# scale-lab/MTLoRA

Hardware: AMD Instinct MI355X
Metric: images/sec (train step) Swin-T/448 r=64 4-task (higher is better)
Workload: dtype bf16; 1 GPU; BASELINE configs[1]: Swin-T 448, 4 tasks (semseg,normals,sal,human_parts), r_shared=64 r_task=4 scale4; train step (fwd+loss+bwd+clip+AdamW), dropout .05, drop_path .2; per_gpu_batch=32, global_batch=32, img_size=448, parallelism=dp1, trainable_params=8344634, allreduce_bytes=0

## Files before the change

include/mtlora_hip.h:

```cpp
#ifndef MTLORA_HIP_H
#define MTLORA_HIP_H

#include <stdint.h>

#ifdef __cplusplus
extern "C" {
#endif

#define MTLORA_ABI_VERSION 12
#define MTLORA_MAX_TASKS 8

typedef enum mtlora_dtype {
    MTLORA_F32 = 0,
    MTLORA_BF16 = 1,
    MTLORA_F16 = 2,
    MTLORA_U8 = 3
} mtlora_dtype;

typedef enum mtlora_status {
    MTLORA_OK = 0,
    MTLORA_ERR_DTYPE = -1,
    MTLORA_ERR_SHAPE = -2,
    MTLORA_ERR_ALIGN = -3,
    MTLORA_ERR_NULL = -4,
// ... 4 lines not shown

int mtlora_version(void);
const char* mtlora_error_string(int status);

int mtlora_roll_and_window_partition_forward(const void* image, void* windows, int64_t B, int64_t H, int64_t W,
                                             int64_t C, int shift_size, int window_size, int dtype, void* stream);
int mtlora_roll_and_window_partition_backward(const void* grad_windows, void* grad_image, int64_t B, int64_t H,
                                              int64_t W, int64_t C, int shift_size, int window_size, int dtype,
                                              void* stream);
int mtlora_window_merge_and_roll_forward(const void* windows, void* image, int64_t B, int64_t H, int64_t W,
                                         int64_t C, int shift_size, int window_size, int dtype, void* stream);
int mtlora_window_merge_and_roll_backward(const void* grad_image, void* grad_windows, int64_t B, int64_t H,
                                          int64_t W, int64_t C, int shift_size, int window_size, int dtype,
                                          void* stream);

typedef struct mtlora_linear_desc {
    int64_t M, K, N;
    int32_t dtype;
    int32_t mode;
    int32_t T;
    int32_t r_s;
    int32_t r_t[MTLORA_MAX_TASKS];
    float scale_s;
    float scale_t[MTLORA_MAX_TASKS];
    int32_t has_x_tasks;
    float dropout_p;
    uint64_t seed;
    const uint64_t* seed_offset;
    int32_t bwd_phase;
    int32_t sel_stream;
    int32_t sel_dense;
    int32_t sel_tn;
    int32_t sel_projk;
    int32_t max_cu;
    const void* packed;
    int32_t hid;
    int32_t hid_pad_;
    const void* hid_ptr;
} mtlora_linear_desc;

#define MTLORA_HID_FWD_BASE 1
#define MTLORA_HID_P_GIVEN 2
#define MTLORA_HID_Q_GIVEN 4

int64_t mtlora_linear_ctx_bytes(const mtlora_linear_desc* d);

int64_t mtlora_linear_packed_bytes(const mtlora_linear_desc* d);
int mtlora_linear_pack(const mtlora_linear_desc* d, const float* A_s, const float* B_s, const float* const* A_t,
                       const float* const* B_t, void* packed, int64_t packed_bytes, void* stream);
int64_t mtlora_linear_pack_entry_bytes(void);
int mtlora_linear_pack_entry(const mtlora_linear_desc* d, const float* A_s, const float* B_s, const float* const* A_t,
                             const float* const* B_t, void* packed, int64_t packed_bytes, void* entry_host);
int mtlora_linear_pack_table(const void* table_dev, int n_entries, int dtype, void* stream);
int64_t mtlora_linear_bwd_scratch_bytes(const mtlora_linear_desc* d);

int mtlora_linear_fwd(const mtlora_linear_desc* d, const void* x, const void* const* x_t, const void* W,
                      const float* bias, const float* A_s, const float* B_s, const float* const* A_t,
                      const float* const* B_t, void* y_s, void* const* y_t, void* ctx, int64_t ctx_bytes,
                      void* stream);

int mtlora_linear_bwd(const mtlora_linear_desc* d, const void* x, const void* const* x_t, const void* Wt,
                      const void* dy_s, const void* const* dy_t, const void* ctx, int64_t ctx_bytes, void* dx,
                      void* const* dx_t, float* dA_s, float* dB_s, float* const* dA_t, float* const* dB_t,
                      void* scratch, int64_t scratch_bytes, void* stream);

int mtlora_linear_fwd_gelu(const mtlora_linear_desc* d, const void* x, const void* const* x_t, const void* W,
                           const float* bias, const float* A_s, const float* B_s, const float* const* A_t,
                           const float* const* B_t, void* y_s, void* const* y_t, void* a_s, void* const* a_t, void* ctx,
                           int64_t ctx_bytes, void* stream);

int mtlora_linear_bwd_gelu(const mtlora_linear_desc* d, const void* x, const void* const* x_t, const void* Wt,
                           const void* dy_s, const void* const* dy_t, const void* ctx, int64_t ctx_bytes, void* dx,
                           void* const* dx_t, float* dA_s, float* dB_s, float* const* dA_t, float* const* dB_t,
                           void* scratch, int64_t scratch_bytes, const void* h_s, const void* const* h_t, void* stream);

int mtlora_mlp_hid_supported(const mtlora_linear_desc* d1, const mtlora_linear_desc* d2);
int64_t mtlora_mlp_hid_fwd_scratch_bytes(const mtlora_linear_desc* d1, const mtlora_linear_desc* d2);
int64_t mtlora_mlp_hid_bwd_scratch_bytes(const mtlora_linear_desc* d1, const mtlora_linear_desc* d2);
int mtlora_mlp_hid_proj(const mtlora_linear_desc* d1, const mtlora_linear_desc* d2, const void* h_base, const void* ctx1,
                        void* ctx2, void* scratch, int64_t scratch_bytes, void* stream);
int mtlora_mlp_hid_bwd(const mtlora_linear_desc* d1, const mtlora_linear_desc* d2, const void* h_base, const void* dh_s,
                       const void* ctx1, const void* ctx2, const void* scratch2, void* scratch1, void* g, float* const* dB1_t,
                       float* const* dA2_t, void* part, int64_t part_bytes, void* stream);

int64_t mtlora_gemm_tn_scratch_bytes(int64_t M, int Na, int Nb);
int mtlora_gemm_tn(const void* a, const void* b, float* out, int64_t M, int Na, int Nb, int64_t lda, int64_t ldb,
                   int dtype, void* scratch, int64_t scratch_bytes, void* stream);

typedef struct mtlora_attn_desc {
    int64_t B;
    int32_t H, W;
    int32_t window_size;
    int32_t shift;
    int32_t num_heads;
    int32_t head_dim;
    int32_t image_layout;
    int32_t dtype;
    float scale;
    float mask_value;
} mtlora_attn_desc;

int64_t mtlora_window_attn_bwd_scratch_bytes(const mtlora_attn_desc* d);

int mtlora_window_attn_fwd(const mtlora_attn_desc* d, const void* qkv, const float* bias, const float* mask,
                           const int32_t* mask_ids, void* out, void* stream);
int mtlora_window_attn_bwd(const mtlora_attn_desc* d, const void* qkv, const float* bias, const float* mask,
                           const int32_t* mask_ids, const void* dout, void* dqkv, float* dbias, void* scratch,
                           int64_t scratch_bytes, void* stream);

int mtlora_layernorm_fwd(const void* x, const float* gamma, const float* beta, void* y, float* mean, float* rstd,
                         int64_t M, int64_t C, float eps, int x_dtype, int y_dtype, int merge_h, int merge_w, void* stream);
int64_t mtlora_layernorm_bwd_scratch_bytes(int64_t M, int64_t C, int x_dtype);
int mtlora_layernorm_bwd(const void* dy, const void* x, const float* gamma, const float* mean, const float* rstd,
                         void* dx, float* dgamma, float* dbeta, int64_t M, int64_t C, int x_dtype, int dy_dtype,
                         void* scratch, int64_t scratch_bytes, const void* dx_addend, int merge_h, int merge_w, void* stream);

int mtlora_residual_layernorm_fwd(const void* shortcut, const void* branch, const float* scale, int64_t B, const float* gamma,
                                  const float* beta, void* x_new, void* y, float* mean, float* rstd, int64_t M, int64_t C,
                                  float eps, int x_dtype, int y_dtype, void* stream);
int mtlora_residual_layernorm_bwd(const void* dy, const void* x_new, const float* gamma, const float* mean, const float* rstd,
                                  void* d_shortcut, void* d_branch, float* dgamma, float* dbeta, const float* scale,
                                  int64_t B, int64_t M, int64_t C, int x_dtype, int dy_dtype, void* scratch,
                                  int64_t scratch_bytes, const void* dx_addend, void* stream);

int64_t mtlora_layernorm_multi_bwd_scratch_bytes(int n, int64_t M, int64_t C, int x_dtype);
int mtlora_layernorm_multi_fwd(int n, const void* const* x, const float* gamma, const float* beta, void* const* y,
                               float* const* mean, float* const* rstd, int64_t M, int64_t C, float eps, int x_dtype, int y_dtype,
                               int merge_h, int merge_w, void* stream);
int mtlora_layernorm_multi_bwd(int n, const void* const* dy, const void* const* x, const float* gamma, const float* const* mean,
                               const float* const* rstd, void* const* dx, float* dgamma, float* dbeta, int64_t M, int64_t C,
                               int x_dtype, int dy_dtype, void* scratch, int64_t scratch_bytes, const void* const* dx_addend,
                               int merge_h, int merge_w, void* stream);

int mtlora_residual_layernorm_streams_fwd(int n, const void* const* res, const void* const* branch, const float* scale,
                                          int64_t B, const float* gamma, const float* beta, void* const* x_new, void* const* y,
                                          float* const* mean, float* const* rstd, int64_t M, int64_t C, float eps, int x_dtype,
                                          int y_dtype, int merge_h, int merge_w, void* stream);
int mtlora_residual_layernorm_streams_bwd(int n, const void* const* dy, const void* const* x_new, const float* gamma,
                                          const float* const* mean, const float* const* rstd, void* const* d_res,
                                          void* const* d_branch, float* dgamma, float* dbeta, const float* scale, int64_t B,
                                          int64_t M, int64_t C, int x_dtype, int dy_dtype, void* scratch, int64_t scratch_bytes,
                                          const void* const* dx_addend, int merge_h, int merge_w, void* stream);

int mtlora_residual_layernorm_multi_fwd(int n, const void* shortcut, const void* const* branch, const float* scale, int64_t B,
                                        const float* gamma, const float* beta, void* const* x_new, void* const* y,
                                        float* const* mean, float* const* rstd, int64_t M, int64_t C, float eps, int x_dtype,
                                        int y_dtype, void* stream);
int mtlora_residual_layernorm_multi_bwd(int n, const void* const* dy, const void* const* x_new, const float* gamma,
                                        const float* const* mean, const float* const* rstd, const void* const* dx_addend,
                                        void* d_shortcut, void* const* d_branch, float* dgamma, float* dbeta, const float* scale,
                                        int64_t B, int64_t M, int64_t C, int x_dtype, int dy_dtype, void* scratch,
                                        int64_t scratch_bytes, void* stream);

int64_t mtlora_bn_scratch_bytes(int64_t R, int64_t C, int dtype);
int mtlora_bn_relu_fwd(const void* x, const float* gamma, const float* beta, float* running_mean, float* running_var,
                       float momentum, float eps, int relu, void* y, float* save_mean, float* save_rstd,
                       float* save_scale, float* save_shift, int64_t R, int64_t C, int dtype, void* scratch,
                       int64_t scratch_bytes, void* stream);
int mtlora_bn_relu_bwd(const void* dy, const void* x, const float* save_mean, const float* save_rstd,
                       const float* save_scale, const float* save_shift, int relu, void* dx, float* dgamma, float* dbeta,
                       int64_t R, int64_t C, int dtype, void* scratch, int64_t scratch_bytes, void* stream);

int mtlora_residual_droppath_fwd(int n, const void* const* res, const void* const* y, void* const* out,
                                 const float* scale, int64_t M, int64_t C, int64_t B, int res_dtype, int y_dtype,
                                 void* stream);
int mtlora_residual_droppath_bwd(int n, const void* const* g, void* const* dy, void* dres, const float* scale,
                                 int64_t M, int64_t C, int64_t B, int res_dtype, int y_dtype, void* stream);

int64_t mtlora_upsample_loss_partials(int64_t B, int h, int w, int scale);
int mtlora_upsample_loss(int kind, const void* low, const float* label, const float* stat, void* dlow, float* partials,
                         int64_t B, int h, int w, int C, int scale, int dtype, float ignore_index, void* stream);

int mtlora_upsample_metrics_sizes(int kind, int64_t B, int h, int w, int C, int scale, int64_t* n_int64,
                                  int64_t* n_float_partials);
int mtlora_upsample_metrics(int kind, const void* low, const float* label, const float* stat, int64_t* counts,
                            float* fpartials, int64_t B, int h, int w, int C, int scale, int dtype, float ignore_index,
                            void* stream);

int mtlora_upsample_predict(int kind, const void* low, void* out, int64_t B, int h, int w, int C, int scale, int dtype,
                            int out_dtype, void* stream);

int64_t mtlora_colsum_scratch_bytes(int64_t M, int64_t N);
int mtlora_colsum(const void* x, int64_t M, int64_t N, int dtype, float* out, void* scratch, int64_t scratch_bytes, void* stream);
int64_t mtlora_label_stat_scratch_bytes(int64_t n);
int mtlora_label_stat(const float* label, int64_t n, int kind, float ignore_index, float* out, void* scratch,
                      int64_t scratch_bytes, void* stream);

int mtlora_upsample_cl_fwd(const void* coarse, void* fine, int64_t B, int h, int w, int C, int scale, int64_t ld_fine,
                           int dtype, void* stream);
int mtlora_upsample_cl_bwd(const void* grad_fine, void* grad_coarse, int64_t B, int h, int w, int C, int scale,
                           int64_t ld_fine, int dtype, void* stream);

typedef struct mtlora_block_desc {
    int64_t B;
    int32_t H, W, C, hidden;
    int32_t num_heads, window_size, shift;
    int32_t dtype;
    int32_t x_dtype;
    int32_t has_norm1;
    float eps1, eps2, eps_next;
    float attn_scale, mask_value;
    mtlora_linear_desc lin[4];
} mtlora_block_desc;

typedef struct mtlora_block_params {
    const float *norm1_g, *norm1_b;
    const float *norm2_g, *norm2_b, *next_g, *next_b;
    const void* W[4];
    const void* Wt[4];
    const float* bias[4];
    const float* A[4];
    const float* Bf[4];
    const float* attn_bias;
    const int32_t* mask_ids;
    const float* mask;
    const float *scale1, *scale2;
} mtlora_block_params;

typedef struct mtlora_block_grads {
    void* g_x;
    void* g_normed;
    float *d_norm1_g, *d_norm1_b;
    float *d_norm2_g, *d_norm2_b, *d_next_g, *d_next_b;
    float* dA[4];
    float* dB[4];
    float* dbias;
} mtlora_block_grads;

int64_t mtlora_block_save_bytes(const mtlora_block_desc* d);
int64_t mtlora_block_fwd_tmp_bytes(const mtlora_block_desc* d);
int64_t mtlora_block_bwd_scratch_bytes(const mtlora_block_desc* d);
int mtlora_block_fwd(const mtlora_block_desc* d, const mtlora_block_params* p, const void* x, const void* normed, void* x_out,
                     void* normed_out, void* save, int64_t save_bytes, void* tmp, int64_t tmp_bytes, void* stream);
int mtlora_block_bwd(const mtlora_block_desc* d, const mtlora_block_params* p, const void* x, const void* normed,
                     const void* x_out, const void* g_x_out, const void* g_normed_out, const void* save, int64_t save_bytes,
                     const mtlora_block_grads* g, void* scratch, int64_t scratch_bytes, int phase, void* stream);

#define MTLORA_ADAMW_CHUNK 4096
#define MTLORA_ADAMW_MAX_GROUPS 16
#define MTLORA_ADAMW_CTRL_WORDS 64
typedef struct mtlora_adamw_group {
    double lr, beta1, beta2, eps, weight_decay;
} mtlora_adamw_group;
int mtlora_adamw_sizes(int64_t n_tensors, const int64_t* numel, int64_t* n_chunks, int64_t* table_bytes,
                       int64_t* scratch_bytes);
int mtlora_adamw_table(int64_t n_tensors, const int64_t* numel, const int32_t* group, void* const* p, void* const* m,
                       void* const* v, void* host_table, int64_t table_bytes);
int mtlora_adamw_update(const void* table, const void* grads, int64_t n_tensors, int64_t n_chunks,
                        const mtlora_adamw_group* groups, int n_groups, float max_norm, float* ctrl, float* norm_out,
                        float* scale, int32_t* growth_tracker, float growth_factor, float backoff_factor,
                        int growth_interval, void* scratch, int64_t scratch_bytes, void* stream);

#define MTLORA_INGEST_MAX_JOBS 8
typedef enum mtlora_ingest_kind {
    MTLORA_INGEST_IMAGE = 0,
    MTLORA_INGEST_CLASS = 1,
    MTLORA_INGEST_CLASS_ALLZERO_IGNORE = 2,
    MTLORA_INGEST_NORMALS = 3,
    MTLORA_INGEST_DEPTH = 4
} mtlora_ingest_kind;
typedef struct mtlora_ingest_job {
    const void* src;
    void* dst;
    int32_t kind, src_dtype, C, reserved;
} mtlora_ingest_job;
int64_t mtlora_ingest_scratch_bytes(int n_jobs, int64_t B);
int mtlora_ingest_batch(const mtlora_ingest_job* jobs, int n_jobs, int64_t B, int32_t H, int32_t W, const uint8_t* flip,
                        const float* lut, void* scratch, int64_t scratch_bytes, void* stream);

#define MTLORA_AUGMENT_GEOM_BITS 24
#define MTLORA_AUGMENT_FLAG_NO_RENORM 1
typedef enum mtlora_augment_kind {
    MTLORA_AUGMENT_IMAGE_CUBIC_U8 = 0,
    MTLORA_AUGMENT_CLASS_NEAREST_U8 = 1,
    MTLORA_AUGMENT_NORMALS_CUBIC_F32 = 2,
    MTLORA_AUGMENT_DEPTH_NEAREST_F32 = 3
} mtlora_augment_kind;
typedef struct mtlora_augment_job {
    const void* src;
    void* dst;
    int32_t kind, flags;
} mtlora_augment_job;
int mtlora_augment_batch(const mtlora_augment_job* jobs, int n_jobs, int64_t B, int32_t Hc, int32_t Wc, int32_t Ho, int32_t Wo,
                         const int32_t* size, const int64_t* geom, const float* side, const int32_t* cubic_q15,
                         const float* cubic_f32, void* stream);

int mtlora_selftest_layouts(int32_t* out, void* stream);

#define MTLORA_PROF_KINDS 24
typedef struct mtlora_prof_summary {
    int64_t count[MTLORA_PROF_KINDS];
    double ms[MTLORA_PROF_KINDS];
    double alg_bytes[MTLORA_PROF_KINDS];
    double s8d_bytes[MTLORA_PROF_KINDS];
    double flops[MTLORA_PROF_KINDS];
} mtlora_prof_summary;
int mtlora_prof_begin(int max_records);
int mtlora_prof_end(mtlora_prof_summary* out);
const char* mtlora_prof_kind_name(int kind);

#ifdef __cplusplus
}
#endif
#endif
```

mtlora_amd/_lib.py:

```python
from __future__ import annotations

import ctypes
import os
from ctypes import POINTER, Structure, c_char_p, c_double, c_float, c_int, c_int32, c_int64, c_uint64, c_void_p

import torch

MAX_TASKS = 8
ABI_VERSION = 12
F32, BF16, F16, U8 = 0, 1, 2, 3
_DT = {torch.float32: F32, torch.bfloat16: BF16, torch.float16: F16}

_HERE = os.path.dirname(os.path.abspath(__file__))
LIB_PATH = os.path.join(_HERE, "csrc", "libmtlora_hip.so")


class LinearDesc(Structure):
    _fields_ = [("M", c_int64), ("K", c_int64), ("N", c_int64), ("dtype", c_int32), ("mode", c_int32),
                ("T", c_int32), ("r_s", c_int32), ("r_t", c_int32 * MAX_TASKS), ("scale_s", c_float),
                ("scale_t", c_float * MAX_TASKS), ("has_x_tasks", c_int32), ("dropout_p", c_float),
                ("seed", c_uint64), ("seed_offset", c_void_p), ("bwd_phase", c_int32),
                ("sel_stream", c_int32), ("sel_dense", c_int32), ("sel_tn", c_int32), ("sel_projk", c_int32),
                ("max_cu", c_int32), ("packed", c_void_p),
                ("hid", c_int32), ("hid_pad_", c_int32), ("hid_ptr", c_void_p)]


HID_FWD_BASE, HID_P_GIVEN, HID_Q_GIVEN = 1, 2, 4


class AttnDesc(Structure):
    _fields_ = [("B", c_int64), ("H", c_int32), ("W", c_int32), ("window_size", c_int32), ("shift", c_int32),
                ("num_heads", c_int32), ("head_dim", c_int32), ("image_layout", c_int32), ("dtype", c_int32),
                ("scale", c_float), ("mask_value", c_float)]


class BlockDesc(Structure):
    _fields_ = [("B", c_int64), ("H", c_int32), ("W", c_int32), ("C", c_int32), ("hidden", c_int32), ("num_heads", c_int32),
                ("window_size", c_int32), ("shift", c_int32), ("dtype", c_int32), ("x_dtype", c_int32), ("has_norm1", c_int32),
                ("eps1", c_float), ("eps2", c_float), ("eps_next", c_float), ("attn_scale", c_float), ("mask_value", c_float),
                ("lin", LinearDesc * 4)]


class BlockParams(Structure):
    _fields_ = [("norm1_g", c_void_p), ("norm1_b", c_void_p), ("norm2_g", c_void_p), ("norm2_b", c_void_p), ("next_g", c_void_p),
                ("next_b", c_void_p), ("W", c_void_p * 4), ("Wt", c_void_p * 4), ("bias", c_void_p * 4), ("A", c_void_p * 4),
                ("Bf", c_void_p * 4), ("attn_bias", c_void_p), ("mask_ids", c_void_p), ("mask", c_void_p), ("scale1", c_void_p),
                ("scale2", c_void_p)]


class BlockGrads(Structure):
    _fields_ = [("g_x", c_void_p), ("g_normed", c_void_p), ("d_norm1_g", c_void_p), ("d_norm1_b", c_void_p), ("d_norm2_g", c_void_p),
                ("d_norm2_b", c_void_p), ("d_next_g", c_void_p), ("d_next_b", c_void_p), ("dA", c_void_p * 4), ("dB", c_void_p * 4),
                ("dbias", c_void_p)]


class AdamwGroup(Structure):
    _fields_ = [("lr", c_double), ("beta1", c_double), ("beta2", c_double), ("eps", c_double), ("weight_decay", c_double)]


class IngestJob(Structure):
    _fields_ = [("src", c_void_p), ("dst", c_void_p), ("kind", c_int32), ("src_dtype", c_int32), ("C", c_int32),
                ("reserved", c_int32)]


class AugmentJob(Structure):
    _fields_ = [("src", c_void_p), ("dst", c_void_p), ("kind", c_int32), ("flags", c_int32)]


INGEST_MAX_JOBS = 8
AUGMENT_IMAGE_CUBIC_U8, AUGMENT_CLASS_NEAREST_U8, AUGMENT_NORMALS_CUBIC_F32, AUGMENT_DEPTH_NEAREST_F32 = 0, 1, 2, 3
AUGMENT_GEOM_BITS, AUGMENT_FLAG_NO_RENORM = 24, 1
INGEST_IMAGE, INGEST_CLASS, INGEST_CLASS_ALLZERO_IGNORE, INGEST_NORMALS, INGEST_DEPTH = 0, 1, 2, 3, 4

ADAMW_CHUNK, ADAMW_MAX_GROUPS, ADAMW_CTRL_WORDS = 4096, 16, 64

PROF_KINDS = 24


class ProfSummary(Structure):
    _fields_ = [("count", c_int64 * PROF_KINDS), ("ms", ctypes.c_double * PROF_KINDS),
                ("alg_bytes", ctypes.c_double * PROF_KINDS), ("s8d_bytes", ctypes.c_double * PROF_KINDS),
                ("flops", ctypes.c_double * PROF_KINDS)]


PtrArr = c_void_p * MAX_TASKS
PtrArr9 = c_void_p * (MAX_TASKS + 1)

_SIGS = {
    "mtlora_version": (c_int, []),
    "mtlora_error_string": (c_char_p, [c_int]),
    "mtlora_roll_and_window_partition_forward": (c_int, [c_void_p, c_void_p, c_int64, c_int64, c_int64, c_int64, c_int, c_int, c_int, c_void_p]),
    "mtlora_roll_and_window_partition_backward": (c_int, [c_void_p, c_void_p, c_int64, c_int64, c_int64, c_int64, c_int, c_int, c_int, c_void_p]),
    "mtlora_window_merge_and_roll_forward": (c_int, [c_void_p, c_void_p, c_int64, c_int64, c_int64, c_int64, c_int, c_int, c_int, c_void_p]),
    "mtlora_window_merge_and_roll_backward": (c_int, [c_void_p, c_void_p, c_int64, c_int64, c_int64, c_int64, c_int, c_int, c_int, c_void_p]),
    "mtlora_linear_ctx_bytes": (c_int64, [POINTER(LinearDesc)]),
    "mtlora_linear_bwd_scratch_bytes": (c_int64, [POINTER(LinearDesc)]),
    "mtlora_linear_packed_bytes": (c_int64, [POINTER(LinearDesc)]),
    "mtlora_linear_pack": (c_int, [POINTER(LinearDesc), c_void_p, c_void_p, POINTER(c_void_p), POINTER(c_void_p), c_void_p, c_int64,
                                   c_void_p]),
    "mtlora_linear_pack_entry_bytes": (c_int64, []),
    "mtlora_linear_pack_entry": (c_int, [POINTER(LinearDesc), c_void_p, c_void_p, POINTER(c_void_p), POINTER(c_void_p), c_void_p, c_int64,
                                         c_void_p]),
    "mtlora_linear_pack_table": (c_int, [c_void_p, c_int, c_int, c_void_p]),
    "mtlora_linear_fwd": (c_int, [POINTER(LinearDesc), c_void_p, POINTER(c_void_p), c_void_p, c_void_p, c_void_p, c_void_p,
                                  POINTER(c_void_p), POINTER(c_void_p), c_void_p, POINTER(c_void_p), c_void_p, c_int64,
                                  c_void_p]),
    "mtlora_linear_bwd": (c_int, [POINTER(LinearDesc), c_void_p, POINTER(c_void_p), c_void_p, c_void_p, POINTER(c_void_p),
                                  c_void_p, c_int64, c_void_p, POINTER(c_void_p), c_void_p, c_void_p, POINTER(c_void_p),
                                  POINTER(c_void_p), c_void_p, c_int64, c_void_p]),
    "mtlora_gemm_tn_scratch_bytes": (c_int64, [c_int64, c_int, c_int]),
    "mtlora_gemm_tn": (c_int, [c_void_p, c_void_p, c_void_p, c_int64, c_int, c_int, c_int64, c_int64, c_int, c_void_p, c_int64,
                               c_void_p]),
    "mtlora_linear_fwd_gelu": (c_int, [POINTER(LinearDesc), c_void_p, POINTER(c_void_p), c_void_p, c_void_p, c_void_p, c_void_p,
                                       POINTER(c_void_p), POINTER(c_void_p), c_void_p, POINTER(c_void_p), c_void_p,
                                       POINTER(c_void_p), c_void_p, c_int64, c_void_p]),
    "mtlora_linear_bwd_gelu": (c_int, [POINTER(LinearDesc), c_void_p, POINTER(c_void_p), c_void_p, c_void_p, POINTER(c_void_p),
                                       c_void_p, c_int64, c_void_p, POINTER(c_void_p), c_void_p, c_void_p, POINTER(c_void_p),
                                       POINTER(c_void_p), c_void_p, c_int64, c_void_p, POINTER(c_void_p), c_void_p]),
    "mtlora_mlp_hid_supported": (c_int, [POINTER(LinearDesc), POINTER(LinearDesc)]),
    "mtlora_mlp_hid_bwd_scratch_bytes": (c_int64, [POINTER(LinearDesc), POINTER(LinearDesc)]),
    "mtlora_mlp_hid_fwd_scratch_bytes": (c_int64, [POINTER(LinearDesc), POINTER(LinearDesc)]),
    "mtlora_mlp_hid_proj": (c_int, [POINTER(LinearDesc), POINTER(LinearDesc), c_void_p, c_void_p, c_void_p, c_void_p, c_int64, c_void_p]),
    "mtlora_mlp_hid_bwd": (c_int, [POINTER(LinearDesc), POINTER(LinearDesc), c_void_p, c_void_p, c_void_p, c_void_p, c_void_p, c_void_p,
                                   c_void_p, POINTER(c_void_p), POINTER(c_void_p), c_void_p, c_int64, c_void_p]),
    "mtlora_window_attn_bwd_scratch_bytes": (c_int64, [POINTER(AttnDesc)]),
    "mtlora_window_attn_fwd": (c_int, [POINTER(AttnDesc), c_void_p, c_void_p, c_void_p, c_void_p, c_void_p, c_void_p]),
    "mtlora_window_attn_bwd": (c_int, [POINTER(AttnDesc), c_void_p, c_void_p, c_void_p, c_void_p, c_void_p, c_void_p,
                                       c_void_p, c_void_p, c_int64, c_void_p]),
    "mtlora_layernorm_fwd": (c_int, [c_void_p, c_void_p, c_void_p, c_void_p, c_void_p, c_void_p, c_int64, c_int64, c_float,
                                     c_int, c_int, c_int, c_int, c_void_p]),
    "mtlora_layernorm_bwd_scratch_bytes": (c_int64, [c_int64, c_int64, c_int]),
    "mtlora_residual_layernorm_fwd": (c_int, [c_void_p, c_void_p, c_void_p, c_int64, c_void_p, c_void_p, c_void_p, c_void_p,
                                              c_void_p, c_void_p, c_int64, c_int64, c_float, c_int, c_int, c_void_p]),
    "mtlora_layernorm_multi_bwd_scratch_bytes": (c_int64, [c_int, c_int64, c_int64, c_int]),
    "mtlora_layernorm_multi_fwd": (c_int, [c_int, POINTER(c_void_p), c_void_p, c_void_p, POINTER(c_void_p), POINTER(c_void_p),
                                           POINTER(c_void_p), c_int64, c_int64, c_float, c_int, c_int, c_int, c_int, c_void_p]),
    "mtlora_layernorm_multi_bwd": (c_int, [c_int, POINTER(c_void_p), POINTER(c_void_p), c_void_p, POINTER(c_void_p),
                                           POINTER(c_void_p), POINTER(c_void_p), c_void_p, c_void_p, c_int64, c_int64, c_int,
                                           c_int, c_void_p, c_int64, POINTER(c_void_p), c_int, c_int, c_void_p]),
    "mtlora_residual_layernorm_streams_fwd": (c_int, [c_int, POINTER(c_void_p), POINTER(c_void_p), c_void_p, c_int64, c_void_p,
                                                      c_void_p, POINTER(c_void_p), POINTER(c_void_p), POINTER(c_void_p),
                                                      POINTER(c_void_p), c_int64, c_int64, c_float, c_int, c_int, c_int, c_int,
                                                      c_void_p]),
    "mtlora_residual_layernorm_streams_bwd": (c_int, [c_int, POINTER(c_void_p), POINTER(c_void_p), c_void_p, POINTER(c_void_p),
                                                      POINTER(c_void_p), POINTER(c_void_p), POINTER(c_void_p), c_void_p, c_void_p,
                                                      c_void_p, c_int64, c_int64, c_int64, c_int, c_int, c_void_p, c_int64,
                                                      POINTER(c_void_p), c_int, c_int, c_void_p]),
    "mtlora_residual_layernorm_multi_fwd": (c_int, [c_int, c_void_p, POINTER(c_void_p), c_void_p, c_int64, c_void_p, c_void_p,
                                                    POINTER(c_void_p), POINTER(c_void_p), POINTER(c_void_p), POINTER(c_void_p),
                                                    c_int64, c_int64, c_float, c_int, c_int, c_void_p]),
    "mtlora_residual_layernorm_multi_bwd": (c_int, [c_int, POINTER(c_void_p), POINTER(c_void_p), c_void_p, POINTER(c_void_p),
                                                    POINTER(c_void_p), POINTER(c_void_p), c_void_p, POINTER(c_void_p), c_void_p,
                                                    c_void_p, c_void_p, c_int64, c_int64, c_int64, c_int, c_int, c_void_p, c_int64,
                                                    c_void_p]),
    "mtlora_residual_layernorm_bwd": (c_int, [c_void_p, c_void_p, c_void_p, c_void_p, c_void_p, c_void_p, c_void_p, c_void_p,
                                              c_void_p, c_void_p, c_int64, c_int64, c_int64, c_int, c_int, c_void_p, c_int64,
                                              c_void_p, c_void_p]),
    "mtlora_layernorm_bwd": (c_int, [c_void_p, c_void_p, c_void_p, c_void_p, c_void_p, c_void_p, c_void_p, c_void_p,
                                     c_int64, c_int64, c_int, c_int, c_void_p, c_int64, c_void_p, c_int, c_int, c_void_p]),
    "mtlora_bn_scratch_bytes": (c_int64, [c_int64, c_int64, c_int]),
    "mtlora_bn_relu_fwd": (c_int, [c_void_p, c_void_p, c_void_p, c_void_p, c_void_p, c_float, c_float, c_int, c_void_p,
                                   c_void_p, c_void_p, c_void_p, c_void_p, c_int64, c_int64, c_int, c_void_p, c_int64,
                                   c_void_p]),
    "mtlora_bn_relu_bwd": (c_int, [c_void_p, c_void_p, c_void_p, c_void_p, c_void_p, c_void_p, c_int, c_void_p, c_void_p,
                                   c_void_p, c_int64, c_int64, c_int, c_void_p, c_int64, c_void_p]),
    "mtlora_residual_droppath_fwd": (c_int, [c_int, POINTER(c_void_p), POINTER(c_void_p), POINTER(c_void_p), c_void_p,
                                             c_int64, c_int64, c_int64, c_int, c_int, c_void_p]),
    "mtlora_residual_droppath_bwd": (c_int, [c_int, POINTER(c_void_p), POINTER(c_void_p), c_void_p, c_void_p, c_int64,
                                             c_int64, c_int64, c_int, c_int, c_void_p]),
    "mtlora_upsample_loss_partials": (c_int64, [c_int64, c_int, c_int, c_int]),
    "mtlora_colsum_scratch_bytes": (c_int64, [c_int64, c_int64]),
    "mtlora_colsum": (c_int, [c_void_p, c_int64, c_int64, c_int, c_void_p, c_void_p, c_int64, c_void_p]),
    "mtlora_label_stat_scratch_bytes": (c_int64, [c_int64]),
    "mtlora_label_stat": (c_int, [c_void_p, c_int64, c_int, c_float, c_void_p, c_void_p, c_int64, c_void_p]),
    "mtlora_upsample_loss": (c_int, [c_int, c_void_p, c_void_p, c_void_p, c_void_p, c_void_p, c_int64, c_int, c_int, c_int,
                                     c_int, c_int, ctypes.c_float, c_void_p]),
    "mtlora_upsample_metrics_sizes": (c_int, [c_int, c_int64, c_int, c_int, c_int, c_int, POINTER(c_int64), POINTER(c_int64)]),
    "mtlora_upsample_metrics": (c_int, [c_int, c_void_p, c_void_p, c_void_p, c_void_p, c_void_p, c_int64, c_int, c_int, c_int,
                                        c_int, c_int, ctypes.c_float, c_void_p]),
    "mtlora_upsample_predict": (c_int, [c_int, c_void_p, c_void_p, c_int64, c_int, c_int, c_int, c_int, c_int, c_int, c_void_p]),
    "mtlora_upsample_cl_fwd": (c_int, [c_void_p, c_void_p, c_int64, c_int, c_int, c_int, c_int, c_int64, c_int, c_void_p]),
    "mtlora_upsample_cl_bwd": (c_int, [c_void_p, c_void_p, c_int64, c_int, c_int, c_int, c_int, c_int64, c_int, c_void_p]),
    "mtlora_block_save_bytes": (c_int64, [POINTER(BlockDesc)]),
    "mtlora_block_fwd_tmp_bytes": (c_int64, [POINTER(BlockDesc)]),
    "mtlora_block_bwd_scratch_bytes": (c_int64, [POINTER(BlockDesc)]),
    "mtlora_block_fwd": (c_int, [POINTER(BlockDesc), POINTER(BlockParams), c_void_p, c_void_p, c_void_p, c_void_p, c_void_p, c_int64,
                                 c_void_p, c_int64, c_void_p]),
    "mtlora_block_bwd": (c_int, [POINTER(BlockDesc), POINTER(BlockParams), c_void_p, c_void_p, c_void_p, c_void_p, c_void_p, c_void_p,
                                 c_int64, POINTER(BlockGrads), c_void_p, c_int64, c_int, c_void_p]),
    "mtlora_adamw_sizes": (c_int, [c_int64, POINTER(c_int64), POINTER(c_int64), POINTER(c_int64), POINTER(c_int64)]),
    "mtlora_adamw_table": (c_int, [c_int64, POINTER(c_int64), POINTER(c_int32), POINTER(c_void_p), POINTER(c_void_p), POINTER(c_void_p),
                                   c_void_p, c_int64]),
    "mtlora_adamw_update": (c_int, [c_void_p, c_void_p, c_int64, c_int64, POINTER(AdamwGroup), c_int, c_float, c_void_p, c_void_p,
                                    c_void_p, c_void_p, c_float, c_float, c_int, c_void_p, c_int64, c_void_p]),
    "mtlora_ingest_scratch_bytes": (c_int64, [c_int, c_int64]),
    "mtlora_ingest_batch": (c_int, [POINTER(IngestJob), c_int, c_int64, c_int32, c_int32, c_void_p, c_void_p, c_void_p, c_int64,
                                    c_void_p]),
    "mtlora_augment_batch": (c_int, [POINTER(AugmentJob), c_int, c_int64, c_int32, c_int32, c_int32, c_int32, c_void_p, c_void_p,
                                     c_void_p, c_void_p, c_void_p, c_void_p]),
    "mtlora_selftest_layouts": (c_int, [c_void_p, c_void_p]),
    "mtlora_prof_begin": (c_int, [c_int]),
    "mtlora_prof_end": (c_int, [POINTER(ProfSummary)]),
    "mtlora_prof_kind_name": (c_char_p, [c_int]),
}
EXPORTS = tuple(_SIGS)

_lib = None


def lib() -> ctypes.CDLL:
    global _lib
    if _lib is None:
        if not os.path.exists(LIB_PATH):
            raise RuntimeError(
                f"mtlora_amd: {LIB_PATH} not found. Build it with `python -m mtlora_amd.csrc.build` "
                "(or __graft_entry__.build()). There is no eager/CPU fallback for the MTLoRA hot path.")
        L = ctypes.CDLL(LIB_PATH)
        for name, (res, args) in _SIGS.items():
            fn = getattr(L, name)
            fn.restype, fn.argtypes = res, args
        v = L.mtlora_version()
        if v != ABI_VERSION:
            raise RuntimeError(f"mtlora_amd: libmtlora_hip.so ABI {v} != binding ABI {ABI_VERSION}; rebuild")
        _lib = L
    return _lib


def check(status: int, what: str) -> None:
    if status != 0:
        msg = lib().mtlora_error_string(status).decode()
        raise RuntimeError(f"mtlora_amd: {what} failed: {msg} (status {status})")


def dtype_code(t: torch.Tensor, allow_f16: bool = True) -> int:
    code = _DT.get(t.dtype)
    if code is None or (code == F16 and not allow_f16):
        raise RuntimeError(f"mtlora_amd: unsupported dtype {t.dtype} (fp32, bf16 and fp16 are supported)")
    return code


def require_gpu(*tensors: torch.Tensor) -> None:
    cur = None
    for t in tensors:
        if t is None:
            continue
        if not t.is_cuda:
            raise RuntimeError("mtlora_amd: tensors must live on a ROCm GPU (MI355X); the HIP path has no CPU fallback")
        if cur is None:
            cur = torch._C._cuda_getDevice()
        if t.device.index != cur:
            raise RuntimeError(f"mtlora_amd: tensor on cuda:{t.device.index} but the current device is cuda:{cur}; the HIP "
                               "path launches on the current device's stream -- call torch.cuda.set_device(tensor.device) first")


def ptr(t) -> c_void_p:
    return c_void_p(0 if t is None else t.data_ptr())


_NO_PTRS = None


def ptr_array(ts) -> "PtrArr":
    global _NO_PTRS
    if not ts:
        if _NO_PTRS is None:
            _NO_PTRS = PtrArr()
        return _NO_PTRS
    a = PtrArr()
    for i in range(MAX_TASKS):
        a[i] = 0 if (ts is None or i >= len(ts) or ts[i] is None) else ts[i].data_ptr()
    return a


def ptr_array9(ts) -> "PtrArr9":
    a = PtrArr9()
    for i in range(MAX_TASKS + 1):
        a[i] = 0 if (ts is None or i >= len(ts) or ts[i] is None) else ts[i].data_ptr()
    return a


def stream_ptr() -> c_void_p:
    return c_void_p(torch._C._cuda_getCurrentRawStream(torch._C._cuda_getDevice()))
```

mtlora_amd/csrc/glue.hip:

```cpp
#include "common.h"
#include "internal.h"

namespace {

constexpr int LN_MAXV = 8;

template <typename T>
__device__ __forceinline__ void ld_vec(const T* p, float (&f)[8]);
template <>
__device__ __forceinline__ void ld_vec<float>(const float* p, float (&f)[8]) {
    f32x4 v = *reinterpret_cast<const f32x4*>(p);
    f[0] = v[0];
    f[1] = v[1];
    f[2] = v[2];
    f[3] = v[3];
}
template <>
__device__ __forceinline__ void ld_vec<bf16>(const bf16* p, float (&f)[8]) {
    Vec16<bf16> v = mtl_ld16<bf16>(p);
#pragma unroll
    for (int e = 0; e < 8; ++e) f[e] = (float)v.e[e];
}
template <>
__device__ __forceinline__ void ld_vec<f16>(const f16* p, float (&f)[8]) {
    Vec16<f16> v = mtl_ld16<f16>(p);
#pragma unroll
    for (int e = 0; e < 8; ++e) f[e] = (float)v.e[e];
}
template <typename T, int NE>
__device__ __forceinline__ void st_vec(T* p, const float* f) {
    if constexpr (sizeof(T) == 4) {
#pragma unroll
        for (int e = 0; e < NE; e += 4) *reinterpret_cast<f32x4*>(p + e) = f32x4{f[e], f[e + 1], f[e + 2], f[e + 3]};
    } else if constexpr (NE == 8) {
        Vec16<T> v;
#pragma unroll
        for (int e = 0; e < 8; ++e) v.e[e] = (T)f[e];
        *reinterpret_cast<u32x4*>(p) = v.raw;
    } else {
        *reinterpret_cast<u32x2*>(p) = u32x2{mtl_pack2<T>(f[0], f[1]), mtl_pack2<T>(f[2], f[3])};
    }
}

template <int LPR>
__device__ __forceinline__ float group_sum(float v) {
#pragma unroll
    for (int o = LPR / 2; o > 0; o >>= 1) v += __shfl_xor(v, o);
    return v;
}

struct LnParams {
    const void* x;
    const float* gamma;
    const float* beta;
    void* y;
    float* mean;
    float* rstd;
    const void* dy;
    void* dx;
    const void* add;
    float* part;
    int64_t M;
    int C;
    float eps;
    int mg_H, mg_W;
    const void* rb;
    void* xsum;
    void* dbr;
    const float* rscale;
    int64_t rows_per_sample;
    int nk;
    const void* rb_k[MTLORA_MAX_TASKS + 1];
    void* xsum_k[MTLORA_MAX_TASKS + 1];
    void* y_k[MTLORA_MAX_TASKS + 1];
    float* mean_k[MTLORA_MAX_TASKS + 1];
    float* rstd_k[MTLORA_MAX_TASKS + 1];
    const void* dy_k[MTLORA_MAX_TASKS + 1];
    const void* add_k[MTLORA_MAX_TASKS + 1];
    void* dbr_k[MTLORA_MAX_TASKS + 1];
    int multi_x;
    const void* x_k[MTLORA_MAX_TASKS + 1];
    void* dx_k[MTLORA_MAX_TASKS + 1];
};
typedef const __attribute__((address_space(4))) LnParams* LnKargs;

__device__ __forceinline__ int64_t row_div(int64_t row, int64_t d, int64_t rows) {
    if (rows <= (int64_t)0x7FFFFFFF) return (int64_t)((uint32_t)row / (uint32_t)d);
    return row / d;
}

struct LnRow {
    int64_t base;
};
__device__ __forceinline__ LnRow ln_row(const LnParams& p, int64_t row) {
    LnRow r;
    if (p.mg_W == 0) {
        r.base = row * p.C;
    } else {
        const int W2 = p.mg_W >> 1, H2 = p.mg_H >> 1, Cs = p.C >> 2;
        const int64_t b = row_div(row, (int64_t)H2 * W2, p.M);
        const int rem = (int)(row - b * H2 * W2);
        const int y2 = rem / W2, x2 = rem - y2 * W2;
        r.base = ((b * p.mg_H + 2 * y2) * p.mg_W + 2 * x2) * (int64_t)Cs;
    }
    return r;
}
__device__ __forceinline__ int64_t ln_col(const LnParams& p, int col) {
    if (p.mg_W == 0) return col;
    const int Cs = p.C >> 2, q = col / Cs, within = col - q * Cs;
    return ((int64_t)(q & 1) * p.mg_W + (q >> 1)) * Cs + within;
}

template <typename T>
__device__ __forceinline__ void cvt_vec(const u32x4& r, float (&f)[8]);
template <>
__device__ __forceinline__ void cvt_vec<float>(const u32x4& r, float (&f)[8]) {
    const f32x4 v = __builtin_bit_cast(f32x4, r);
    f[0] = v[0];
    f[1] = v[1];
    f[2] = v[2];
    f[3] = v[3];
}
template <>
__device__ __forceinline__ void cvt_vec<bf16>(const u32x4& r, float (&f)[8]) {
#pragma unroll
    for (int q = 0; q < 4; ++q) {
        f[2 * q] = __builtin_bit_cast(float, r[q] << 16);
        f[2 * q + 1] = __builtin_bit_cast(float, r[q] & 0xFFFF0000u);
    }
}
template <>
__device__ __forceinline__ void cvt_vec<f16>(const u32x4& r, float (&f)[8]) {
#pragma unroll
    for (int q = 0; q < 4; ++q) {
        f[2 * q] = mtl_lo2<f16>(r[q]);
        f[2 * q + 1] = mtl_hi2<f16>(r[q]);
    }
}

template <typename T, int NE>
__device__ __forceinline__ void ld_n(const T* p, float (&f)[8]) {
    if constexpr (sizeof(T) == 4) {
#pragma unroll
        for (int e = 0; e < NE; e += 4) {
            const f32x4 v = *reinterpret_cast<const f32x4*>(p + e);
            f[e] = v[0];
            f[e + 1] = v[1];
            f[e + 2] = v[2];
            f[e + 3] = v[3];
        }
    } else if constexpr (NE == 8) {
        cvt_vec<T>(*reinterpret_cast<const u32x4*>(p), f);
    } else {
        const u32x2 r = *reinterpret_cast<const u32x2*>(p);
        f[0] = mtl_lo2<T>(r[0]);
        f[1] = mtl_hi2<T>(r[0]);
        f[2] = mtl_lo2<T>(r[1]);
        f[3] = mtl_hi2<T>(r[1]);
    }
}
template <typename T>
__device__ __forceinline__ u32x4 pack_vec(const float (&f)[8]) {
    if constexpr (sizeof(T) == 4) {
        return __builtin_bit_cast(u32x4, f32x4{f[0], f[1], f[2], f[3]});
    } else {
        Vec16<T> v;
#pragma unroll
        for (int e = 0; e < 8; ++e) v.e[e] = (T)f[e];
        return v.raw;
    }
}

template <typename TI, typename TO, int LPR, int MAXV, bool RES>
__global__ __launch_bounds__(256) void k_ln_fwd(const LnParams p) {
    constexpr int VE = ET<TI>::VEC;
    constexpr int RPW = 64 / LPR;
    constexpr int UNR = MAXV <= 3 ? 4 : 1;
    const int lane = threadIdx.x & 63, wave = threadIdx.x >> 6;
    const int sub = lane / LPR, lr = lane % LPR;
    const int nvec = p.C / VE;
    const TI* x = reinterpret_cast<const TI*>(p.x);
    TO* y = reinterpret_cast<TO*>(p.y);
    float* mean_out = p.mean;
    float* rstd_out = p.rstd;
    const void* rb_ptr = p.rb;
    void* xs_ptr = p.xsum;
    const float* rscale = p.rscale;
    if (p.multi_x) {
        LnKargs K = (LnKargs)__builtin_amdgcn_kernarg_segment_ptr();
        const int k = blockIdx.y;
        x = reinterpret_cast<const TI*>(K->x_k[k]);
        y = reinterpret_cast<TO*>(K->y_k[k]);
        mean_out = K->mean_k[k];
        rstd_out = K->rstd_k[k];
        if constexpr (RES) {
            rb_ptr = K->rb_k[k];
            xs_ptr = K->xsum_k[k];
            if (rscale) rscale += (int64_t)k * (p.M / p.rows_per_sample);
        }
    }
    if constexpr (RES) {
        if (p.nk > 0) {
            LnKargs K = (LnKargs)__builtin_amdgcn_kernarg_segment_ptr();
            const int k = blockIdx.y;
            y = reinterpret_cast<TO*>(K->y_k[k]);
            mean_out = K->mean_k[k];
            rstd_out = K->rstd_k[k];
            rb_ptr = K->rb_k[k];
            xs_ptr = K->xsum_k[k];
            if (rscale) rscale += (int64_t)k * (p.M / p.rows_per_sample);
        }
    }
    float g[MAXV][VE], b[MAXV][VE];
#pragma unroll
    for (int i = 0; i < MAXV; ++i) {
        const int v = lr + i * LPR;
#pragma unroll
        for (int e = 0; e < VE; ++e) {
            g[i][e] = v < nvec ? p.gamma[v * VE + e] : 0.f;
            b[i][e] = v < nvec ? p.beta[v * VE + e] : 0.f;
        }
    }
    int64_t coff[MAXV];
#pragma unroll
    for (int i = 0; i < MAXV; ++i) coff[i] = ln_col(p, (lr + i * LPR < nvec ? lr + i * LPR : 0) * VE);
    const float inv_c = 1.f / (float)p.C;
    const int64_t rows_per_blk = 4 * RPW * UNR;
    for (int64_t r0 = (int64_t)blockIdx.x * rows_per_blk; r0 < p.M; r0 += (int64_t)gridDim.x * rows_per_blk) {
        u32x4 raw[UNR][MAXV];
        int64_t row[UNR], xbs[UNR];
#pragma unroll
        for (int u = 0; u < UNR; ++u) {
            row[u] = r0 + (int64_t)(wave * UNR + u) * RPW + sub;
            const int64_t xb = ln_row(p, row[u] < p.M ? row[u] : 0).base;
            xbs[u] = xb;
#pragma unroll
            for (int i = 0; i < MAXV; ++i) {
                const int v = lr + i * LPR;
                raw[u][i] = (row[u] < p.M && v < nvec) ? *reinterpret_cast<const u32x4*>(x + xb + coff[i])
                                                      : u32x4{0u, 0u, 0u, 0u};
            }
        }
        if constexpr (RES) {
            const TO* rb = reinterpret_cast<const TO*>(rb_ptr);
            TI* xs = reinterpret_cast<TI*>(xs_ptr);
            constexpr bool PRE = sizeof(TO) * VE <= 16;
            u32x4 braw[PRE ? UNR : 1][PRE ? MAXV : 1];
            float scv[UNR];
#pragma unroll
            for (int u = 0; u < UNR; ++u) {
                const bool rok = row[u] < p.M;
                scv[u] = (rok && rscale) ? rscale[row_div(row[u], p.rows_per_sample, p.M)] : 1.f;
                if constexpr (PRE) {
#pragma unroll
                    for (int i = 0; i < MAXV; ++i) {
                        const int v = lr + i * LPR;
                        u32x4 b = {0u, 0u, 0u, 0u};
                        if (rok && v < nvec) {
                            if constexpr (sizeof(TO) * VE == 16) {
                                b = *reinterpret_cast<const u32x4*>(rb + xbs[u] + coff[i]);
                            } else {
                                const u32x2 h2 = *reinterpret_cast<const u32x2*>(rb + xbs[u] + coff[i]);
                                b[0] = h2[0];
                                b[1] = h2[1];
                            }
                        }
                        braw[u][i] = b;
                    }
                }
            }
#pragma unroll
            for (int u = 0; u < UNR; ++u) {
                if (row[u] >= p.M) continue;
                const float sc = scv[u];
#pragma unroll
                for (int i = 0; i < MAXV; ++i) {
                    const int v = lr + i * LPR;
                    if (v < nvec) {
                        float fb[8], fx[8];
                        if constexpr (!PRE) {
                            ld_n<TO, VE>(rb + xbs[u] + coff[i], fb);
                        } else if constexpr (sizeof(TO) == 4) {
                            const f32x4 q4 = __builtin_bit_cast(f32x4, braw[u][i]);
                            fb[0] = q4[0];
                            fb[1] = q4[1];
                            fb[2] = q4[2];
                            fb[3] = q4[3];
                        } else if constexpr (VE == 8) {
                            cvt_vec<TO>(braw[u][i], fb);
                        } else {
                            fb[0] = mtl_lo2<TO>(braw[u][i][0]);
                            fb[1] = mtl_hi2<TO>(braw[u][i][0]);
                            fb[2] = mtl_lo2<TO>(braw[u][i][1]);
                            fb[3] = mtl_hi2<TO>(braw[u][i][1]);
                        }
                        cvt_vec<TI>(raw[u][i], fx);
#pragma unroll
                        for (int e = 0; e < VE; ++e) fx[e] += sc * fb[e];
                        raw[u][i] = pack_vec<TI>(fx);
                        *reinterpret_cast<u32x4*>(xs + xbs[u] + coff[i]) = raw[u][i];
                    }
                }
            }
        }
#pragma unroll
        for (int u = 0; u < UNR; ++u) {
            float f[8];
            float s = 0.f;
#pragma unroll
            for (int i = 0; i < MAXV; ++i) {
                cvt_vec<TI>(raw[u][i], f);
#pragma unroll
                for (int e = 0; e < VE; ++e) s += f[e];
            }
            const float mean = group_sum<LPR>(s) * inv_c;
            float q = 0.f;
#pragma unroll
            for (int i = 0; i < MAXV; ++i) {
                if (lr + i * LPR < nvec) {
                    cvt_vec<TI>(raw[u][i], f);
#pragma unroll
                    for (int e = 0; e < VE; ++e) {
                        const float d = f[e] - mean;
                        q += d * d;
                    }
                }
            }
            const float rstd = rsqrtf(group_sum<LPR>(q) * inv_c + p.eps);
            if (row[u] < p.M) {
                if (lr == 0) {
                    mean_out[row[u]] = mean;
                    rstd_out[row[u]] = rstd;
                }
#pragma unroll
                for (int i = 0; i < MAXV; ++i) {
                    const int v = lr + i * LPR;
                    if (v < nvec) {
                        cvt_vec<TI>(raw[u][i], f);
                        float o[8];
#pragma unroll
                        for (int e = 0; e < VE; ++e) o[e] = (f[e] - mean) * rstd * g[i][e] + b[i][e];
                        st_vec<TO, VE>(y + row[u] * p.C + v * VE, o);
                    }
                }
            }
        }
    }
}

template <typename TX, typename TG, int LPR, int MAXV>
__global__ __launch_bounds__(256) void k_ln_bwd(const LnParams p) {
    constexpr int VE = ET<TX>::VEC;
    constexpr int RPW = 64 / LPR;
    extern __shared__ __attribute__((aligned(16))) float sm[];
    const int lane = threadIdx.x & 63, wave = threadIdx.x >> 6;
    const int sub = lane / LPR, lr = lane % LPR;
    const int nvec = p.C / VE;
    const TX* x = reinterpret_cast<const TX*>(p.x);
    const TG* dy = reinterpret_cast<const TG*>(p.dy);
    TX* dx = reinterpret_cast<TX*>(p.dx);
    const TX* addp = reinterpret_cast<const TX*>(p.add);
    const float* mean_in = p.mean;
    const float* rstd_in = p.rstd;
    void* dbr_ptr = p.dbr;
    const float* rscale_in = p.rscale;
    float* part_out = p.part + (int64_t)blockIdx.x * 2 * p.C;
    if (p.multi_x) {
        LnKargs K = (LnKargs)__builtin_amdgcn_kernarg_segment_ptr();
        const int k = blockIdx.y;
        x = reinterpret_cast<const TX*>(K->x_k[k]);
        dy = reinterpret_cast<const TG*>(K->dy_k[k]);
        dx = reinterpret_cast<TX*>(K->dx_k[k]);
        addp = reinterpret_cast<const TX*>(K->add_k[k]);
        mean_in = K->mean_k[k];
        rstd_in = K->rstd_k[k];
        part_out = p.part + ((int64_t)k * gridDim.x + blockIdx.x) * 2 * p.C;
        dbr_ptr = K->dbr_k[k];
        if (rscale_in) rscale_in += (int64_t)k * (p.M / p.rows_per_sample);
    }
    float g[MAXV][VE], ag[MAXV][VE], ab[MAXV][VE];
#pragma unroll
    for (int i = 0; i < MAXV; ++i) {
        const int v = lr + i * LPR;
#pragma unroll
        for (int e = 0; e < VE; ++e) {
            g[i][e] = v < nvec ? p.gamma[v * VE + e] : 0.f;
            ag[i][e] = 0.f;
            ab[i][e] = 0.f;
        }
    }
    int64_t coff[MAXV];
#pragma unroll
    for (int i = 0; i < MAXV; ++i) coff[i] = ln_col(p, (lr + i * LPR < nvec ? lr + i * LPR : 0) * VE);
    constexpr int UNR = (MAXV <= 3 && sizeof(TX) == 4) ? 2 : 1;
    constexpr int GW = sizeof(TG) == sizeof(TX) ? 4 : (sizeof(TG) == 2 ? 2 : 8);
    const int64_t rows_per_blk = 4 * RPW * UNR;
    for (int64_t r0 = (int64_t)blockIdx.x * rows_per_blk; r0 < p.M; r0 += (int64_t)gridDim.x * rows_per_blk) {
        u32x4 rx[UNR][MAXV], ra[UNR][MAXV];
        uint32_t rg[UNR][MAXV][GW];
        int64_t row[UNR], xb[UNR];
        float mean[UNR], rstd[UNR], scv[UNR];
#pragma unroll
        for (int u = 0; u < UNR; ++u) {
            row[u] = r0 + (int64_t)(wave * UNR + u) * RPW + sub;
            const bool rv = row[u] < p.M;
            xb[u] = ln_row(p, rv ? row[u] : 0).base;
            mean[u] = rv ? mean_in[row[u]] : 0.f;
            rstd[u] = rv ? rstd_in[row[u]] : 0.f;
            scv[u] = (rv && dbr_ptr && rscale_in) ? rscale_in[row_div(row[u], p.rows_per_sample, p.M)] : 1.f;
#pragma unroll
            for (int i = 0; i < MAXV; ++i) {
                const int v = lr + i * LPR;
                const bool ok = rv && v < nvec;
                rx[u][i] = ok ? *reinterpret_cast<const u32x4*>(x + xb[u] + coff[i]) : u32x4{0u, 0u, 0u, 0u};
                const TG* gp = dy + (rv ? row[u] : 0) * p.C + (v < nvec ? v : 0) * VE;
                if constexpr (GW == 4) {
                    const u32x4 t = ok ? *reinterpret_cast<const u32x4*>(gp) : u32x4{0u, 0u, 0u, 0u};
#pragma unroll
                    for (int q = 0; q < 4; ++q) rg[u][i][q] = t[q];
                } else if constexpr (GW == 2) {
                    const u32x2 t = ok ? *reinterpret_cast<const u32x2*>(gp) : u32x2{0u, 0u};
                    rg[u][i][0] = t[0];
                    rg[u][i][1] = t[1];
                } else {
                    const u32x4 t0 = ok ? *reinterpret_cast<const u32x4*>(gp) : u32x4{0u, 0u, 0u, 0u};
                    const u32x4 t1 = ok ? *reinterpret_cast<const u32x4*>(gp + 4) : u32x4{0u, 0u, 0u, 0u};
#pragma unroll
                    for (int q = 0; q < 4; ++q) {
                        rg[u][i][q] = t0[q];
                        rg[u][i][4 + q] = t1[q];
                    }
                }
                ra[u][i] = (ok && addp) ? *reinterpret_cast<const u32x4*>(addp + xb[u] + coff[i]) : u32x4{0u, 0u, 0u, 0u};
            }
        }
#pragma unroll
        for (int u = 0; u < UNR; ++u) {
            const bool rv = row[u] < p.M;
            float xh[MAXV][VE], gy[MAXV][VE];
            float c1 = 0.f, c2 = 0.f;
#pragma unroll
            for (int i = 0; i < MAXV; ++i) {
                float fx[8], fg[8];
                cvt_vec<TX>(rx[u][i], fx);
                if constexpr (GW == 4) {
                    cvt_vec<TG>(u32x4{rg[u][i][0], rg[u][i][1], rg[u][i][2], rg[u][i][3]}, fg);
                } else if constexpr (GW == 2) {
                    fg[0] = mtl_lo2<TG>(rg[u][i][0]);
                    fg[1] = mtl_hi2<TG>(rg[u][i][0]);
                    fg[2] = mtl_lo2<TG>(rg[u][i][1]);
                    fg[3] = mtl_hi2<TG>(rg[u][i][1]);
                } else {
#pragma unroll
                    for (int q = 0; q < 8; ++q) fg[q] = __builtin_bit_cast(float, rg[u][i][q]);
                }
#pragma unroll
                for (int e = 0; e < VE; ++e) {
                    const float h = (fx[e] - mean[u]) * rstd[u];
                    xh[i][e] = h;
                    ag[i][e] += fg[e] * h;
                    ab[i][e] += fg[e];
                    const float t = fg[e] * g[i][e];
                    gy[i][e] = t;
                    c1 += t;
                    c2 += t * h;
                }
            }
            c1 = group_sum<LPR>(c1) / p.C;
            c2 = group_sum<LPR>(c2) / p.C;
            if (rv) {
#pragma unroll
                for (int i = 0; i < MAXV; ++i) {
                    const int v = lr + i * LPR;
                    if (v < nvec) {
                        float o[8], fa[8];
                        cvt_vec<TX>(ra[u][i], fa);
#pragma unroll
                        for (int e = 0; e < VE; ++e) o[e] = rstd[u] * (gy[i][e] - c1 - xh[i][e] * c2) + fa[e];
                        st_vec<TX, VE>(dx + xb[u] + coff[i], o);
                        if (dbr_ptr) {
                            const float sc = scv[u];
#pragma unroll
                            for (int e = 0; e < VE; ++e) o[e] *= sc;
                            st_vec<TG, VE>(reinterpret_cast<TG*>(dbr_ptr) + xb[u] + coff[i], o);
                        }
                    }
                }
            }
        }
    }
    float* mine = sm + (size_t)(wave * RPW + sub) * 2 * p.C;
#pragma unroll
    for (int i = 0; i < MAXV; ++i) {
        const int v = lr + i * LPR;
        if (v < nvec) {
#pragma unroll
            for (int e = 0; e < VE; ++e) {
                mine[v * VE + e] = ag[i][e];
                mine[p.C + v * VE + e] = ab[i][e];
            }
        }
    }
    __syncthreads();
    float* dst = part_out;
    for (int i = threadIdx.x; i < 2 * p.C; i += 256) {
        float t = 0.f;
        for (int gi = 0; gi < 4 * RPW; ++gi) t += sm[(size_t)gi * 2 * p.C + i];
        dst[i] = t;
    }
}

template <typename TX, typename TG, int LPR, int MAXV>
__global__ __launch_bounds__(256) void k_resln_bwd_multi(const LnParams p) {
    constexpr int VE = ET<TX>::VEC;
    constexpr int RPW = 64 / LPR;
    constexpr int GW = sizeof(TG) == sizeof(TX) ? 4 : (sizeof(TG) == 2 ? 2 : 8);
    extern __shared__ __attribute__((aligned(16))) float sm[];
    LnKargs K = (LnKargs)__builtin_amdgcn_kernarg_segment_ptr();
    const int lane = threadIdx.x & 63, wave = threadIdx.x >> 6;
    const int sub = lane / LPR, lr = lane % LPR;
    const int nvec = p.C / VE;
    TX* dsh = reinterpret_cast<TX*>(p.dx);
    const int64_t Bn = p.M / p.rows_per_sample;
    float g[MAXV][VE], ag[MAXV][VE], ab[MAXV][VE];
#pragma unroll
    for (int i = 0; i < MAXV; ++i) {
        const int v = lr + i * LPR;
#pragma unroll
        for (int e = 0; e < VE; ++e) {
            g[i][e] = v < nvec ? p.gamma[v * VE + e] : 0.f;
            ag[i][e] = 0.f;
            ab[i][e] = 0.f;
        }
    }
    struct Regs {
        u32x4 rx[MAXV], ra[MAXV];
        uint32_t rg[MAXV][GW];
        float mean, rstd, sc;
    };
    const int64_t rows_per_blk = 4 * RPW;
    for (int64_t r0 = (int64_t)blockIdx.x * rows_per_blk; r0 < p.M; r0 += (int64_t)gridDim.x * rows_per_blk) {
        const int64_t row = r0 + wave * RPW + sub;
        const bool rv = row < p.M;
        const int64_t rbase = (rv ? row : 0) * p.C;
        float dsum[MAXV][VE];
#pragma unroll
        for (int i = 0; i < MAXV; ++i)
#pragma unroll
            for (int e = 0; e < VE; ++e) dsum[i][e] = 0.f;
        auto load = [&](Regs& R, int k) __attribute__((always_inline)) {
            const TX* x = reinterpret_cast<const TX*>(K->xsum_k[k]);
            const TG* dy = reinterpret_cast<const TG*>(K->dy_k[k]);
            const TX* addp = reinterpret_cast<const TX*>(K->add_k[k]);
            R.mean = rv ? K->mean_k[k][row] : 0.f;
            R.rstd = rv ? K->rstd_k[k][row] : 0.f;
            R.sc = (rv && p.rscale) ? p.rscale[(int64_t)k * Bn + row_div(row, p.rows_per_sample, p.M)] : 1.f;
#pragma unroll
            for (int i = 0; i < MAXV; ++i) {
                const int v = lr + i * LPR;
                const bool ok = rv && v < nvec;
                const int64_t off = rbase + (v < nvec ? v : 0) * VE;
                R.rx[i] = ok ? *reinterpret_cast<const u32x4*>(x + off) : u32x4{0u, 0u, 0u, 0u};
                R.ra[i] = (ok && addp) ? *reinterpret_cast<const u32x4*>(addp + off) : u32x4{0u, 0u, 0u, 0u};
                const TG* gp = dy + off;
                if constexpr (GW == 4) {
                    const u32x4 t = ok ? *reinterpret_cast<const u32x4*>(gp) : u32x4{0u, 0u, 0u, 0u};
#pragma unroll
                    for (int q = 0; q < 4; ++q) R.rg[i][q] = t[q];
                } else if constexpr (GW == 2) {
                    const u32x2 t = ok ? *reinterpret_cast<const u32x2*>(gp) : u32x2{0u, 0u};
                    R.rg[i][0] = t[0];
                    R.rg[i][1] = t[1];
                } else {
                    const u32x4 t0 = ok ? *reinterpret_cast<const u32x4*>(gp) : u32x4{0u, 0u, 0u, 0u};
                    const u32x4 t1 = ok ? *reinterpret_cast<const u32x4*>(gp + 4) : u32x4{0u, 0u, 0u, 0u};
#pragma unroll
                    for (int q = 0; q < 4; ++q) {
                        R.rg[i][q] = t0[q];
                        R.rg[i][4 + q] = t1[q];
                    }
                }
            }
        };
        auto compute = [&](Regs& R, int k) __attribute__((always_inline)) {
            TG* dbr = reinterpret_cast<TG*>(K->dbr_k[k]);
            float xh[MAXV][VE], gy[MAXV][VE];
            float c1 = 0.f, c2 = 0.f;
#pragma unroll
            for (int i = 0; i < MAXV; ++i) {
                float fx[8], fg[8];
                cvt_vec<TX>(R.rx[i], fx);
                if constexpr (GW == 4) {
                    cvt_vec<TG>(u32x4{R.rg[i][0], R.rg[i][1], R.rg[i][2], R.rg[i][3]}, fg);
                } else if constexpr (GW == 2) {
                    fg[0] = mtl_lo2<TG>(R.rg[i][0]);
                    fg[1] = mtl_hi2<TG>(R.rg[i][0]);
                    fg[2] = mtl_lo2<TG>(R.rg[i][1]);
                    fg[3] = mtl_hi2<TG>(R.rg[i][1]);
                } else {
#pragma unroll
                    for (int q = 0; q < 8; ++q) fg[q] = __builtin_bit_cast(float, R.rg[i][q]);
                }
#pragma unroll
                for (int e = 0; e < VE; ++e) {
                    const float h = (fx[e] - R.mean) * R.rstd;
                    xh[i][e] = h;
                    ag[i][e] += fg[e] * h;
                    ab[i][e] += fg[e];
                    const float t = fg[e] * g[i][e];
                    gy[i][e] = t;
                    c1 += t;
                    c2 += t * h;
                }
            }
            c1 = group_sum<LPR>(c1) / p.C;
            c2 = group_sum<LPR>(c2) / p.C;
            if (rv) {
#pragma unroll
                for (int i = 0; i < MAXV; ++i) {
                    const int v = lr + i * LPR;
                    if (v < nvec) {
                        float o[8], fa[8];
                        cvt_vec<TX>(R.ra[i], fa);
#pragma unroll
                        for (int e = 0; e < VE; ++e) {
                            o[e] = R.rstd * (gy[i][e] - c1 - xh[i][e] * c2) + fa[e];
                            dsum[i][e] += o[e];
                            o[e] *= R.sc;
                        }
                        if (dbr) st_vec<TG, VE>(dbr + rbase + v * VE, o);
                    }
                }
            }
        };
        if constexpr (sizeof(TX) == 4) {
            Regs A, Bq;
            load(A, 0);
            for (int k = 0; k < p.nk; k += 2) {
                if (k + 1 < p.nk) load(Bq, k + 1);
                compute(A, k);
                if (k + 1 < p.nk) {
                    if (k + 2 < p.nk) load(A, k + 2);
                    compute(Bq, k + 1);
                }
            }
        } else {
            Regs A;
            for (int k = 0; k < p.nk; ++k) {
                load(A, k);
                compute(A, k);
            }
        }
        if (rv) {
#pragma unroll
            for (int i = 0; i < MAXV; ++i) {
                const int v = lr + i * LPR;
                if (v < nvec) st_vec<TX, VE>(dsh + rbase + v * VE, dsum[i]);
            }
        }
    }
    float* mine = sm + (size_t)(wave * RPW + sub) * 2 * p.C;
#pragma unroll
    for (int i = 0; i < MAXV; ++i) {
        const int v = lr + i * LPR;
        if (v < nvec) {
#pragma unroll
            for (int e = 0; e < VE; ++e) {
                mine[v * VE + e] = ag[i][e];
                mine[p.C + v * VE + e] = ab[i][e];
            }
        }
    }
    __syncthreads();
    float* dst = p.part + (int64_t)blockIdx.x * 2 * p.C;
    for (int i = threadIdx.x; i < 2 * p.C; i += 256) {
        float t = 0.f;
        for (int gi = 0; gi < 4 * RPW; ++gi) t += sm[(size_t)gi * 2 * p.C + i];
        dst[i] = t;
    }
}

constexpr int LN_RW = 16;
__global__ __launch_bounds__(64 * LN_RW) void k_ln_reduce(const float* part, float* dgamma, float* dbeta, int nblk, int C) {
    __shared__ float sm[LN_RW][64];
    const int lane = threadIdx.x & 63, wave = threadIdx.x >> 6;
    const int c = blockIdx.x * 64 + lane;
    float a0 = 0.f, a1 = 0.f, a2 = 0.f, a3 = 0.f;
    if (c < 2 * C) {
        int b = wave;
        for (; b + 3 * LN_RW < nblk; b += 4 * LN_RW) {
            a0 += part[(int64_t)b * 2 * C + c];
            a1 += part[(int64_t)(b + LN_RW) * 2 * C + c];
            a2 += part[(int64_t)(b + 2 * LN_RW) * 2 * C + c];
            a3 += part[(int64_t)(b + 3 * LN_RW) * 2 * C + c];
        }
        for (; b < nblk; b += LN_RW) a0 += part[(int64_t)b * 2 * C + c];
    }
    sm[wave][lane] = (a0 + a1) + (a2 + a3);
    __syncthreads();
    if (wave == 0 && c < 2 * C) {
        float t = 0.f;
#pragma unroll
        for (int w = 0; w < LN_RW; ++w) t += sm[w][lane];
        if (c < C)
            dgamma[c] = t;
        else
            dbeta[c - C] = t;
    }
}

int pick_lpr(int nvec) {
    int lpr = 8;
    while (lpr < 64 && (nvec + lpr - 1) / lpr > 3) lpr *= 2;
    return lpr;
}

int ln_grid(int64_t M, int lpr, int cap = 256 * 4, int unr = 1) {
    const int64_t rows_per_blk = 4 * (64 / lpr) * unr;
    int64_t g = mtl_ceil_div(M, rows_per_blk);
    if (g > cap) g = cap;
    return (int)(g < 1 ? 1 : g);
}

int ln_merge(LnParams& p, int64_t M, int64_t C, int xdt, int mh, int mw) {
    p.mg_H = p.mg_W = 0;
    if (mh == 0 && mw == 0) return MTLORA_OK;
    const int ve = xdt == MTLORA_F32 ? 4 : 8;
    if (mh <= 0 || mw <= 0 || (mh & 1) || (mw & 1) || C % 4 || (C / 4) % ve) return MTLORA_ERR_SHAPE;
    if (M % ((int64_t)(mh / 2) * (mw / 2))) return MTLORA_ERR_SHAPE;
    p.mg_H = mh;
    p.mg_W = mw;
    return MTLORA_OK;
}

int ln_check(int64_t M, int64_t C, int xdt, int ydt) {
    if (xdt < MTLORA_F32 || xdt > MTLORA_F16 || ydt < MTLORA_F32 || ydt > MTLORA_F16) return MTLORA_ERR_DTYPE;
    if (xdt != MTLORA_F32 && ydt != MTLORA_F32 && xdt != ydt) return MTLORA_ERR_DTYPE;
    const int ve = xdt == MTLORA_F32 ? 4 : 8;
    if (M < 0 || C <= 0 || C % ve) return MTLORA_ERR_SHAPE;
    if (mtl_ceil_div(C / ve, 64) > LN_MAXV) return MTLORA_ERR_UNSUPPORTED;
    return MTLORA_OK;
}

}

extern "C" {

int64_t mtlora_layernorm_bwd_scratch_bytes(int64_t M, int64_t C, int x_dtype) {
    if (ln_check(M, C, x_dtype, MTLORA_F32) != MTLORA_OK) return -1;
    const int lpr = pick_lpr((int)(C / (x_dtype == MTLORA_F32 ? 4 : 8)));
    return (int64_t)ln_grid(M, lpr) * 2 * C * 4 + 256;
}

#define LN_LAUNCH(KERNEL, L_, ...)                                                                        \
    if (vpl <= 3)                                                                                           \
        hipLaunchKernelGGL((KERNEL<__VA_ARGS__, L_, 3 LN_EXTRA>), dim3(grid), dim3(256), lds, s, p);         \
    else                                                                                                    \
        hipLaunchKernelGGL((KERNEL<__VA_ARGS__, L_, LN_MAXV LN_EXTRA>), dim3(grid), dim3(256), lds, s, p);
#define LN_DISPATCH_LPR(KERNEL, ...)                       \
    switch (lpr) {                                         \
        case 8: LN_LAUNCH(KERNEL, 8, __VA_ARGS__) break;   \
        case 16: LN_LAUNCH(KERNEL, 16, __VA_ARGS__) break; \
        case 32: LN_LAUNCH(KERNEL, 32, __VA_ARGS__) break; \
        default: LN_LAUNCH(KERNEL, 64, __VA_ARGS__) break; \
    }

static int ln_fwd_impl(const void* x, const float* gamma, const float* beta, void* y, float* mean, float* rstd, int64_t M,
                       int64_t C, float eps, int x_dtype, int y_dtype, int merge_h, int merge_w, const void* branch,
                       void* x_new, const float* scale, int64_t B, void* stream) {
    int st = ln_check(M, C, x_dtype, y_dtype);
    if (st != MTLORA_OK) return st;
    if (!x || !gamma || !beta || !y || !mean || !rstd) return MTLORA_ERR_NULL;
    if (((uintptr_t)x | (uintptr_t)y | (uintptr_t)branch | (uintptr_t)x_new) & 15u) return MTLORA_ERR_ALIGN;
    if (branch && (!x_new || B <= 0 || M % B || merge_h || merge_w)) return MTLORA_ERR_SHAPE;
    if (M == 0) return MTLORA_OK;
    LnParams p = {};
    p.rb = branch;
    p.xsum = x_new;
    p.rscale = scale;
    p.rows_per_sample = branch ? M / B : 1;
    p.x = x;
    p.gamma = gamma;
    p.beta = beta;
    p.y = y;
    p.mean = mean;
    p.rstd = rstd;
    p.M = M;
    p.C = (int)C;
    p.eps = eps;
    st = ln_merge(p, M, C, x_dtype, merge_h, merge_w);
    if (st != MTLORA_OK) return st;
    const int nvec_h = (int)(C / (x_dtype == MTLORA_F32 ? 4 : 8));
    const int lpr = pick_lpr(nvec_h);
    const int vpl = (nvec_h + lpr - 1) / lpr;
    const int grid = (int)mtl_ceil_div(ln_grid(M, lpr, 1 << 30), vpl <= 3 ? 4 : 1) < 256 * 8
                         ? (int)mtl_ceil_div(ln_grid(M, lpr, 1 << 30), vpl <= 3 ? 4 : 1)
                         : 256 * 8;
    const size_t lds = 0;
    hipStream_t s = (hipStream_t)stream;
    const int es_x = mtl_elem_size(x_dtype), es_y = mtl_elem_size(y_dtype);
    mtl_prof_tag("M%lld C%lld x%d y%d mg%d", (long long)M, (long long)C, x_dtype, y_dtype, merge_w);
    MtlProfScope prof(PK_LN_FWD, (double)M * C * (es_x + es_y + (branch ? es_x + es_y : 0)), s);
    if (branch) {
#define LN_EXTRA , true
        if (x_dtype == MTLORA_F32 && y_dtype == MTLORA_F32) {
            LN_DISPATCH_LPR(k_ln_fwd, float, float)
        } else if (x_dtype == MTLORA_F16 || y_dtype == MTLORA_F16) {
            if (x_dtype == MTLORA_F32) {
                LN_DISPATCH_LPR(k_ln_fwd, float, f16)
            } else if (y_dtype == MTLORA_F32) {
                LN_DISPATCH_LPR(k_ln_fwd, f16, float)
            } else {
                LN_DISPATCH_LPR(k_ln_fwd, f16, f16)
            }
        } else if (x_dtype == MTLORA_F32) {
            LN_DISPATCH_LPR(k_ln_fwd, float, bf16)
        } else if (y_dtype == MTLORA_F32) {
            LN_DISPATCH_LPR(k_ln_fwd, bf16, float)
        } else {
            LN_DISPATCH_LPR(k_ln_fwd, bf16, bf16)
        }
#undef LN_EXTRA
    } else {
#define LN_EXTRA , false
        if (x_dtype == MTLORA_F32 && y_dtype == MTLORA_F32) {
            LN_DISPATCH_LPR(k_ln_fwd, float, float)
        } else if (x_dtype == MTLORA_F16 || y_dtype == MTLORA_F16) {
            if (x_dtype == MTLORA_F32) {
                LN_DISPATCH_LPR(k_ln_fwd, float, f16)
            } else if (y_dtype == MTLORA_F32) {
                LN_DISPATCH_LPR(k_ln_fwd, f16, float)
            } else {
                LN_DISPATCH_LPR(k_ln_fwd, f16, f16)
            }
        } else if (x_dtype == MTLORA_F32) {
            LN_DISPATCH_LPR(k_ln_fwd, float, bf16)
        } else if (y_dtype == MTLORA_F32) {
            LN_DISPATCH_LPR(k_ln_fwd, bf16, float)
        } else {
            LN_DISPATCH_LPR(k_ln_fwd, bf16, bf16)
        }
#undef LN_EXTRA
    }
    MTL_CHECK_LAUNCH();
    return MTLORA_OK;
}

int mtlora_layernorm_fwd(const void* x, const float* gamma, const float* beta, void* y, float* mean, float* rstd,
                         int64_t M, int64_t C, float eps, int x_dtype, int y_dtype, int merge_h, int merge_w, void* stream) {
    return ln_fwd_impl(x, gamma, beta, y, mean, rstd, M, C, eps, x_dtype, y_dtype, merge_h, merge_w, nullptr, nullptr, nullptr,
                       1, stream);
}

int mtlora_residual_layernorm_fwd(const void* shortcut, const void* branch, const float* scale, int64_t B, const float* gamma,
                                  const float* beta, void* x_new, void* y, float* mean, float* rstd, int64_t M, int64_t C,
                                  float eps, int x_dtype, int y_dtype, void* stream) {
    if (!branch || !x_new) return MTLORA_ERR_NULL;
    return ln_fwd_impl(shortcut, gamma, beta, y, mean, rstd, M, C, eps, x_dtype, y_dtype, 0, 0, branch, x_new, scale, B, stream);
}

static int ln_bwd_impl(const void* dy, const void* x, const float* gamma, const float* mean, const float* rstd, void* dx,
                       float* dgamma, float* dbeta, int64_t M, int64_t C, int x_dtype, int dy_dtype, void* scratch,
                       int64_t scratch_bytes, const void* dx_addend, int merge_h, int merge_w, void* d_branch,
                       const float* scale, int64_t B, void* stream, int phase = 0) {
    int st = ln_check(M, C, x_dtype, dy_dtype);
    if (st != MTLORA_OK) return st;
    if (!dy || !x || !gamma || !mean || !rstd || !dx || !dgamma || !dbeta || !scratch) return MTLORA_ERR_NULL;
    if (((uintptr_t)x | (uintptr_t)dy | (uintptr_t)dx | (uintptr_t)scratch | (uintptr_t)dx_addend | (uintptr_t)d_branch) & 15u)
        return MTLORA_ERR_ALIGN;
    if (d_branch && (B <= 0 || M % B || merge_h || merge_w)) return MTLORA_ERR_SHAPE;
    if (scratch_bytes < mtlora_layernorm_bwd_scratch_bytes(M, C, x_dtype) - 256) return MTLORA_ERR_WORKSPACE;
    hipStream_t s = (hipStream_t)stream;
    if (M == 0) {
        mtl_zero_async(dgamma, (size_t)C * 4, s);
        mtl_zero_async(dbeta, (size_t)C * 4, s);
        return MTLORA_OK;
    }
    LnParams p = {};
    p.x = x;
    p.dy = dy;
    p.gamma = gamma;
    p.mean = const_cast<float*>(mean);
    p.rstd = const_cast<float*>(rstd);
    p.dx = dx;
    p.add = dx_addend;
    p.dbr = d_branch;
    p.rscale = scale;
    p.rows_per_sample = d_branch ? M / B : 1;
    p.part = reinterpret_cast<float*>(scratch);
    p.M = M;
    p.C = (int)C;
    st = ln_merge(p, M, C, x_dtype, merge_h, merge_w);
    if (st != MTLORA_OK) return st;
    const int nvec_h = (int)(C / (x_dtype == MTLORA_F32 ? 4 : 8));
    const int lpr = pick_lpr(nvec_h);
    const int vpl = (nvec_h + lpr - 1) / lpr;
    const int grid = ln_grid(M, lpr);
    const size_t lds = (size_t)4 * (64 / lpr) * 2 * C * 4;
    const int es_x = mtl_elem_size(x_dtype), es_g = mtl_elem_size(dy_dtype);
    if (phase != 2) {
        mtl_prof_tag("M%lld C%lld x%d g%d mg%d add%d", (long long)M, (long long)C, x_dtype, dy_dtype, merge_w, dx_addend ? 1 : 0);
        MtlProfScope prof(PK_LN_BWD, (double)M * C * (2 * es_x + es_g + (dx_addend ? es_x : 0) + (d_branch ? es_g : 0)), s);
#define LN_EXTRA
        if (x_dtype == MTLORA_F32 && dy_dtype == MTLORA_F32) {
            LN_DISPATCH_LPR(k_ln_bwd, float, float)
        } else if (x_dtype == MTLORA_F16 || dy_dtype == MTLORA_F16) {
            if (x_dtype == MTLORA_F32) {
                LN_DISPATCH_LPR(k_ln_bwd, float, f16)
            } else if (dy_dtype == MTLORA_F32) {
                LN_DISPATCH_LPR(k_ln_bwd, f16, float)
            } else {
                LN_DISPATCH_LPR(k_ln_bwd, f16, f16)
            }
        } else if (x_dtype == MTLORA_F32) {
            LN_DISPATCH_LPR(k_ln_bwd, float, bf16)
        } else if (dy_dtype == MTLORA_F32) {
            LN_DISPATCH_LPR(k_ln_bwd, bf16, float)
        } else {
            LN_DISPATCH_LPR(k_ln_bwd, bf16, bf16)
        }
#undef LN_EXTRA
    }
    if (phase != 1)
        hipLaunchKernelGGL(k_ln_reduce, dim3((unsigned)mtl_ceil_div(2 * C, 64)), dim3(64 * LN_RW), 0, s, (const float*)p.part, dgamma,
                           dbeta, grid, (int)C);
    MTL_CHECK_LAUNCH();
    return MTLORA_OK;
}

int mtli_layernorm_bwd(const void* dy, const void* x, const float* gamma, const float* mean, const float* rstd, void* dx,
                       float* dgamma, float* dbeta, int64_t M, int64_t C, int x_dtype, int dy_dtype, void* scratch,
                       int64_t scratch_bytes, const void* dx_addend, int phase, void* stream) {
    return ln_bwd_impl(dy, x, gamma, mean, rstd, dx, dgamma, dbeta, M, C, x_dtype, dy_dtype, scratch, scratch_bytes, dx_addend, 0, 0,
                       nullptr, nullptr, 1, stream, phase);
}

int mtli_residual_layernorm_bwd(const void* dy, const void* x_new, const float* gamma, const float* mean, const float* rstd,
                                void* d_shortcut, void* d_branch, float* dgamma, float* dbeta, const float* scale, int64_t B,
                                int64_t M, int64_t C, int x_dtype, int dy_dtype, void* scratch, int64_t scratch_bytes,
                                const void* dx_addend, int phase, void* stream) {
    if (!d_branch) return MTLORA_ERR_NULL;
    return ln_bwd_impl(dy, x_new, gamma, mean, rstd, d_shortcut, dgamma, dbeta, M, C, x_dtype, dy_dtype, scratch, scratch_bytes,
                       dx_addend, 0, 0, d_branch, scale, B, stream, phase);
}

int mtlora_layernorm_bwd(const void* dy, const void* x, const float* gamma, const float* mean, const float* rstd,
                         void* dx, float* dgamma, float* dbeta, int64_t M, int64_t C, int x_dtype, int dy_dtype,
                         void* scratch, int64_t scratch_bytes, const void* dx_addend, int merge_h, int merge_w, void* stream) {
    return ln_bwd_impl(dy, x, gamma, mean, rstd, dx, dgamma, dbeta, M, C, x_dtype, dy_dtype, scratch, scratch_bytes, dx_addend,
                       merge_h, merge_w, nullptr, nullptr, 1, stream);
}

int mtlora_residual_layernorm_bwd(const void* dy, const void* x_new, const float* gamma, const float* mean, const float* rstd,
                                  void* d_shortcut, void* d_branch, float* dgamma, float* dbeta, const float* scale,
                                  int64_t B, int64_t M, int64_t C, int x_dtype, int dy_dtype, void* scratch,
                                  int64_t scratch_bytes, const void* dx_addend, void* stream) {
    if (!d_branch) return MTLORA_ERR_NULL;
    return ln_bwd_impl(dy, x_new, gamma, mean, rstd, d_shortcut, dgamma, dbeta, M, C, x_dtype, dy_dtype, scratch, scratch_bytes,
                       dx_addend, 0, 0, d_branch, scale, B, stream);
}

int64_t mtlora_layernorm_multi_bwd_scratch_bytes(int n, int64_t M, int64_t C, int x_dtype) {
    const int64_t one = mtlora_layernorm_bwd_scratch_bytes(M, C, x_dtype);
    if (one < 0 || n < 1 || n > MTLORA_MAX_TASKS + 1) return -1;
    return (one - 256) * n + 256;
}

static int ln_multi_fwd_impl(int n, const void* const* x, const float* gamma, const float* beta, void* const* y,
                             float* const* mean, float* const* rstd, int64_t M, int64_t C, float eps, int x_dtype, int y_dtype,
                             int merge_h, int merge_w, const void* const* branch, void* const* x_new, const float* scale,
                             int64_t B, void* stream) {
    int st = ln_check(M, C, x_dtype, y_dtype);
    if (st != MTLORA_OK) return st;
    if (n < 1 || n > MTLORA_MAX_TASKS + 1) return MTLORA_ERR_SHAPE;
    if (!x || !gamma || !beta || !y || !mean || !rstd) return MTLORA_ERR_NULL;
    if (branch && (!x_new || B <= 0 || M % B)) return MTLORA_ERR_SHAPE;
    LnParams p = {};
    for (int k = 0; k < n; ++k) {
        if (!x[k] || !y[k] || !mean[k] || !rstd[k]) return MTLORA_ERR_NULL;
        if (((uintptr_t)x[k] | (uintptr_t)y[k]) & 15u) return MTLORA_ERR_ALIGN;
        p.x_k[k] = x[k];
        p.y_k[k] = y[k];
        p.mean_k[k] = mean[k];
        p.rstd_k[k] = rstd[k];
        if (branch) {
            if (!branch[k] || !x_new[k]) return MTLORA_ERR_NULL;
            if (((uintptr_t)branch[k] | (uintptr_t)x_new[k]) & 15u) return MTLORA_ERR_ALIGN;
            p.rb_k[k] = branch[k];
            p.xsum_k[k] = x_new[k];
        }
    }
    if (M == 0) return MTLORA_OK;
    if (branch) {
        p.rb = branch[0];
        p.xsum = x_new[0];
        p.rscale = scale;
    }
    p.multi_x = 1;
    p.x = x[0];
    p.y = y[0];
    p.mean = mean[0];
    p.rstd = rstd[0];
    p.gamma = gamma;
    p.beta = beta;
    p.M = M;
    p.C = (int)C;
    p.eps = eps;
    p.rows_per_sample = branch ? M / B : 1;
    st = ln_merge(p, M, C, x_dtype, merge_h, merge_w);
    if (st != MTLORA_OK) return st;
    const int nvec_h = (int)(C / (x_dtype == MTLORA_F32 ? 4 : 8));
    const int lpr = pick_lpr(nvec_h);
    const int vpl = (nvec_h + lpr - 1) / lpr;
    const int gx = (int)mtl_ceil_div(ln_grid(M, lpr, 1 << 30), vpl <= 3 ? 4 : 1) < 256 * 8
                       ? (int)mtl_ceil_div(ln_grid(M, lpr, 1 << 30), vpl <= 3 ? 4 : 1)
                       : 256 * 8;
    const dim3 grid((unsigned)gx, (unsigned)n);
    const size_t lds = 0;
    hipStream_t s = (hipStream_t)stream;
    const int es_x = mtl_elem_size(x_dtype), es_y = mtl_elem_size(y_dtype);
    mtl_prof_tag("M%lld C%lld x%d y%d mg%d n%d res%d", (long long)M, (long long)C, x_dtype, y_dtype, merge_w, n, branch ? 1 : 0);
    MtlProfScope prof(PK_LN_FWD, (double)n * M * C * (es_x + es_y + (branch ? es_x + es_y : 0)), s);
    if (branch) {
#define LN_EXTRA , true
        if (x_dtype == MTLORA_F32 && y_dtype == MTLORA_F32) {
            LN_DISPATCH_LPR(k_ln_fwd, float, float)
        } else if (x_dtype == MTLORA_F16 || y_dtype == MTLORA_F16) {
            if (x_dtype == MTLORA_F32) {
                LN_DISPATCH_LPR(k_ln_fwd, float, f16)
            } else if (y_dtype == MTLORA_F32) {
                LN_DISPATCH_LPR(k_ln_fwd, f16, float)
            } else {
                LN_DISPATCH_LPR(k_ln_fwd, f16, f16)
            }
        } else if (x_dtype == MTLORA_F32) {
            LN_DISPATCH_LPR(k_ln_fwd, float, bf16)
        } else if (y_dtype == MTLORA_F32) {
            LN_DISPATCH_LPR(k_ln_fwd, bf16, float)
        } else {
            LN_DISPATCH_LPR(k_ln_fwd, bf16, bf16)
        }
#undef LN_EXTRA
    } else {
#define LN_EXTRA , false
        if (x_dtype == MTLORA_F32 && y_dtype == MTLORA_F32) {
            LN_DISPATCH_LPR(k_ln_fwd, float, float)
        } else if (x_dtype == MTLORA_F16 || y_dtype == MTLORA_F16) {
            if (x_dtype == MTLORA_F32) {
                LN_DISPATCH_LPR(k_ln_fwd, float, f16)
            } else if (y_dtype == MTLORA_F32) {
                LN_DISPATCH_LPR(k_ln_fwd, f16, float)
            } else {
                LN_DISPATCH_LPR(k_ln_fwd, f16, f16)
            }
        } else if (x_dtype == MTLORA_F32) {
            LN_DISPATCH_LPR(k_ln_fwd, float, bf16)
        } else if (y_dtype == MTLORA_F32) {
            LN_DISPATCH_LPR(k_ln_fwd, bf16, float)
        } else {
            LN_DISPATCH_LPR(k_ln_fwd, bf16, bf16)
        }
#undef LN_EXTRA
    }
    MTL_CHECK_LAUNCH();
    return MTLORA_OK;
}

int mtlora_layernorm_multi_fwd(int n, const void* const* x, const float* gamma, const float* beta, void* const* y,
                               float* const* mean, float* const* rstd, int64_t M, int64_t C, float eps, int x_dtype, int y_dtype,
                               int merge_h, int merge_w, void* stream) {
    return ln_multi_fwd_impl(n, x, gamma, beta, y, mean, rstd, M, C, eps, x_dtype, y_dtype, merge_h, merge_w, nullptr, nullptr,
                             nullptr, 1, stream);
}

int mtlora_residual_layernorm_streams_fwd(int n, const void* const* res, const void* const* branch, const float* scale,
                                          int64_t B, const float* gamma, const float* beta, void* const* x_new, void* const* y,
                                          float* const* mean, float* const* rstd, int64_t M, int64_t C, float eps, int x_dtype,
                                          int y_dtype, int merge_h, int merge_w, void* stream) {
    if (!branch || !x_new) return MTLORA_ERR_NULL;
    return ln_multi_fwd_impl(n, res, gamma, beta, y, mean, rstd, M, C, eps, x_dtype, y_dtype, merge_h, merge_w, branch, x_new,
                             scale, B, stream);
}

static int ln_multi_bwd_impl(int n, const void* const* dy, const void* const* x, const float* gamma, const float* const* mean,
                             const float* const* rstd, void* const* dx, float* dgamma, float* dbeta, int64_t M, int64_t C,
                             int x_dtype, int dy_dtype, void* scratch, int64_t scratch_bytes, const void* const* dx_addend,
                             int merge_h, int merge_w, void* const* d_branch, const float* scale, int64_t B, void* stream) {
    int st = ln_check(M, C, x_dtype, dy_dtype);
    if (d_branch && (B <= 0 || M % B)) return MTLORA_ERR_SHAPE;
    if (st != MTLORA_OK) return st;
    if (n < 1 || n > MTLORA_MAX_TASKS + 1) return MTLORA_ERR_SHAPE;
    if (!dy || !x || !gamma || !mean || !rstd || !dx || !dgamma || !dbeta || !scratch) return MTLORA_ERR_NULL;
    if ((uintptr_t)scratch & 15u) return MTLORA_ERR_ALIGN;
    if (scratch_bytes < mtlora_layernorm_multi_bwd_scratch_bytes(n, M, C, x_dtype) - 256) return MTLORA_ERR_WORKSPACE;
    hipStream_t s = (hipStream_t)stream;
    if (M == 0) {
        mtl_zero_async(dgamma, (size_t)C * 4, s);
        mtl_zero_async(dbeta, (size_t)C * 4, s);
        return MTLORA_OK;
    }
    LnParams p = {};
    for (int k = 0; k < n; ++k) {
        if (!dy[k] || !x[k] || !mean[k] || !rstd[k] || !dx[k]) return MTLORA_ERR_NULL;
        const void* ad = dx_addend ? dx_addend[k] : nullptr;
        if (((uintptr_t)dy[k] | (uintptr_t)x[k] | (uintptr_t)dx[k] | (uintptr_t)ad) & 15u) return MTLORA_ERR_ALIGN;
        p.dy_k[k] = dy[k];
        p.x_k[k] = x[k];
        p.dx_k[k] = dx[k];
        p.add_k[k] = ad;
        p.mean_k[k] = const_cast<float*>(mean[k]);
        p.rstd_k[k] = const_cast<float*>(rstd[k]);
        if (d_branch) {
            if ((uintptr_t)d_branch[k] & 15u) return MTLORA_ERR_ALIGN;
            p.dbr_k[k] = d_branch[k];
        }
    }
    p.multi_x = 1;
    p.x = x[0];
    p.dy = dy[0];
    p.dx = dx[0];
    p.gamma = gamma;
    p.mean = const_cast<float*>(mean[0]);
    p.rstd = const_cast<float*>(rstd[0]);
    p.part = reinterpret_cast<float*>(scratch);
    p.M = M;
    p.C = (int)C;
    p.rscale = d_branch ? scale : nullptr;
    p.rows_per_sample = d_branch ? M / B : 1;
    st = ln_merge(p, M, C, x_dtype, merge_h, merge_w);
    if (st != MTLORA_OK) return st;
    const int nvec_h = (int)(C / (x_dtype == MTLORA_F32 ? 4 : 8));
    const int lpr = pick_lpr(nvec_h);
    const int vpl = (nvec_h + lpr - 1) / lpr;
    const int gx = ln_grid(M, lpr);
    const dim3 grid((unsigned)gx, (unsigned)n);
    const size_t lds = (size_t)4 * (64 / lpr) * 2 * C * 4;
    const int es_x = mtl_elem_size(x_dtype), es_g = mtl_elem_size(dy_dtype);
    {
        mtl_prof_tag("M%lld C%lld x%d g%d mg%d n%d", (long long)M, (long long)C, x_dtype, dy_dtype, merge_w, n);
        MtlProfScope prof(PK_LN_BWD, (double)n * M * C * (2 * es_x + es_g + (dx_addend ? es_x : 0)), s);
#define LN_EXTRA
        if (x_dtype == MTLORA_F32 && dy_dtype == MTLORA_F32) {
            LN_DISPATCH_LPR(k_ln_bwd, float, float)
        } else if (x_dtype == MTLORA_F16 || dy_dtype == MTLORA_F16) {
            if (x_dtype == MTLORA_F32) {
                LN_DISPATCH_LPR(k_ln_bwd, float, f16)
            } else if (dy_dtype == MTLORA_F32) {
                LN_DISPATCH_LPR(k_ln_bwd, f16, float)
            } else {
                LN_DISPATCH_LPR(k_ln_bwd, f16, f16)
            }
        } else if (x_dtype == MTLORA_F32) {
            LN_DISPATCH_LPR(k_ln_bwd, float, bf16)
        } else if (dy_dtype == MTLORA_F32) {
            LN_DISPATCH_LPR(k_ln_bwd, bf16, float)
        } else {
            LN_DISPATCH_LPR(k_ln_bwd, bf16, bf16)
        }
#undef LN_EXTRA
    }
    hipLaunchKernelGGL(k_ln_reduce, dim3((unsigned)mtl_ceil_div(2 * C, 64)), dim3(64 * LN_RW), 0, s, (const float*)p.part, dgamma,
                       dbeta, gx * n, (int)C);
    MTL_CHECK_LAUNCH();
    return MTLORA_OK;
}

int mtlora_layernorm_multi_bwd(int n, const void* const* dy, const void* const* x, const float* gamma, const float* const* mean,
                               const float* const* rstd, void* const* dx, float* dgamma, float* dbeta, int64_t M, int64_t C,
                               int x_dtype, int dy_dtype, void* scratch, int64_t scratch_bytes, const void* const* dx_addend,
                               int merge_h, int merge_w, void* stream) {
    return ln_multi_bwd_impl(n, dy, x, gamma, mean, rstd, dx, dgamma, dbeta, M, C, x_dtype, dy_dtype, scratch, scratch_bytes,
                             dx_addend, merge_h, merge_w, nullptr, nullptr, 1, stream);
}

int mtlora_residual_layernorm_streams_bwd(int n, const void* const* dy, const void* const* x_new, const float* gamma,
                                          const float* const* mean, const float* const* rstd, void* const* d_res,
                                          void* const* d_branch, float* dgamma, float* dbeta, const float* scale, int64_t B,
                                          int64_t M, int64_t C, int x_dtype, int dy_dtype, void* scratch, int64_t scratch_bytes,
                                          const void* const* dx_addend, int merge_h, int merge_w, void* stream) {
    if (!d_branch) return MTLORA_ERR_NULL;
    return ln_multi_bwd_impl(n, dy, x_new, gamma, mean, rstd, d_res, dgamma, dbeta, M, C, x_dtype, dy_dtype, scratch,
                             scratch_bytes, dx_addend, merge_h, merge_w, d_branch, scale, B, stream);
}

int mtlora_residual_layernorm_multi_fwd(int n, const void* shortcut, const void* const* branch, const float* scale, int64_t B,
                                        const float* gamma, const float* beta, void* const* x_new, void* const* y,
                                        float* const* mean, float* const* rstd, int64_t M, int64_t C, float eps, int x_dtype,
                                        int y_dtype, void* stream) {
    int st = ln_check(M, C, x_dtype, y_dtype);
    if (st != MTLORA_OK) return st;
    if (n < 1 || n > MTLORA_MAX_TASKS + 1 || B <= 0 || M % B) return MTLORA_ERR_SHAPE;
    if (!shortcut || !branch || !gamma || !beta || !x_new || !y || !mean || !rstd) return MTLORA_ERR_NULL;
    if ((uintptr_t)shortcut & 15u) return MTLORA_ERR_ALIGN;
    LnParams p = {};
    for (int k = 0; k < n; ++k) {
        if (!branch[k] || !x_new[k] || !y[k] || !mean[k] || !rstd[k]) return MTLORA_ERR_NULL;
        if (((uintptr_t)branch[k] | (uintptr_t)x_new[k] | (uintptr_t)y[k]) & 15u) return MTLORA_ERR_ALIGN;
        p.rb_k[k] = branch[k];
        p.xsum_k[k] = x_new[k];
        p.y_k[k] = y[k];
        p.mean_k[k] = mean[k];
        p.rstd_k[k] = rstd[k];
    }
    if (M == 0) return MTLORA_OK;
    p.nk = n;
    p.x = shortcut;
    p.gamma = gamma;
    p.beta = beta;
    p.rb = branch[0];
    p.xsum = x_new[0];
    p.y = y[0];
    p.mean = mean[0];
    p.rstd = rstd[0];
    p.rscale = scale;
    p.rows_per_sample = M / B;
    p.M = M;
    p.C = (int)C;
    p.eps = eps;
    const int nvec_h = (int)(C / (x_dtype == MTLORA_F32 ? 4 : 8));
    const int lpr = pick_lpr(nvec_h);
    const int vpl = (nvec_h + lpr - 1) / lpr;
    const int gx = (int)mtl_ceil_div(ln_grid(M, lpr, 1 << 30), vpl <= 3 ? 4 : 1) < 256 * 8
                       ? (int)mtl_ceil_div(ln_grid(M, lpr, 1 << 30), vpl <= 3 ? 4 : 1)
                       : 256 * 8;
    const dim3 grid((unsigned)gx, (unsigned)n);
    const size_t lds = 0;
    hipStream_t s = (hipStream_t)stream;
    const int es_x = mtl_elem_size(x_dtype), es_y = mtl_elem_size(y_dtype);
    mtl_prof_tag("M%lld C%lld x%d y%d n%d", (long long)M, (long long)C, x_dtype, y_dtype, n);
    MtlProfScope prof(PK_LN_FWD, (double)M * C * (es_x + (double)n * (es_x + 2 * es_y)), s);
#define LN_EXTRA , true
    if (x_dtype == MTLORA_F32 && y_dtype == MTLORA_F32) {
        LN_DISPATCH_LPR(k_ln_fwd, float, float)
    } else if (x_dtype == MTLORA_F16 || y_dtype == MTLORA_F16) {
        if (x_dtype == MTLORA_F32) {
            LN_DISPATCH_LPR(k_ln_fwd, float, f16)
        } else if (y_dtype == MTLORA_F32) {
            LN_DISPATCH_LPR(k_ln_fwd, f16, float)
        } else {
            LN_DISPATCH_LPR(k_ln_fwd, f16, f16)
        }
    } else if (x_dtype == MTLORA_F32) {
        LN_DISPATCH_LPR(k_ln_fwd, float, bf16)
    } else if (y_dtype == MTLORA_F32) {
        LN_DISPATCH_LPR(k_ln_fwd, bf16, float)
    } else {
        LN_DISPATCH_LPR(k_ln_fwd, bf16, bf16)
    }
#undef LN_EXTRA
    MTL_CHECK_LAUNCH();
    return MTLORA_OK;
}

int mtlora_residual_layernorm_multi_bwd(int n, const void* const* dy, const void* const* x_new, const float* gamma,
                                        const float* const* mean, const float* const* rstd, const void* const* dx_addend,
                                        void* d_shortcut, void* const* d_branch, float* dgamma, float* dbeta, const float* scale,
                                        int64_t B, int64_t M, int64_t C, int x_dtype, int dy_dtype, void* scratch,
                                        int64_t scratch_bytes, void* stream) {
    int st = ln_check(M, C, x_dtype, dy_dtype);
    if (st != MTLORA_OK) return st;
    if (n < 1 || n > MTLORA_MAX_TASKS + 1 || B <= 0 || M % B) return MTLORA_ERR_SHAPE;
    if (!dy || !x_new || !gamma || !mean || !rstd || !d_shortcut || !dgamma || !dbeta || !scratch) return MTLORA_ERR_NULL;
    if (((uintptr_t)d_shortcut | (uintptr_t)scratch) & 15u) return MTLORA_ERR_ALIGN;
    if (scratch_bytes < mtlora_layernorm_bwd_scratch_bytes(M, C, x_dtype) - 256) return MTLORA_ERR_WORKSPACE;
    hipStream_t s = (hipStream_t)stream;
    if (M == 0) {
        mtl_zero_async(dgamma, (size_t)C * 4, s);
        mtl_zero_async(dbeta, (size_t)C * 4, s);
        return MTLORA_OK;
    }
    LnParams p = {};
    for (int k = 0; k < n; ++k) {
        if (!dy[k] || !x_new[k] || !mean[k] || !rstd[k]) return MTLORA_ERR_NULL;
        const void* ad = dx_addend ? dx_addend[k] : nullptr;
        void* db = d_branch ? d_branch[k] : nullptr;
        if (((uintptr_t)dy[k] | (uintptr_t)x_new[k] | (uintptr_t)ad | (uintptr_t)db) & 15u) return MTLORA_ERR_ALIGN;
        p.dy_k[k] = dy[k];
        p.xsum_k[k] = const_cast<void*>(x_new[k]);
        p.mean_k[k] = const_cast<float*>(mean[k]);
        p.rstd_k[k] = const_cast<float*>(rstd[k]);
        p.add_k[k] = ad;
        p.dbr_k[k] = db;
    }
    p.nk = n;
    p.gamma = gamma;
    p.dx = d_shortcut;
    p.rscale = scale;
    p.rows_per_sample = M / B;
    p.part = reinterpret_cast<float*>(scratch);
    p.M = M;
    p.C = (int)C;
    const int nvec_h = (int)(C / (x_dtype == MTLORA_F32 ? 4 : 8));
    const int lpr = pick_lpr(nvec_h);
    const int vpl = (nvec_h + lpr - 1) / lpr;
    const int grid = ln_grid(M, lpr);
    const size_t lds = (size_t)4 * (64 / lpr) * 2 * C * 4;
    const int es_x = mtl_elem_size(x_dtype), es_g = mtl_elem_size(dy_dtype);
    {
        mtl_prof_tag("M%lld C%lld x%d g%d n%d", (long long)M, (long long)C, x_dtype, dy_dtype, n);
        MtlProfScope prof(PK_LN_BWD, (double)M * C * (es_x + (double)n * (2 * es_x + 2 * es_g)), s);
#define LN_EXTRA
        if (x_dtype == MTLORA_F32 && dy_dtype == MTLORA_F32) {
            LN_DISPATCH_LPR(k_resln_bwd_multi, float, float)
        } else if (x_dtype == MTLORA_F16 || dy_dtype == MTLORA_F16) {
            if (x_dtype == MTLORA_F32) {
                LN_DISPATCH_LPR(k_resln_bwd_multi, float, f16)
            } else if (dy_dtype == MTLORA_F32) {
                LN_DISPATCH_LPR(k_resln_bwd_multi, f16, float)
            } else {
                LN_DISPATCH_LPR(k_resln_bwd_multi, f16, f16)
            }
        } else if (x_dtype == MTLORA_F32) {
            LN_DISPATCH_LPR(k_resln_bwd_multi, float, bf16)
        } else if (dy_dtype == MTLORA_F32) {
            LN_DISPATCH_LPR(k_resln_bwd_multi, bf16, float)
        } else {
            LN_DISPATCH_LPR(k_resln_bwd_multi, bf16, bf16)
        }
#undef LN_EXTRA
    }
    hipLaunchKernelGGL(k_ln_reduce, dim3((unsigned)mtl_ceil_div(2 * C, 64)), dim3(64 * LN_RW), 0, s, (const float*)p.part, dgamma,
                       dbeta, grid, (int)C);
    MTL_CHECK_LAUNCH();
    return MTLORA_OK;
}
}

namespace {

struct BnParams {
    const void* x;
    const void* dy;
    void* y;
    void* dx;
    const float* gamma;
    const float* beta;
    float* running_mean;
    float* running_var;
    float* mean;
    float* rstd;
    float* scale;
    float* shift;
    float* part;
    float* dgamma;
    float* dbeta;
    float* c1;
    float* c2;
    int64_t R;
    int C, VW, rows_per_iter, nblk, relu;
    float momentum, eps;
};

template <typename T, bool BWD>
__global__ __launch_bounds__(512) void k_bn_colsum(const BnParams p) {
    constexpr int VE = ET<T>::VEC;
    extern __shared__ __attribute__((aligned(16))) float sm[];
    const int tid = threadIdx.x;
    const int ro = tid / p.VW, v = tid % p.VW;
    const bool active = ro < p.rows_per_iter;
    const T* x = reinterpret_cast<const T*>(p.x);
    const T* dy = reinterpret_cast<const T*>(p.dy);
    float a0[VE], a1[VE], sc[VE], sh[VE], mu[VE], rs[VE];
#pragma unroll
    for (int e = 0; e < VE; ++e) {
        a0[e] = a1[e] = 0.f;
        if (BWD && active) {
            sc[e] = p.scale[v * VE + e];
            sh[e] = p.shift[v * VE + e];
            mu[e] = p.mean[v * VE + e];
            rs[e] = p.rstd[v * VE + e];
        }
    }
    const int64_t rows_blk = mtl_ceil_div(p.R, p.nblk);
    const int64_t r_lo = (int64_t)blockIdx.x * rows_blk;
    int64_t r_hi = r_lo + rows_blk;
    if (r_hi > p.R) r_hi = p.R;
    if (active) {
        constexpr int UN = 4;
        for (int64_t r = r_lo + ro; r < r_hi; r += (int64_t)UN * p.rows_per_iter) {
            u32x4 rx[UN], rg[UN];
#pragma unroll
            for (int u = 0; u < UN; ++u) {
                const int64_t rr = r + (int64_t)u * p.rows_per_iter;
                const bool ok = rr < r_hi;
                rx[u] = ok ? *reinterpret_cast<const u32x4*>(x + rr * p.C + v * VE) : u32x4{0u, 0u, 0u, 0u};
                if (BWD) rg[u] = ok ? *reinterpret_cast<const u32x4*>(dy + rr * p.C + v * VE) : u32x4{0u, 0u, 0u, 0u};
            }
#pragma unroll
            for (int u = 0; u < UN; ++u) {
                float fx[8];
                cvt_vec<T>(rx[u], fx);
                if (!BWD) {
#pragma unroll
                    for (int e = 0; e < VE; ++e) {
                        a0[e] += fx[e];
                        a1[e] += fx[e] * fx[e];
                    }
                } else {
                    float fg[8];
                    cvt_vec<T>(rg[u], fg);
#pragma unroll
                    for (int e = 0; e < VE; ++e) {
                        const float yv = fx[e] * sc[e] + sh[e];
                        const float g = (p.relu && yv <= 0.f) ? 0.f : fg[e];
                        a0[e] += g;
                        a1[e] += g * (fx[e] - mu[e]) * rs[e];
                    }
                }
            }
        }
        float* mine = sm + (size_t)ro * 2 * p.C;
#pragma unroll
        for (int e = 0; e < VE; ++e) {
            mine[v * VE + e] = a0[e];
            mine[p.C + v * VE + e] = a1[e];
        }
    }
    __syncthreads();
    float* dst = p.part + (int64_t)blockIdx.x * 2 * p.C;
    for (int i = tid; i < 2 * p.C; i += blockDim.x) {
        float t = 0.f;
        for (int g = 0; g < p.rows_per_iter; ++g) t += sm[(size_t)g * 2 * p.C + i];
        dst[i] = t;
    }
}

constexpr int BN_FW = 16;
__global__ __launch_bounds__(64 * BN_FW) void k_bn_finalize(const BnParams p) {
    __shared__ double sm[BN_FW][2][64];
    const int lane = threadIdx.x & 63, wave = threadIdx.x >> 6;
    const int c = blockIdx.x * 64 + lane;
    double s0 = 0.0, q0 = 0.0, s1 = 0.0, q1 = 0.0;
    if (c < p.C) {
        int b = wave;
        for (; b + BN_FW < p.nblk; b += 2 * BN_FW) {
            s0 += p.part[(int64_t)b * 2 * p.C + c];
            q0 += p.part[(int64_t)b * 2 * p.C + p.C + c];
            s1 += p.part[(int64_t)(b + BN_FW) * 2 * p.C + c];
            q1 += p.part[(int64_t)(b + BN_FW) * 2 * p.C + p.C + c];
        }
        for (; b < p.nblk; b += BN_FW) {
            s0 += p.part[(int64_t)b * 2 * p.C + c];
            q0 += p.part[(int64_t)b * 2 * p.C + p.C + c];
        }
    }
    sm[wave][0][lane] = s0 + s1;
    sm[wave][1][lane] = q0 + q1;
    __syncthreads();
    if (wave != 0 || c >= p.C) return;
    double S = 0.0, Q = 0.0;
    for (int w = 0; w < BN_FW; ++w) {
        S += sm[w][0][lane];
        Q += sm[w][1][lane];
    }
    const double n = (double)p.R, mean = S / n;
    double m2 = Q - S * mean;
    m2 = m2 < 0.0 ? 0.0 : m2;
    const double var = m2 / n;
    const float rstd = (float)(1.0 / sqrt(var + (double)p.eps));
    const float sc = p.gamma[c] * rstd;
    p.mean[c] = (float)mean;
    p.rstd[c] = rstd;
    p.scale[c] = sc;
    p.shift[c] = p.beta[c] - (float)mean * sc;
    if (p.running_mean) {
        const double unb = n > 1.0 ? m2 / (n - 1.0) : var;
        p.running_mean[c] = (1.f - p.momentum) * p.running_mean[c] + p.momentum * (float)mean;
        p.running_var[c] = (1.f - p.momentum) * p.running_var[c] + p.momentum * (float)unb;
    }
}

__global__ __launch_bounds__(64 * BN_FW) void k_bn_bwd_finalize(const BnParams p) {
    __shared__ double sm[BN_FW][2][64];
    const int lane = threadIdx.x & 63, wave = threadIdx.x >> 6;
    const int c = blockIdx.x * 64 + lane;
    double s0 = 0.0, s1 = 0.0, t0 = 0.0, t1 = 0.0;
    if (c < p.C) {
// ... 405 lines not shown
```

mtlora_amd/functional.py:

```python
from __future__ import annotations

import ctypes
import os
from dataclasses import dataclass, field
from typing import List, Optional, Sequence, Tuple

import torch

from . import _lib as L

_seed_counter = 0


_seed_offset: Optional[torch.Tensor] = None


def set_seed_offset(t: Optional[torch.Tensor]) -> None:
    global _seed_offset
    if t is not None and not (t.is_cuda and t.dtype == torch.int64 and t.numel() == 1):
        raise RuntimeError("mtlora_amd: the seed offset must be a CUDA int64 tensor with one element")
    _seed_offset = t


_factor_stream: Optional["torch.cuda.Stream"] = None
# ... 918 lines not shown
    outs = ResidualLayerNormMultiFn.apply(scale, mod.weight, mod.bias, mod.eps, out_dtype, n, shortcut, *branches)
    return list(outs[:n]), list(outs[n:])


def residual_layer_norm(mod: torch.nn.Module, shortcut: torch.Tensor, branch: torch.Tensor, drop_prob: float, training: bool):
    C = shortcut.shape[-1]
    ok = (type(mod) is torch.nn.LayerNorm and mod.elementwise_affine and mod.bias is not None
          and len(mod.normalized_shape) == 1 and shortcut.is_cuda and shortcut.dtype in _GLUE_DTYPES
          and C % 8 == 0 and C <= (2048 if shortcut.dtype == torch.float32 else 4096) and branch.shape == shortcut.shape
          and shortcut.dim() == 3 and torch.is_grad_enabled() and (shortcut.requires_grad or branch.requires_grad))
    if ok:
        out_dtype = glue_dtype(shortcut)
        ok = branch.dtype == out_dtype
    if not ok:
        x = residual_droppath(shortcut, [branch], drop_prob, training)[0]
        return layer_norm_fork(mod, x)
    scale = None
    if training and drop_prob > 0.0:
        keep = 1.0 - drop_prob
        scale = droppath_scale(1, shortcut.shape[0], keep, shortcut.device)[0]
    return ResidualLayerNormFn.apply(shortcut, branch, scale, mod.weight, mod.bias, mod.eps, out_dtype)


def layer_norm_fork(mod: torch.nn.Module, x: torch.Tensor):
    y = layer_norm(mod, x, _fork=True)
    return y if isinstance(y, tuple) else (x, y)


def layer_norm_merge(mod: torch.nn.Module, x: torch.Tensor, H: int, W: int) -> torch.Tensor:
    B, Lt, C = x.shape
    ve = 4 if x.dtype == torch.float32 else 8
    ok = (type(mod) is torch.nn.LayerNorm and mod.elementwise_affine and mod.bias is not None and x.is_cuda
          and x.dtype in _GLUE_DTYPES and C % ve == 0 and Lt == H * W and H % 2 == 0 and W % 2 == 0
          and 4 * C <= (2048 if x.dtype == torch.float32 else 4096))
    if not ok:
        g = x.view(B, H // 2, 2, W // 2, 2, C).permute(0, 1, 3, 4, 2, 5).reshape(B, (H // 2) * (W // 2), 4 * C)
        return layer_norm(mod, g)
    return LayerNormFn.apply(x, mod.weight, mod.bias, mod.eps, glue_dtype(x), (H, W))


class LayerNormMergeMultiFn(torch.autograd.Function):

    @staticmethod
    def forward(ctx, weight, bias, eps: float, out_dtype: torch.dtype, H: int, W: int, n: int, *xs):
        L.require_gpu(weight, bias, *xs)
        B, Lt, Ct = xs[0].shape
        C, M = 4 * Ct, B * Lt // 4
        x2 = [x.contiguous() for x in xs]
        w, b = weight.detach().float().contiguous(), bias.detach().float().contiguous()
        y = torch.empty((n, M, C), dtype=out_dtype, device=x2[0].device)
        stats = torch.empty((2 * n, M), dtype=torch.float32, device=x2[0].device)
        means, rstds = [stats[k] for k in range(n)], [stats[n + k] for k in range(n)]
        st = L.lib().mtlora_layernorm_multi_fwd(n, L.ptr_array9(x2), L.ptr(w), L.ptr(b), L.ptr_array9([y[k] for k in range(n)]),
                                                L.ptr_array9(means), L.ptr_array9(rstds), M, C, float(eps), L.dtype_code(x2[0]),
                                                L.dtype_code(y), H, W, L.stream_ptr())
        L.check(st, "mtlora_layernorm_multi_fwd")
        ctx.save_for_backward(w, stats, *x2)
        ctx.cfg = (n, M, C, H, W, xs[0].shape)
        return y.view(n * B, Lt // 4, C)

    @staticmethod
    def backward(ctx, g):
        w, stats, *x2 = ctx.saved_tensors
        n, M, C, H, W, shape = ctx.cfg
        g3 = g.reshape(n, M, C)
        if g3.dtype not in _GLUE_DTYPES:
            g3 = g3.float()
        g3 = g3.contiguous()
        dev = x2[0].device
        lib = L.lib()
        sb = lib.mtlora_layernorm_multi_bwd_scratch_bytes(n, M, C, L.dtype_code(x2[0]))
        scratch = torch.empty(sb, dtype=torch.uint8, device=dev)
        dxs = [torch.empty_like(x) for x in x2]
        dg = torch.empty(C, dtype=torch.float32, device=dev)
        db = torch.empty(C, dtype=torch.float32, device=dev)
        means, rstds = [stats[k] for k in range(n)], [stats[n + k] for k in range(n)]
        st = lib.mtlora_layernorm_multi_bwd(n, L.ptr_array9([g3[k] for k in range(n)]), L.ptr_array9(x2), L.ptr(w),
                                            L.ptr_array9(means), L.ptr_array9(rstds), L.ptr_array9(dxs), L.ptr(dg), L.ptr(db), M, C,
                                            L.dtype_code(x2[0]), L.dtype_code(g3), L.ptr(scratch), sb, L.ptr_array9(None), H, W,
                                            L.stream_ptr())
        L.check(st, "mtlora_layernorm_multi_bwd")
        return (dg, db, None, None, None, None, None, *[d.view(shape) for d in dxs])


class ResidualMergeNormStreamsFn(torch.autograd.Function):

    @staticmethod
    def forward(ctx, scale, weight, bias, eps: float, out_dtype: torch.dtype, H: int, W: int, n: int, *tensors):
        res, brs = tensors[:n], tensors[n:]
        L.require_gpu(weight, bias, *tensors)
        B, Lt, Ct = res[0].shape
        C, M = 4 * Ct, B * Lt // 4
        r2 = [x.contiguous() for x in res]
        b2 = [x.contiguous() for x in brs]
        w, b = weight.detach().float().contiguous(), bias.detach().float().contiguous()
        xs = [torch.empty_like(x) for x in r2]
        y = torch.empty((n, M, C), dtype=out_dtype, device=r2[0].device)
        stats = torch.empty((2 * n, M), dtype=torch.float32, device=r2[0].device)
        means, rstds = [stats[k] for k in range(n)], [stats[n + k] for k in range(n)]
        st = L.lib().mtlora_residual_layernorm_streams_fwd(n, L.ptr_array9(r2), L.ptr_array9(b2), L.ptr(scale), B, L.ptr(w), L.ptr(b),
                                                           L.ptr_array9(xs), L.ptr_array9([y[k] for k in range(n)]),
                                                           L.ptr_array9(means), L.ptr_array9(rstds), M, C, float(eps),
                                                           L.dtype_code(r2[0]), L.dtype_code(y), H, W, L.stream_ptr())
        L.check(st, "mtlora_residual_layernorm_streams_fwd")
        ctx.save_for_backward(w, stats, scale, *xs)
        ctx.cfg = (n, M, C, H, W, B, res[0].shape, brs[0].dtype)
        return y.view(n * B, Lt // 4, C)

    @staticmethod
    def backward(ctx, g):
        w, stats, scale, *xs = ctx.saved_tensors
        n, M, C, H, W, B, shape, bdt = ctx.cfg
        g3 = g.reshape(n, M, C)
        if g3.dtype != bdt:
            g3 = g3.to(bdt)
        g3 = g3.contiguous()
        dev = xs[0].device
        lib = L.lib()
        sb = lib.mtlora_layernorm_multi_bwd_scratch_bytes(n, M, C, L.dtype_code(xs[0]))
        scratch = torch.empty(sb, dtype=torch.uint8, device=dev)
        dres = [torch.empty_like(x) for x in xs]
        dbr = [torch.empty(shape, dtype=bdt, device=dev) for _ in range(n)]
        dg = torch.empty(C, dtype=torch.float32, device=dev)
        db = torch.empty(C, dtype=torch.float32, device=dev)
        means, rstds = [stats[k] for k in range(n)], [stats[n + k] for k in range(n)]
        st = lib.mtlora_residual_layernorm_streams_bwd(n, L.ptr_array9([g3[k] for k in range(n)]), L.ptr_array9(xs), L.ptr(w),
                                                       L.ptr_array9(means), L.ptr_array9(rstds), L.ptr_array9(dres),
                                                       L.ptr_array9(dbr), L.ptr(dg), L.ptr(db), L.ptr(scale), B, M, C,
                                                       L.dtype_code(xs[0]), L.dtype_code(g3), L.ptr(scratch), sb, L.ptr_array9(None),
                                                       H, W, L.stream_ptr())
        L.check(st, "mtlora_residual_layernorm_streams_bwd")
        return (None, dg, db, None, None, None, None, None, *[d.view(shape) for d in dres], *dbr)


def residual_merge_norm_streams(mod: torch.nn.Module, res, branches, H: int, W: int, drop_prob: float, training: bool):
    n = len(res)
    B, Lt, C = res[0].shape
    ve = 4 if res[0].dtype == torch.float32 else 8
    ok = (type(mod) is torch.nn.LayerNorm and mod.elementwise_affine and mod.bias is not None and 2 <= n <= L.MAX_TASKS + 1
          and len(branches) == n and all(x.is_cuda and x.dtype == res[0].dtype and x.shape == res[0].shape for x in res)
          and all(x.shape == res[0].shape and x.dtype == branches[0].dtype for x in branches)
          and res[0].dtype in _GLUE_DTYPES and C % ve == 0 and Lt == H * W and H % 2 == 0 and W % 2 == 0
          and 4 * C <= (2048 if res[0].dtype == torch.float32 else 4096) and torch.is_grad_enabled())
    if ok:
        out_dtype = glue_dtype(res[0])
        ok = branches[0].dtype == out_dtype
    if not ok:
        return None
    scale = None
    if training and drop_prob > 0.0:
        keep = 1.0 - drop_prob
        scale = droppath_scale(n, B, keep, res[0].device)
    return ResidualMergeNormStreamsFn.apply(scale, mod.weight, mod.bias, mod.eps, out_dtype, H, W, n, *res, *branches)


def layer_norm_merge_multi(mod: torch.nn.Module, xs, H: int, W: int):
    B, Lt, C = xs[0].shape
    ve = 4 if xs[0].dtype == torch.float32 else 8
    ok = (type(mod) is torch.nn.LayerNorm and mod.elementwise_affine and mod.bias is not None and 2 <= len(xs) <= L.MAX_TASKS + 1
          and all(x.is_cuda and x.dtype == xs[0].dtype and x.shape == xs[0].shape for x in xs)
          and xs[0].dtype in _GLUE_DTYPES and C % ve == 0 and Lt == H * W and H % 2 == 0 and W % 2 == 0
          and 4 * C <= (2048 if xs[0].dtype == torch.float32 else 4096))
    if not ok:
        return None
    return LayerNormMergeMultiFn.apply(mod.weight, mod.bias, mod.eps, glue_dtype(xs[0]), H, W, len(xs), *xs)


def layer_norm(mod: torch.nn.Module, x: torch.Tensor, feeds_linear: bool = True, _fork: bool = False):
    ok = (type(mod) is torch.nn.LayerNorm and mod.elementwise_affine and mod.bias is not None
          and len(mod.normalized_shape) == 1 and x.is_cuda and x.dtype in _GLUE_DTYPES
          and x.shape[-1] % 8 == 0 and x.shape[-1] <= (2048 if x.dtype == torch.float32 else 4096))
    if not ok:
        return mod(x)
    if feeds_linear:
        out_dtype = glue_dtype(x)
    else:
        out_dtype = torch.float32 if torch.is_autocast_enabled() else x.dtype
    if _fork and x.requires_grad:
        return LayerNormForkFn.apply(x, mod.weight, mod.bias, mod.eps, out_dtype)
    return LayerNormFn.apply(x, mod.weight, mod.bias, mod.eps, out_dtype)


class BatchNormReluFn(torch.autograd.Function):
    @staticmethod
    def forward(ctx, x, weight, bias, running_mean, running_var, momentum: float, eps: float, relu: bool):
        L.require_gpu(x, weight, bias)
        R, C = x.shape
        x = x.contiguous()
        w, b = weight.detach().float().contiguous(), bias.detach().float().contiguous()
        y = torch.empty_like(x)
        saves = torch.empty(4, C, dtype=torch.float32, device=x.device)
        lib = L.lib()
        sb = lib.mtlora_bn_scratch_bytes(R, C, L.dtype_code(x))
        if sb < 0:
            raise RuntimeError(f"mtlora_amd: unsupported BatchNorm shape ({R}, {C}) {x.dtype}")
        scratch = torch.empty(sb, dtype=torch.uint8, device=x.device)
        st = lib.mtlora_bn_relu_fwd(L.ptr(x), L.ptr(w), L.ptr(b), L.ptr(running_mean), L.ptr(running_var), float(momentum),
                                    float(eps), int(relu), L.ptr(y), L.ptr(saves[0]), L.ptr(saves[1]), L.ptr(saves[2]),
                                    L.ptr(saves[3]), R, C, L.dtype_code(x), L.ptr(scratch), sb, L.stream_ptr())
        L.check(st, "mtlora_bn_relu_fwd")
        ctx.save_for_backward(x, saves)
        ctx.relu = relu
        return y

    @staticmethod
    def backward(ctx, dy):
        x, saves = ctx.saved_tensors
        R, C = x.shape
        dy = dy.to(x.dtype).contiguous()
        lib = L.lib()
        sb = lib.mtlora_bn_scratch_bytes(R, C, L.dtype_code(x))
        scratch = torch.empty(sb, dtype=torch.uint8, device=x.device)
        dx = torch.empty_like(x)
        dg = torch.empty(C, dtype=torch.float32, device=x.device)
        db = torch.empty(C, dtype=torch.float32, device=x.device)
        st = lib.mtlora_bn_relu_bwd(L.ptr(dy), L.ptr(x), L.ptr(saves[0]), L.ptr(saves[1]), L.ptr(saves[2]), L.ptr(saves[3]),
                                    int(ctx.relu), L.ptr(dx), L.ptr(dg), L.ptr(db), R, C, L.dtype_code(x), L.ptr(scratch), sb,
                                    L.stream_ptr())
        L.check(st, "mtlora_bn_relu_bwd")
        return dx, dg, db, None, None, None, None, None


class ResidualDropPathFn(torch.autograd.Function):

    @staticmethod
    def forward(ctx, scale, shared: bool, n: int, *tensors):
        nres = 1 if shared else n
        res, ys = list(tensors[:nres]), list(tensors[nres:nres + n])
        L.require_gpu(*res, *ys)
        B = res[0].shape[0]
        C = res[0].shape[-1]
        M = res[0].numel() // C
        res_c = [r.contiguous() for r in res]
        ys_c = [y.contiguous() for y in ys]
        outs = [torch.empty_like(res_c[0]) for _ in range(n)]
        rlist = res_c * n if shared else res_c
        st = L.lib().mtlora_residual_droppath_fwd(n, L.ptr_array9(rlist), L.ptr_array9(ys_c), L.ptr_array9(outs), L.ptr(scale),
                                                  M, C, B, L.dtype_code(res_c[0]), L.dtype_code(ys_c[0]), L.stream_ptr())
        L.check(st, "mtlora_residual_droppath_fwd")
        ctx.cfg = (shared, n, M, C, B, res_c[0].dtype, ys_c[0].dtype, res_c[0].shape)
        ctx.save_for_backward(scale)
        ctx.set_materialize_grads(False)
        return tuple(outs)

    @staticmethod
    def backward(ctx, *grads):
        shared, n, M, C, B, rdt, ydt, shape = ctx.cfg
        (scale,) = ctx.saved_tensors
        if all(g is None for g in grads):
            return (None,) * (3 + (1 if shared else n) + n)
        dev = next(g for g in grads if g is not None).device
        gs = [None if g is None else g.to(rdt).contiguous() for g in grads]
        dys = [None if g is None else torch.empty(shape, dtype=ydt, device=dev) for g in gs]
        dres = torch.empty(shape, dtype=rdt, device=dev) if shared else None
        st = L.lib().mtlora_residual_droppath_bwd(n, L.ptr_array9(gs), L.ptr_array9(dys), L.ptr(dres), L.ptr(scale), M, C, B,
                                                  L.dtype_code(gs[[g is not None for g in gs].index(True)]),
                                                  _DT_CODE.get(ydt, L.F32), L.stream_ptr())
        L.check(st, "mtlora_residual_droppath_bwd")
        dres_out = [dres] if shared else gs
        return (None, None, None, *dres_out, *dys)


def residual_droppath(res, ys, drop_prob: float, training: bool):
    shared = not isinstance(res, (list, tuple))
    rl = [res] if shared else list(res)
    n = len(ys)
    ok = (rl[0].is_cuda and rl[0].shape[-1] % 8 == 0 and all(t.dtype in _GLUE_DTYPES for t in rl + list(ys))
          and len({t.dtype for t in rl}) == 1 and len({t.dtype for t in ys}) == 1 and n <= L.MAX_TASKS + 1
          and all(t.shape == rl[0].shape for t in list(ys) + rl))
    scale = None
    if training and drop_prob > 0.0:
        keep = 1.0 - drop_prob
        scale = droppath_scale(n, rl[0].shape[0], keep, rl[0].device)
    if not ok:
        out = []
        for k in range(n):
            y = ys[k] if scale is None else ys[k] * scale[k].view(-1, *([1] * (ys[k].ndim - 1))).to(ys[k].dtype)
            out.append((rl[0] if shared else rl[k]) + y)
        return out
    return list(ResidualDropPathFn.apply(scale, shared, n, *rl, *ys))


def column_sum(g2: torch.Tensor) -> torch.Tensor:
    M, N = g2.shape
    ve = 4 if g2.dtype == torch.float32 else 8
    if g2.dtype not in (torch.float32, torch.bfloat16) or N % ve or not g2.is_contiguous() or M == 0:
        return g2.sum(0, dtype=torch.float32)
    lib = L.lib()
    sb = lib.mtlora_colsum_scratch_bytes(M, N)
    scratch = torch.empty(sb, dtype=torch.uint8, device=g2.device)
    out = torch.empty(N, dtype=torch.float32, device=g2.device)
    L.check(lib.mtlora_colsum(L.ptr(g2), M, N, L.dtype_code(g2), L.ptr(out), L.ptr(scratch), sb, L.stream_ptr()), "mtlora_colsum")
    return out


def label_stat(lab: torch.Tensor, kind: int, ignore_index: float) -> torch.Tensor:
    n = lab.numel()
    lib = L.lib()
    sb = lib.mtlora_label_stat_scratch_bytes(n)
    scratch = torch.empty(sb, dtype=torch.uint8, device=lab.device)
    out = torch.empty(1, dtype=torch.float32, device=lab.device)
    L.check(lib.mtlora_label_stat(L.ptr(lab), n, kind, float(ignore_index), L.ptr(out), L.ptr(scratch), sb, L.stream_ptr()),
            "mtlora_label_stat")
    return out


# ... 632 lines not shown
```

mtlora_amd/swin_transformer_mtlora.py:

```python
from __future__ import annotations

from typing import Dict, Optional

import torch
import torch.nn as nn
from torch import Tensor

import os

from . import functional as Fn
from .lora import MTLoRALinear
from .window_process import WindowProcess, WindowProcessReverse


_FUSED_BLOCKS = os.environ.get("MTLORA_FUSED_BLOCKS", "1") != "0"


def set_fused_blocks(on: bool) -> bool:
    global _FUSED_BLOCKS
    prev, _FUSED_BLOCKS = _FUSED_BLOCKS, bool(on)
    return prev


def to_2tuple(v):
    return tuple(v) if isinstance(v, (tuple, list)) else (v, v)


trunc_normal_ = nn.init.trunc_normal_


class DropPath(nn.Module):

    def __init__(self, drop_prob: float = 0.0, scale_by_keep: bool = True):
        super().__init__()
        self.drop_prob, self.scale_by_keep = drop_prob, scale_by_keep

    def forward(self, x):
        if self.drop_prob == 0.0 or not self.training:
            return x
        keep = 1.0 - self.drop_prob
        m = x.new_empty((x.shape[0],) + (1,) * (x.ndim - 1)).bernoulli_(keep)
        if keep > 0.0 and self.scale_by_keep:
            m.div_(keep)
        return x * m

    def extra_repr(self):
        return f"drop_prob={self.drop_prob:.3f}"


class CompatLinear(nn.Linear):

    def forward(self, input: Tensor, x_tasks: dict = None):
        if input.is_cuda and self.weight.requires_grad:
            sh = input.shape
            y = Fn.linear_big_m(input.reshape(-1, sh[-1]), self.weight, self.bias)
            return y.view(*sh[:-1], y.shape[-1]), None
        return super().forward(input), None


def _mtlora_linear(mtlora, layer_idx, fin, fout, tasks, **kw):
    return MTLoRALinear(fin, fout, r=mtlora.R_PER_TASK_LIST[layer_idx], lora_shared_scale=mtlora.SHARED_SCALE[layer_idx],
                        lora_task_scale=mtlora.SCALE_PER_TASK_LIST[layer_idx], lora_dropout=mtlora.DROPOUT[layer_idx],
                        tasks=tasks, trainable_scale_shared=mtlora.TRAINABLE_SCALE_SHARED,
                        trainable_scale_per_task=mtlora.TRAINABLE_SCALE_PER_TASK, shared_mode=mtlora.SHARED_MODE, **kw)


class Mlp(nn.Module):
    def __init__(self, in_features, hidden_features=None, out_features=None, act_layer=nn.GELU, drop=0.0, lora=False,
                 tasks=None, mtlora=None, layer_idx=0):
        super().__init__()
        out_features = out_features or in_features
        hidden_features = hidden_features or in_features
        t = tasks if (lora or mtlora.INTERMEDIATE_SPECIALIZATION) else None
        self.fc1 = (_mtlora_linear(mtlora, layer_idx, in_features, hidden_features, t) if mtlora.FC1_ENABLED
                    else CompatLinear(in_features, hidden_features))
        self.act = act_layer()
        self.fc2 = (_mtlora_linear(mtlora, layer_idx, hidden_features, out_features, t) if mtlora.FC2_ENABLED
                    else CompatLinear(hidden_features, out_features))
        self.tasks = tasks
        self.drop = nn.Dropout(drop)

    def _fused_gelu_backward(self, h, h_t) -> bool:
        from .lora import MTLoRALinear
        ts = [h] + ([h_t[t] for t in self.tasks] if h_t is not None else [])
        return (isinstance(self.fc2, MTLoRALinear) and type(self.act) is nn.GELU and getattr(self.act, "approximate", "none") == "none"
                and (self.drop.p == 0.0 or not self.training) and torch.is_grad_enabled() and h.requires_grad
                and all(t.is_cuda and t.is_contiguous() and t.dtype == Fn.compute_dtype(t) for t in ts)
                and self.fc2.linear.in_features % 8 == 0 and not self.fc2.linear.weight.requires_grad
                and self.fc2.shared_mode in ("matrix", "matrixv2"))

    def _fused_gelu(self, x) -> bool:
        from .lora import MTLoRALinear
        ok = lambda m: (isinstance(m, MTLoRALinear) and m.shared_mode in ("matrix", "matrixv2") and not m.linear.weight.requires_grad
                        and m.linear.in_features % 8 == 0 and m.linear.out_features % 8 == 0)
        return (ok(self.fc1) and ok(self.fc2) and type(self.act) is nn.GELU and getattr(self.act, "approximate", "none") == "none"
                and (self.drop.p == 0.0 or not self.training) and torch.is_grad_enabled() and x.is_cuda and x.requires_grad
                and self.fc1.tasks == self.fc2.tasks)

    def _hid_forward(self, x, x_tasks):
        tasks = self.tasks
        if not (Fn.mlp_hid_enabled() and x_tasks is not None and tasks and self.fc1.tasks is not None
                and list(self.fc1.tasks) == list(tasks) and list(self.fc2.tasks) == list(tasks)
                and self.fc1.linear.out_features == self.fc2.linear.in_features and all(t in x_tasks for t in tasks)):
            return None
        dtype = Fn.compute_dtype(x)
        if dtype not in (torch.bfloat16, torch.float16) or x.shape[-1] != self.fc1.linear.in_features:
            return None
        xt = [x_tasks[t] for t in tasks]
        if (not x.is_cuda) or any(v.device != x.device or v.shape != x.shape for v in xt):
            return None
        H, r1, r2 = self.fc1.linear.out_features, self.fc1._ranks, self.fc2._ranks
        if H % 128 or any(not (1 <= r1.get(t, 0) <= 8 and 1 <= r2.get(t, 0) <= 8) for t in tasks):
            return None
        c1 = self.fc1.hid_call(dtype, x.device)
        c2 = self.fc2.hid_call(dtype, x.device) if c1 is not None else None
        if c1 is None or c2 is None:
            return None
        (m1, (W1c, W1t, b1), f1), (m2, (W2c, W2t, b2), f2) = c1, c2
        M = x.numel() // m1.K
        if not Fn.mlp_hid_supported(m1, m2, M):
            return None
        outs = Fn.MlpHidFn.apply(m1, m2, x, W1c, W1t, b1, W2c, W2t, b2, f1[0], f1[1], f2[0], f2[1], *xt, *f1[2], *f1[3], *f2[2], *f2[3])
        return outs[0], {t: outs[1 + i] for i, t in enumerate(tasks)}

    def forward(self, x, x_tasks=None):
        if x_tasks is not None and self._fused_gelu(x):
            out = self._hid_forward(x, x_tasks)
            if out is not None:
                return out
        if self._fused_gelu(x):
            h, h_t, a, a_t = self.fc1(x, x_tasks, gelu_out=True)
            return self.fc2(a, a_t, gelu_gate=(h.detach(), None if h_t is None else {t: v.detach() for t, v in h_t.items()}))
        h, h_t = self.fc1(x, x_tasks)
        if self._fused_gelu_backward(h, h_t):
            a = Fn.GeluDeferredGradFn.apply(h)
            a_t = {t: Fn.GeluDeferredGradFn.apply(h_t[t]) for t in self.tasks} if h_t is not None else None
            return self.fc2(a, a_t, gelu_gate=(h, h_t))
        h = self.drop(self.act(h))
        if h_t is not None:
            h_t = {t: self.drop(self.act(h_t[t])) for t in self.tasks}
        y, y_t = self.fc2(h, h_t)
        y = self.drop(y)
        if y_t is not None:
            y_t = {t: self.drop(y_t[t]) for t in self.tasks}
        return y, y_t


def window_partition(x, window_size):
    B, H, W, C = x.shape
    x = x.view(B, H // window_size, window_size, W // window_size, window_size, C)
    return x.permute(0, 1, 3, 2, 4, 5).contiguous().view(-1, window_size, window_size, C)


def window_reverse(windows, window_size, H, W):
    B = int(windows.shape[0] / (H * W / window_size / window_size))
    x = windows.view(B, H // window_size, W // window_size, window_size, window_size, -1)
    return x.permute(0, 1, 3, 2, 4, 5).contiguous().view(B, H, W, -1)


def _relative_position_index(wh: int, ww: int) -> Tensor:
    ys, xs = torch.meshgrid(torch.arange(wh), torch.arange(ww), indexing="ij")
    pos = torch.stack([ys.reshape(-1), xs.reshape(-1)])
    rel = pos[:, :, None] - pos[:, None, :]
    return (rel[0] + wh - 1) * (2 * ww - 1) + (rel[1] + ww - 1)


class WindowAttention(nn.Module):

    def __init__(self, dim, window_size, num_heads, qkv_bias=True, qk_scale=None, attn_drop=0.0, proj_drop=0.0,
                 lora=False, tasks=None, mtlora=None, layer_idx=0):
        super().__init__()
        self.dim = dim
        self.window_size = window_size
        self.num_heads = num_heads
# ... 34 lines not shown
                                      "(every MTLoRA config uses 0)")
        return Fn.WindowAttentionFn.apply(meta, qkv, self.dense_bias(), mask, mask_ids)

    def _project(self, a: Tensor):
        y, y_t = self.proj(a)
        y = self.proj_drop(y)
        if y_t is not None:
            y_t = {t: self.proj_drop(y_t[t]) for t in self.tasks}
        return y, y_t

    def forward(self, x, mask=None):
        B_, N, C = x.shape
        qkv, _ = self.qkv(x)
        nW = 1 if mask is None else mask.shape[0]
        ws = self.window_size[0]
        meta = Fn.AttnMeta(B=B_ // nW, H=ws, W=ws * nW, window_size=ws, shift=0, num_heads=self.num_heads,
                           head_dim=C // self.num_heads, image_layout=False, scale=self.scale)
        return self._project(self._core(qkv, meta, mask, None))

    def forward_image(self, x, H: int, W: int, shift: int, mask=None, mask_ids=None):
        B, L, C = x.shape
        qkv, _ = self.qkv(x)
        meta = Fn.AttnMeta(B=B, H=H, W=W, window_size=self.window_size[0], shift=shift, num_heads=self.num_heads,
                           head_dim=C // self.num_heads, image_layout=True, scale=self.scale)
        return self._project(self._core(qkv, meta, mask, mask_ids))

    def extra_repr(self) -> str:
        return f"dim={self.dim}, window_size={self.window_size}, num_heads={self.num_heads}"

    def flops(self, N):
        return 4 * N * self.dim * self.dim + 2 * self.num_heads * N * N * (self.dim // self.num_heads)


def _shift_regions(H: int, W: int, ws: int, shift: int) -> Tensor:
    ids = torch.zeros(H, W)
    edges_h = (0, H - ws, H - shift, H)
    edges_w = (0, W - ws, W - shift, W)
    for a in range(3):
        for b in range(3):
            ids[edges_h[a]:edges_h[a + 1], edges_w[b]:edges_w[b + 1]] = 3 * a + b
    return ids.view(H // ws, ws, W // ws, ws).permute(0, 2, 1, 3).reshape(-1, ws * ws)


def _shift_mask(H: int, W: int, ws: int, shift: int) -> Tensor:
    win = _shift_regions(H, W, ws, shift)
    diff = win[:, None, :] - win[:, :, None]
    return torch.where(diff != 0, torch.full_like(diff, -100.0), torch.zeros_like(diff))


class SwinTransformerBlock(nn.Module):
    def __init__(self, dim, input_resolution, num_heads, window_size=7, shift_size=0, mlp_ratio=4.0, qkv_bias=True,
                 qk_scale=None, drop=0.0, attn_drop=0.0, drop_path=0.0, act_layer=nn.GELU, norm_layer=nn.LayerNorm,
                 fused_window_process=False, lora=False, tasks=None, mtlora=None, layer_idx=0):
        super().__init__()
        self.dim = dim
        self.input_resolution = input_resolution
        self.num_heads = num_heads
        self.window_size = window_size
        self.shift_size = shift_size
        self.mlp_ratio = mlp_ratio
        self.tasks = tasks
        self.lora = lora
        if min(self.input_resolution) <= self.window_size:
            self.shift_size = 0
            self.window_size = min(self.input_resolution)
        assert 0 <= self.shift_size < self.window_size, "shift_size must in 0-window_size"
        self.norm1 = norm_layer(dim)
        self.attn = WindowAttention(dim, window_size=to_2tuple(self.window_size), num_heads=num_heads,
                                    qkv_bias=qkv_bias, qk_scale=qk_scale, attn_drop=attn_drop, proj_drop=drop, lora=lora,
                                    tasks=tasks, mtlora=mtlora, layer_idx=layer_idx)
        self.drop_path = DropPath(drop_path) if drop_path > 0.0 else nn.Identity()
        self.norm2 = norm_layer(dim)
        self.mlp = Mlp(in_features=dim, hidden_features=int(dim * mlp_ratio), act_layer=act_layer, drop=drop, lora=lora,
                       tasks=tasks, mtlora=mtlora, layer_idx=layer_idx)
        H, W = self.input_resolution
        mask = _shift_mask(H, W, self.window_size, self.shift_size) if self.shift_size > 0 else None
        self.register_buffer("attn_mask", mask)
        self.register_buffer("_attn_mask_ids", None if mask is None else
                             _shift_regions(H, W, self.window_size, self.shift_size).to(torch.int32), persistent=False)
        self.fused_window_process = fused_window_process
        self.attention_layout = "image"

    def _fusable_static(self, next_norm) -> bool:
        def plain_ln(m):
            return type(m) is nn.LayerNorm and m.elementwise_affine and m.bias is not None and len(m.normalized_shape) == 1

        def stock_linear(m):
            return isinstance(m, MTLoRALinear) and m.r > 0 and m.tasks is None and hasattr(m, "lora_shared_A") and m.shared_mode == "matrix"

        lin = (self.attn.qkv, self.attn.proj, self.mlp.fc1, self.mlp.fc2)
        C = self.dim
        return (not self.lora and next_norm is not None
                and all(stock_linear(m) for m in lin) and all(plain_ln(m) for m in (self.norm1, self.norm2, next_norm))
                and type(self.mlp.act) is nn.GELU and getattr(self.mlp.act, "approximate", "none") == "none"
                and all(isinstance(d, nn.Dropout) for d in (self.mlp.drop, self.attn.proj_drop, self.attn.attn_drop))
                and C % 8 == 0 and self.mlp.fc1.linear.out_features % 8 == 0
                and C // self.num_heads == 32 and self.window_size * self.window_size <= 64)

    def _block_call(self, has_norm1: bool, next_norm, cdtype, x):
        lin = (self.attn.qkv, self.attn.proj, self.mlp.fc1, self.mlp.fc2)
        dev = x.device
        if self.attention_layout != "image" or self.mlp.drop.p != 0.0 or self.attn.proj_drop.p != 0.0 or self.attn.attn_drop.p != 0.0:
            return None
        for m in (self, self.attn, self.mlp, self.norm1, self.norm2, next_norm, self.mlp.act, self.drop_path) + lin:
            if m._forward_hooks or m._forward_pre_hooks or m._backward_hooks or m._backward_pre_hooks:
                return None
        for n in (self.norm1, self.norm2, next_norm):
            for t in (n.weight, n.bias):
                if t.dtype != torch.float32 or t.device != dev or not t.is_contiguous():
                    return None
        for m in lin:
            if (m.merged or isinstance(m.lora_shared_scale, torch.Tensor) or m.rank_aware_shared() or m.linear.weight.requires_grad
                    or (m.linear.bias is not None and m.linear.bias.requires_grad)):
                return None
            for t in (m.lora_shared_A, m.lora_shared_B):
                if t.dtype != torch.float32 or t.device != dev or not t.is_contiguous():
                    return None
            if m.linear.weight.device != dev:
                return None
        tab = self.attn.relative_position_bias_table
        if tab.device != dev or (self._attn_mask_ids is not None and (self._attn_mask_ids.device != dev or self._attn_mask_ids.dtype != torch.int32
                                                                      or not self._attn_mask_ids.is_contiguous())):
            return None
        metas, weights, fparams = [], [], []
        for m in lin:
            metas.append(m.meta_t0(cdtype, dev))
            weights.append(m._weights(cdtype))
            fparams += [m.lora_shared_A, m.lora_shared_B]
        p_dp = self.drop_path.drop_prob if isinstance(self.drop_path, DropPath) else 0.0
        s1 = s2 = None
        if self.training and p_dp > 0.0:
            keep = 1.0 - p_dp
            s1 = Fn.droppath_scale(1, x.shape[0], keep, x.device)[0]
            s2 = Fn.droppath_scale(1, x.shape[0], keep, x.device)[0]
        H, W = self.input_resolution
        call = Fn.BlockCall(has_norm1, metas, weights, self.attn_mask, self._attn_mask_ids, H, W, self.num_heads, self.window_size,
                            self.shift_size, self.mlp.fc1.linear.out_features, (self.norm1.eps, self.norm2.eps, next_norm.eps),
                            self.attn.scale, tuple(fparams))
        flat = [self.attn.dense_bias(), s1, s2]
        if has_norm1:
            flat += [self.norm1.weight, self.norm1.bias]
        flat += [self.norm2.weight, self.norm2.bias, next_norm.weight, next_norm.bias]
        call.norm_params = tuple(flat[3:])
        flat += fparams
        return call, flat

    def _attend_windows(self, xn: Tensor, B: int, H: int, W: int, C: int):
        ws, s = self.window_size, self.shift_size
        xw = WindowProcess.apply(xn.view(B, H, W, C).contiguous(), B, H, W, C, -s, ws).view(-1, ws * ws, C)
        a, a_t = self.attn(xw, mask=self.attn_mask)
        merge = lambda v: WindowProcessReverse.apply(v.reshape(-1, ws, ws, C).contiguous(), B, H, W, C, s, ws).view(B, H * W, C)
        return merge(a), None if a_t is None else {t: merge(a_t[t]) for t in self.tasks}

    def forward(self, x, normed=None, next_norm=None, defer_residual=False):
        H, W = self.input_resolution
        B, L, C = x.shape
        assert L == H * W, "input feature has wrong size"
        if normed is None:
            shortcut, xn = Fn.layer_norm_fork(self.norm1, x)
        else:
            shortcut, xn = x, normed
        if self.attention_layout == "windows":
            a, a_t = self._attend_windows(xn, B, H, W, C)
        else:
            a, a_t = self.attn.forward_image(xn, H, W, self.shift_size, self.attn_mask, self._attn_mask_ids)
        p_dp = self.drop_path.drop_prob if isinstance(self.drop_path, DropPath) else 0.0
        x_t = None
        xn2_t = None
        if a_t is not None:
            xs, xns = Fn.residual_layer_norm_multi(self.norm2, shortcut, [a] + [a_t[t] for t in self.tasks], p_dp, self.training)
            x, xn2 = xs[0], xns[0]
            x_t = {t: xs[1 + i] for i, t in enumerate(self.tasks)}
            xn2_t = {t: xns[1 + i] for i, t in enumerate(self.tasks)}
        else:
            x, xn2 = Fn.residual_layer_norm(self.norm2, shortcut, a, p_dp, self.training)
        m, m_t = self.mlp(xn2, xn2_t)
        if m_t is None:
            if next_norm is not None:
                x, nxt = Fn.residual_layer_norm(next_norm, x, m, p_dp, self.training)
                return x, None, nxt
            return Fn.residual_droppath(x, [m], p_dp, self.training)[0], None
        if x_t is None:
            out = Fn.residual_droppath(x, [m], p_dp, self.training)[0]
            return out, {t: self.drop_path(m_t[t]) for t in self.tasks}
        if defer_residual:
            return None, None, None, ([x] + [x_t[t] for t in self.tasks], [m] + [m_t[t] for t in self.tasks], p_dp)
        r = Fn.residual_droppath([x] + [x_t[t] for t in self.tasks], [m] + [m_t[t] for t in self.tasks], p_dp, self.training)
        return r[0], {t: r[1 + i] for i, t in enumerate(self.tasks)}

    def extra_repr(self) -> str:
        return (f"dim={self.dim}, input_resolution={self.input_resolution}, num_heads={self.num_heads}, "
                f"window_size={self.window_size}, shift_size={self.shift_size}, mlp_ratio={self.mlp_ratio}")

    def flops(self):
        H, W = self.input_resolution
        nW = H * W / self.window_size / self.window_size
        return (2 * self.dim * H * W + nW * self.attn.flops(self.window_size * self.window_size)
                + 2 * H * W * self.dim * self.dim * self.mlp_ratio)


class PatchMerging(nn.Module):

    def __init__(self, input_resolution, dim, norm_layer=nn.LayerNorm, layer_idx=0, mtlora=None):
        super().__init__()
        self.input_resolution = input_resolution
        self.dim = dim
        self.reduction = (_mtlora_linear(mtlora, layer_idx, 4 * dim, 2 * dim, None, bias=False)
                          if mtlora.DOWNSAMPLER_ENABLED else CompatLinear(4 * dim, 2 * dim, bias=False))
        self.norm = norm_layer(4 * dim)

    def forward(self, x):
        H, W = self.input_resolution
        B, L, C = x.shape
        assert L == H * W, "input feature has wrong size"
        assert H % 2 == 0 and W % 2 == 0, f"x size ({H}*{W}) are not even."
        y, _ = self.reduction(Fn.layer_norm_merge(self.norm, x, H, W))
        return y

    def forward_residual_multi(self, res, branches, drop_prob, training):
        H, W = self.input_resolution
        stacked = Fn.residual_merge_norm_streams(self.norm, res, branches, H, W, drop_prob, training)
        if stacked is None:
            return self.forward_multi(Fn.residual_droppath(list(res), list(branches), drop_prob, training))
        y, _ = self.reduction(stacked)
        return list(y.view(len(res), -1, *y.shape[1:]).unbind(0))

    def forward_multi(self, xs):
        H, W = self.input_resolution
        stacked = Fn.layer_norm_merge_multi(self.norm, xs, H, W) if len(xs) > 1 else None
        if stacked is None:
            return [self.forward(x) for x in xs]
        y, _ = self.reduction(stacked)
        return list(y.view(len(xs), -1, *y.shape[1:]).unbind(0))

    def extra_repr(self) -> str:
        return f"input_resolution={self.input_resolution}, dim={self.dim}"

    def flops(self):
        H, W = self.input_resolution
        return H * W * self.dim + (H // 2) * (W // 2) * 4 * self.dim * 2 * self.dim


class BasicLayer(nn.Module):

    def __init__(self, dim, input_resolution, depth, num_heads, window_size, mlp_ratio=4.0, qkv_bias=True, qk_scale=None,
                 drop=0.0, attn_drop=0.0, drop_path=0.0, norm_layer=nn.LayerNorm, downsample=None, use_checkpoint=False,
                 fused_window_process=False, tasks=None, mtlora=None, layer_idx=0):
        super().__init__()
        self.dim = dim
        self.input_resolution = input_resolution
        self.depth = depth
        self.use_checkpoint = use_checkpoint
        self.tasks = tasks
        self.blocks = nn.ModuleList([
            SwinTransformerBlock(dim=dim, input_resolution=input_resolution, num_heads=num_heads, window_size=window_size,
                                 shift_size=0 if i % 2 == 0 else window_size // 2, mlp_ratio=mlp_ratio,
                                 qkv_bias=qkv_bias, qk_scale=qk_scale, drop=drop, attn_drop=attn_drop,
                                 drop_path=drop_path[i] if isinstance(drop_path, list) else drop_path,
                                 norm_layer=norm_layer, fused_window_process=fused_window_process,
                                 lora=(i == depth - 1), tasks=tasks, mtlora=mtlora, layer_idx=layer_idx)
            for i in range(depth)])
        self.downsample = (downsample(input_resolution, dim=dim, norm_layer=norm_layer, layer_idx=layer_idx, mtlora=mtlora)
                           if downsample is not None else None)

    def _fused_run(self, x):
        ok = (_FUSED_BLOCKS and x.is_cuda and x.dim() == 3 and x.is_contiguous() and torch.is_grad_enabled() and x.dtype in Fn._GLUE_DTYPES)
        if not ok:
            return 0, x, None
        cdtype = Fn.compute_dtype(x)
        C = x.shape[-1]
        if C > (2048 if x.dtype == torch.float32 else 4096) or (x.dtype != torch.float32 and x.dtype != cdtype):
            return 0, x, None
        st = self.__dict__.get("_fusable_cache")
        if st is None:
            st = [blk._fusable_static(self.blocks[i + 1].norm1 if i + 1 < len(self.blocks) else None) for i, blk in enumerate(self.blocks)]
            self.__dict__["_fusable_cache"] = st
        calls, flat = [], []
        for i, blk in enumerate(self.blocks):
            if not st[i] or blk.training != self.training:
                break
            cf = blk._block_call(i == 0, self.blocks[i + 1].norm1, cdtype, x)
            if cf is None:
                break
            calls.append(cf[0])
            flat += cf[1]
        if not calls:
            return 0, x, None
        x, normed = Fn.SwinBlockRunFn.apply(calls, x, None, *flat)
        return len(calls), x, normed

    def _apply(self, fn, *a, **k):
        self.__dict__.pop("_fusable_cache", None)
        return super()._apply(fn, *a, **k)

    def invalidate_fused_cache(self) -> None:
        self.__dict__.pop("_fusable_cache", None)

    def forward(self, x):
        tasks_lora = None
        deferred = None
        first, x, normed = self._fused_run(x)
        for i, blk in enumerate(self.blocks):
            if i < first:
                continue
            nxt = self.blocks[i + 1].norm1 if (i + 1 < len(self.blocks) and not blk.lora) else None
            last = i + 1 == len(self.blocks)
            defer = (last and blk.lora and self.downsample is not None and hasattr(self.downsample, "forward_residual_multi")
                     and self.training and torch.is_grad_enabled())
            out = blk(x, normed, nxt, defer) if defer else blk(x, normed, nxt)
            x, tasks_lora = out[0], out[1]
            normed = out[2] if len(out) > 2 else None
            deferred = out[3] if len(out) > 3 else None
        if deferred is not None:
            outs = self.downsample.forward_residual_multi(deferred[0], deferred[1], deferred[2], self.training)
            return outs[0], {t: outs[1 + i] for i, t in enumerate(self.tasks)}
        if self.downsample is not None:
            if tasks_lora is not None and hasattr(self.downsample, "forward_multi"):
                outs = self.downsample.forward_multi([x] + [tasks_lora[t] for t in self.tasks])
                x, tasks_lora = outs[0], {t: outs[1 + i] for i, t in enumerate(self.tasks)}
            else:
                x = self.downsample(x)
                if tasks_lora is not None:
                    tasks_lora = {t: self.downsample(tasks_lora[t]) for t in self.tasks}
        return x, tasks_lora

    def extra_repr(self) -> str:
        return f"dim={self.dim}, input_resolution={self.input_resolution}, depth={self.depth}"

    def flops(self):
        return sum(b.flops() for b in self.blocks) + (self.downsample.flops() if self.downsample is not None else 0)


class PatchEmbed(nn.Module):
    def __init__(self, img_size=224, patch_size=4, in_chans=3, embed_dim=96, norm_layer=None):
        super().__init__()
        img_size, patch_size = to_2tuple(img_size), to_2tuple(patch_size)
        self.img_size = img_size
        self.patch_size = patch_size
        self.patches_resolution = [img_size[0] // patch_size[0], img_size[1] // patch_size[1]]
        self.num_patches = self.patches_resolution[0] * self.patches_resolution[1]
        self.in_chans = in_chans
        self.embed_dim = embed_dim
        self.proj = nn.Conv2d(in_chans, embed_dim, kernel_size=patch_size, stride=patch_size)
        self.norm = norm_layer(embed_dim) if norm_layer is not None else None

    def forward(self, x):
        B, C, H, W = x.shape
        assert H == self.img_size[0] and W == self.img_size[1], \
            f"Input image size ({H}*{W}) doesn't match model ({self.img_size[0]}*{self.img_size[1]})."
        ph, pw = self.patch_size
        p = x.view(B, C, H // ph, ph, W // pw, pw).permute(0, 2, 4, 1, 3, 5).reshape(B, -1, C * ph * pw)
        sh = p.shape
        x = Fn.linear_big_m(p.reshape(-1, sh[-1]), self.proj.weight.view(self.embed_dim, -1), self.proj.bias)
        x = x.view(*sh[:-1], self.embed_dim)
        return x if self.norm is None else Fn.layer_norm(self.norm, x, feeds_linear=False)

    def flops(self):
        Ho, Wo = self.patches_resolution
        f = Ho * Wo * self.embed_dim * self.in_chans * (self.patch_size[0] * self.patch_size[1])
        return f + (Ho * Wo * self.embed_dim if self.norm is not None else 0)


class SwinTransformerMTLoRA(nn.Module):

    def __init__(self, img_size=224, patch_size=4, in_chans=3, num_classes=1000, embed_dim=96, depths=[2, 2, 6, 2],
                 num_heads=[3, 6, 12, 24], window_size=7, mlp_ratio=4.0, qkv_bias=True, qk_scale=None, drop_rate=0.0,
                 attn_drop_rate=0.0, drop_path_rate=0.1, norm_layer=nn.LayerNorm, ape=False, patch_norm=True,
                 use_checkpoint=False, fused_window_process=False, basic_layer=BasicLayer, tasks=None, mtlora=None,
                 **kwargs):
        super().__init__()
        self.num_classes = num_classes
        self.num_layers = len(depths)
        self.embed_dim = embed_dim
        self.ape = ape
        self.patch_norm = patch_norm
        self.num_features = int(embed_dim * 2 ** (self.num_layers - 1))
        self.mlp_ratio = mlp_ratio
        self.tasks = tasks
        self.mtlora = mtlora
        self.patch_embed = PatchEmbed(img_size=img_size, patch_size=patch_size, in_chans=in_chans, embed_dim=embed_dim,
                                      norm_layer=norm_layer if patch_norm else None)
        res = self.patch_embed.patches_resolution
        self.patches_resolution = res
        if ape:
            self.absolute_pos_embed = nn.Parameter(torch.zeros(1, self.patch_embed.num_patches, embed_dim))
            trunc_normal_(self.absolute_pos_embed, std=0.02)
        self.pos_drop = nn.Dropout(p=drop_rate)
        dpr = [v.item() for v in torch.linspace(0, drop_path_rate, sum(depths))]
        self.layers = nn.ModuleList()
        for i in range(self.num_layers):
            self.layers.append(basic_layer(
                dim=int(embed_dim * 2 ** i), input_resolution=(res[0] // 2 ** i, res[1] // 2 ** i), depth=depths[i],
                num_heads=num_heads[i], window_size=window_size, mlp_ratio=mlp_ratio, qkv_bias=qkv_bias,
                qk_scale=qk_scale, drop=drop_rate, attn_drop=attn_drop_rate,
                drop_path=dpr[sum(depths[:i]):sum(depths[:i + 1])], norm_layer=norm_layer,
                downsample=PatchMerging if i < self.num_layers - 1 else None, use_checkpoint=use_checkpoint,
                fused_window_process=fused_window_process, tasks=tasks, mtlora=mtlora, layer_idx=i))
        self.avgpool = nn.AdaptiveAvgPool1d(1)
        self.head = nn.Linear(self.num_features, num_classes) if num_classes > 0 else nn.Identity()
        self.apply(self._init_weights)

    @staticmethod
    def _init_weights(m):
        if isinstance(m, nn.Linear):
            trunc_normal_(m.weight, std=0.02)
            if m.bias is not None:
                nn.init.constant_(m.bias, 0)
        elif isinstance(m, nn.LayerNorm):
            nn.init.constant_(m.bias, 0)
            nn.init.constant_(m.weight, 1.0)

    @torch.jit.ignore
    def no_weight_decay(self):
        return {"absolute_pos_embed"}

    @torch.jit.ignore
    def no_weight_decay_keywords(self):
        return {"relative_position_bias_table"}

    def forward_features(self, x, return_stages=False, flatten_ft=False):
        x = self.patch_embed(x)
        if self.ape:
            x = x + self.absolute_pos_embed
        x = self.pos_drop(x)
        stages = []
        for layer in self.layers:
            x, tasks_lora = layer(x)
            if tasks_lora is None:
                tasks_lora = {t: x for t in self.tasks}
            stages.append((x, tasks_lora))
        if return_stages:
            return stages
        if flatten_ft:
            x = torch.flatten(self.avgpool(x.transpose(1, 2)), 1)
        return x

    def forward(self, x, return_stages=False, flatten_ft=False):
        return self.head(self.forward_features(x, return_stages, flatten_ft))

    def flops(self, images=None, logger=None, detailed=False):
        f = self.patch_embed.flops() + sum(l.flops() for l in self.layers)
        f += self.num_features * self.patches_resolution[0] * self.patches_resolution[1] // (2 ** self.num_layers)
        return f + self.num_features * self.num_classes
```

Before: 1129 images/sec.

## Recompute residual streams implicitly in last-block layernorms instead of storing sums

Adds implicit-residual variants of the multi-stream residual+layernorm forward and backward kernels for the last LoRA block before patch merging. The kernels no longer write the fp32 residual sums. They recompute them from the shared shortcut and the bf16 branch outputs with drop-path scales in both the norm2 and merge-norm stages. This cuts fp32 activation writes and reads and the memory they hold, at the cost of extra branch loads and FMAs in backward. It also adds a sizeable new autograd path gated by an env flag that is on by default.

```diff
diff --git a/include/mtlora_hip.h b/include/mtlora_hip.h
--- a/include/mtlora_hip.h
+++ b/include/mtlora_hip.h
@@ -180,6 +180,23 @@
                                         int64_t B, int64_t M, int64_t C, int x_dtype, int dy_dtype, void* scratch,
                                         int64_t scratch_bytes, void* stream);
 
+int mtlora_residual_layernorm_multi_implicit_bwd(int n, const void* const* dy, const void* shortcut, const void* const* branch,
+                                                 const float* gamma, const float* const* mean, const float* const* rstd,
+                                                 const void* const* dx_addend, void* d_shortcut, void* const* d_branch,
+                                                 float* dgamma, float* dbeta, const float* scale, int64_t B, int64_t M, int64_t C,
+                                                 int x_dtype, int dy_dtype, void* scratch, int64_t scratch_bytes, void* stream);
+int mtlora_residual_layernorm_streams_implicit_fwd(int n, const void* shortcut, const void* const* inner, const float* scale_in,
+                                                   const void* const* branch, const float* scale, int64_t B, const float* gamma,
+                                                   const float* beta, void* const* y, float* const* mean, float* const* rstd,
+                                                   int64_t M, int64_t C, float eps, int x_dtype, int y_dtype, int merge_h,
+                                                   int merge_w, void* stream);
+int mtlora_residual_layernorm_streams_implicit_bwd(int n, const void* const* dy, const void* shortcut, const void* const* inner,
+                                                   const float* scale_in, const void* const* branch, const float* gamma,
+                                                   const float* const* mean, const float* const* rstd, void* const* d_res,
+                                                   void* const* d_branch, float* dgamma, float* dbeta, const float* scale,
+                                                   int64_t B, int64_t M, int64_t C, int x_dtype, int dy_dtype, void* scratch,
+                                                   int64_t scratch_bytes, int merge_h, int merge_w, void* stream);
+
 int64_t mtlora_bn_scratch_bytes(int64_t R, int64_t C, int dtype);
 int mtlora_bn_relu_fwd(const void* x, const float* gamma, const float* beta, float* running_mean, float* running_var,
                        float momentum, float eps, int relu, void* y, float* save_mean, float* save_rstd,
diff --git a/mtlora_amd/_lib.py b/mtlora_amd/_lib.py
--- a/mtlora_amd/_lib.py
+++ b/mtlora_amd/_lib.py
@@ -153,6 +153,19 @@
                                                     POINTER(c_void_p), POINTER(c_void_p), c_void_p, POINTER(c_void_p), c_void_p,
                                                     c_void_p, c_void_p, c_int64, c_int64, c_int64, c_int, c_int, c_void_p, c_int64,
                                                     c_void_p]),
+    "mtlora_residual_layernorm_multi_implicit_bwd": (c_int, [c_int, POINTER(c_void_p), c_void_p, POINTER(c_void_p), c_void_p,
+                                                             POINTER(c_void_p), POINTER(c_void_p), POINTER(c_void_p), c_void_p,
+                                                             POINTER(c_void_p), c_void_p, c_void_p, c_void_p, c_int64, c_int64,
+                                                             c_int64, c_int, c_int, c_void_p, c_int64, c_void_p]),
+    "mtlora_residual_layernorm_streams_implicit_fwd": (c_int, [c_int, c_void_p, POINTER(c_void_p), c_void_p, POINTER(c_void_p),
+                                                               c_void_p, c_int64, c_void_p, c_void_p, POINTER(c_void_p),
+                                                               POINTER(c_void_p), POINTER(c_void_p), c_int64, c_int64, c_float,
+                                                               c_int, c_int, c_int, c_int, c_void_p]),
+    "mtlora_residual_layernorm_streams_implicit_bwd": (c_int, [c_int, POINTER(c_void_p), c_void_p, POINTER(c_void_p), c_void_p,
+                                                               POINTER(c_void_p), c_void_p, POINTER(c_void_p), POINTER(c_void_p),
+                                                               POINTER(c_void_p), POINTER(c_void_p), c_void_p, c_void_p, c_void_p,
+                                                               c_int64, c_int64, c_int64, c_int, c_int, c_void_p, c_int64, c_int,
+                                                               c_int, c_void_p]),
     "mtlora_residual_layernorm_bwd": (c_int, [c_void_p, c_void_p, c_void_p, c_void_p, c_void_p, c_void_p, c_void_p, c_void_p,
                                               c_void_p, c_void_p, c_int64, c_int64, c_int64, c_int, c_int, c_void_p, c_int64,
                                               c_void_p, c_void_p]),
diff --git a/mtlora_amd/csrc/glue.hip b/mtlora_amd/csrc/glue.hip
--- a/mtlora_amd/csrc/glue.hip
+++ b/mtlora_amd/csrc/glue.hip
@@ -40,6 +40,12 @@
     } else {
         *reinterpret_cast<u32x2*>(p) = u32x2{mtl_pack2<T>(f[0], f[1]), mtl_pack2<T>(f[2], f[3])};
     }
+}
+
+template <int N>
+__device__ __forceinline__ void opaque(float (&f)[8]) {
+#pragma unroll
+    for (int e = 0; e < N; ++e) asm volatile("" : "+v"(f[e]));
 }
 
 template <int LPR>
@@ -81,6 +87,8 @@
     int multi_x;
     const void* x_k[MTLORA_MAX_TASKS + 1];
     void* dx_k[MTLORA_MAX_TASKS + 1];
+    const void* rb_in_k[MTLORA_MAX_TASKS + 1];
+    const float* rscale_in;
 };
 typedef const __attribute__((address_space(4))) LnParams* LnKargs;
 
@@ -171,8 +179,9 @@
     }
 }
 
-template <typename TI, typename TO, int LPR, int MAXV, bool RES>
+template <typename TI, typename TO, int LPR, int MAXV, bool RES, int IMPL = 0>
 __global__ __launch_bounds__(256) void k_ln_fwd(const LnParams p) {
+    static_assert(IMPL == 0 || (RES && sizeof(TI) == 4 && sizeof(TO) == 2), "implicit residuals: fp32 stream, 16-bit branches");
     constexpr int VE = ET<TI>::VEC;
     constexpr int RPW = 64 / LPR;
     constexpr int UNR = MAXV <= 3 ? 4 : 1;
@@ -186,10 +195,17 @@
     const void* rb_ptr = p.rb;
     void* xs_ptr = p.xsum;
     const float* rscale = p.rscale;
+    const void* rbi_ptr = nullptr;
+    const float* rscale_in = p.rscale_in;
     if (p.multi_x) {
         LnKargs K = (LnKargs)__builtin_amdgcn_kernarg_segment_ptr();
         const int k = blockIdx.y;
-        x = reinterpret_cast<const TI*>(K->x_k[k]);
+        if constexpr (IMPL == 2) {
+            rbi_ptr = K->rb_in_k[k];
+            if (rscale_in) rscale_in += (int64_t)k * (p.M / p.rows_per_sample);
+        } else {
+            x = reinterpret_cast<const TI*>(K->x_k[k]);
+        }
         y = reinterpret_cast<TO*>(K->y_k[k]);
         mean_out = K->mean_k[k];
         rstd_out = K->rstd_k[k];
@@ -243,14 +259,23 @@
         }
         if constexpr (RES) {
             const TO* rb = reinterpret_cast<const TO*>(rb_ptr);
-            TI* xs = reinterpret_cast<TI*>(xs_ptr);
+            [[maybe_unused]] TI* xs = reinterpret_cast<TI*>(xs_ptr);
             constexpr bool PRE = sizeof(TO) * VE <= 16;
             u32x4 braw[PRE ? UNR : 1][PRE ? MAXV : 1];
             float scv[UNR];
+            u32x2 biraw[IMPL == 2 ? UNR : 1][IMPL == 2 ? MAXV : 1];
+            float sciv[UNR];
 #pragma unroll
             for (int u = 0; u < UNR; ++u) {
                 const bool rok = row[u] < p.M;
                 scv[u] = (rok && rscale) ? rscale[row_div(row[u], p.rows_per_sample, p.M)] : 1.f;
+                if constexpr (IMPL == 2) {
+                    const TO* rbi = reinterpret_cast<const TO*>(rbi_ptr);
+                    sciv[u] = (rok && rscale_in) ? rscale_in[row_div(row[u], p.rows_per_sample, p.M)] : 1.f;
+#pragma unroll
+                    for (int i = 0; i < MAXV; ++i)
+                        biraw[u][i] = (rok && lr + i * LPR < nvec) ? *reinterpret_cast<const u32x2*>(rbi + xbs[u] + coff[i]) : u32x2{0u, 0u};
+                }
                 if constexpr (PRE) {
 #pragma unroll
                     for (int i = 0; i < MAXV; ++i) {
@@ -295,10 +320,26 @@
                             fb[3] = mtl_hi2<TO>(braw[u][i][1]);
                         }
                         cvt_vec<TI>(raw[u][i], fx);
-#pragma unroll
-                        for (int e = 0; e < VE; ++e) fx[e] += sc * fb[e];
+                        if constexpr (IMPL == 2) {
+                            const float sci = sciv[u];
+                            float fi[4];
+                            fi[0] = mtl_lo2<TO>(biraw[u][i][0]);
+                            fi[1] = mtl_hi2<TO>(biraw[u][i][0]);
+                            fi[2] = mtl_lo2<TO>(biraw[u][i][1]);
+                            fi[3] = mtl_hi2<TO>(biraw[u][i][1]);
+#pragma unroll
+                            for (int e = 0; e < VE; ++e) fx[e] = __builtin_fmaf(sci, fi[e], fx[e]);
+                        }
+                        if constexpr (sizeof(TI) == 4 && sizeof(TO) == 2) {
+#pragma unroll
+                            for (int e = 0; e < VE; ++e) fx[e] = __builtin_fmaf(sc, fb[e], fx[e]);
+                            if constexpr (IMPL != 0) opaque<VE>(fx);
+                        } else {
+#pragma unroll
+                            for (int e = 0; e < VE; ++e) fx[e] += sc * fb[e];
+                        }
                         raw[u][i] = pack_vec<TI>(fx);
-                        *reinterpret_cast<u32x4*>(xs + xbs[u] + coff[i]) = raw[u][i];
+                        if constexpr (IMPL == 0) *reinterpret_cast<u32x4*>(xs + xbs[u] + coff[i]) = raw[u][i];
                     }
                 }
             }
@@ -348,8 +389,10 @@
     }
 }
 
-template <typename TX, typename TG, int LPR, int MAXV>
+template <typename TX, typename TG, int LPR, int MAXV, int IMPL = 0>
 __global__ __launch_bounds__(256) void k_ln_bwd(const LnParams p) {
+    static_assert(IMPL == 0 || IMPL == 2, "k_ln_bwd: stored input or the two-branch implicit form");
+    static_assert(IMPL == 0 || (sizeof(TX) == 4 && sizeof(TG) == 2), "implicit residuals: fp32 stream, 16-bit branches");
     constexpr int VE = ET<TX>::VEC;
     constexpr int RPW = 64 / LPR;
     extern __shared__ __attribute__((aligned(16))) float sm[];
@@ -365,10 +408,21 @@
     void* dbr_ptr = p.dbr;
     const float* rscale_in = p.rscale;
     float* part_out = p.part + (int64_t)blockIdx.x * 2 * p.C;
+    [[maybe_unused]] const TG* rbi = nullptr;
+    [[maybe_unused]] const TG* rbo = nullptr;
+    [[maybe_unused]] const float* rscale_inner = p.rscale_in;
+    [[maybe_unused]] const float* rscale_outer = p.rscale;
     if (p.multi_x) {
         LnKargs K = (LnKargs)__builtin_amdgcn_kernarg_segment_ptr();
         const int k = blockIdx.y;
-        x = reinterpret_cast<const TX*>(K->x_k[k]);
+        if constexpr (IMPL == 2) {
+            rbi = reinterpret_cast<const TG*>(K->rb_in_k[k]);
+            rbo = reinterpret_cast<const TG*>(K->rb_k[k]);
+            if (rscale_inner) rscale_inner += (int64_t)k * (p.M / p.rows_per_sample);
+            if (rscale_outer) rscale_outer += (int64_t)k * (p.M / p.rows_per_sample);
+        } else {
+            x = reinterpret_cast<const TX*>(K->x_k[k]);
+        }
         dy = reinterpret_cast<const TG*>(K->dy_k[k]);
         dx = reinterpret_cast<TX*>(K->dx_k[k]);
         addp = reinterpret_cast<const TX*>(K->add_k[k]);
@@ -400,6 +454,8 @@
         uint32_t rg[UNR][MAXV][GW];
         int64_t row[UNR], xb[UNR];
         float mean[UNR], rstd[UNR], scv[UNR];
+        u32x2 rbi_v[IMPL ? UNR : 1][IMPL ? MAXV : 1], rbo_v[IMPL ? UNR : 1][IMPL ? MAXV : 1];
+        [[maybe_unused]] float sci_v[UNR], sco_v[UNR];
 #pragma unroll
         for (int u = 0; u < UNR; ++u) {
             row[u] = r0 + (int64_t)(wave * UNR + u) * RPW + sub;
@@ -408,6 +464,17 @@
             mean[u] = rv ? mean_in[row[u]] : 0.f;
             rstd[u] = rv ? rstd_in[row[u]] : 0.f;
             scv[u] = (rv && dbr_ptr && rscale_in) ? rscale_in[row_div(row[u], p.rows_per_sample, p.M)] : 1.f;
+            if constexpr (IMPL == 2) {
+                const int64_t smp = rv ? row_div(row[u], p.rows_per_sample, p.M) : 0;
+                sci_v[u] = (rv && rscale_inner) ? rscale_inner[smp] : 1.f;
+                sco_v[u] = (rv && rscale_outer) ? rscale_outer[smp] : 1.f;
+#pragma unroll
+                for (int i = 0; i < MAXV; ++i) {
+                    const bool ok = rv && lr + i * LPR < nvec;
+                    rbi_v[u][i] = ok ? *reinterpret_cast<const u32x2*>(rbi + xb[u] + coff[i]) : u32x2{0u, 0u};
+                    rbo_v[u][i] = ok ? *reinterpret_cast<const u32x2*>(rbo + xb[u] + coff[i]) : u32x2{0u, 0u};
+                }
+            }
 #pragma unroll
             for (int i = 0; i < MAXV; ++i) {
                 const int v = lr + i * LPR;
@@ -443,6 +510,23 @@
             for (int i = 0; i < MAXV; ++i) {
                 float fx[8], fg[8];
                 cvt_vec<TX>(rx[u][i], fx);
+                if constexpr (IMPL == 2) {
+                    float fi[4], fo[4];
+                    fi[0] = mtl_lo2<TG>(rbi_v[u][i][0]);
+                    fi[1] = mtl_hi2<TG>(rbi_v[u][i][0]);
+                    fi[2] = mtl_lo2<TG>(rbi_v[u][i][1]);
+                    fi[3] = mtl_hi2<TG>(rbi_v[u][i][1]);
+                    fo[0] = mtl_lo2<TG>(rbo_v[u][i][0]);
+                    fo[1] = mtl_hi2<TG>(rbo_v[u][i][0]);
+                    fo[2] = mtl_lo2<TG>(rbo_v[u][i][1]);
+                    fo[3] = mtl_hi2<TG>(rbo_v[u][i][1]);
+                    const float sci = sci_v[u], sco = sco_v[u];
+#pragma unroll
+                    for (int e = 0; e < VE; ++e) fx[e] = __builtin_fmaf(sci, fi[e], fx[e]);
+#pragma unroll
+                    for (int e = 0; e < VE; ++e) fx[e] = __builtin_fmaf(sco, fo[e], fx[e]);
+                    opaque<VE>(fx);
+                }
                 if constexpr (GW == 4) {
                     cvt_vec<TG>(u32x4{rg[u][i][0], rg[u][i][1], rg[u][i][2], rg[u][i][3]}, fg);
                 } else if constexpr (GW == 2) {
@@ -512,6 +596,9 @@
 
 template <typename TX, typename TG, int LPR, int MAXV>
 __global__ __launch_bounds__(256) void k_resln_bwd_multi(const LnParams p) {
+    constexpr bool CAN_IMPL = sizeof(TX) == 4 && sizeof(TG) == 2 && MAXV <= 3;
+    constexpr int IMPL = CAN_IMPL ? 1 : 0;
+    const bool impl = CAN_IMPL && p.x != nullptr;
     constexpr int VE = ET<TX>::VEC;
     constexpr int RPW = 64 / LPR;
     constexpr int GW = sizeof(TG) == sizeof(TX) ? 4 : (sizeof(TG) == 2 ? 2 : 8);
@@ -535,6 +622,7 @@
     }
     struct Regs {
         u32x4 rx[MAXV], ra[MAXV];
+        u32x2 rb[IMPL ? MAXV : 1];
         uint32_t rg[MAXV][GW];
         float mean, rstd, sc;
     };
@@ -548,8 +636,17 @@
         for (int i = 0; i < MAXV; ++i)
 #pragma unroll
             for (int e = 0; e < VE; ++e) dsum[i][e] = 0.f;
+        u32x4 shx[IMPL ? MAXV : 1];
+        if constexpr (CAN_IMPL) if (impl) {
+            const TX* sh = reinterpret_cast<const TX*>(p.x);
+#pragma unroll
+            for (int i = 0; i < MAXV; ++i) {
+                const int v = lr + i * LPR;
+                shx[i] = (rv && v < nvec) ? *reinterpret_cast<const u32x4*>(sh + rbase + v * VE) : u32x4{0u, 0u, 0u, 0u};
+            }
+        }
         auto load = [&](Regs& R, int k) __attribute__((always_inline)) {
-            const TX* x = reinterpret_cast<const TX*>(K->xsum_k[k]);
+            [[maybe_unused]] const TX* x = reinterpret_cast<const TX*>(K->xsum_k[k]);
             const TG* dy = reinterpret_cast<const TG*>(K->dy_k[k]);
             const TX* addp = reinterpret_cast<const TX*>(K->add_k[k]);
             R.mean = rv ? K->mean_k[k][row] : 0.f;
@@ -560,7 +657,14 @@
                 const int v = lr + i * LPR;
                 const bool ok = rv && v < nvec;
                 const int64_t off = rbase + (v < nvec ? v : 0) * VE;
-                R.rx[i] = ok ? *reinterpret_cast<const u32x4*>(x + off) : u32x4{0u, 0u, 0u, 0u};
+                bool from_mem = true;
+                if constexpr (CAN_IMPL) {
+                    if (impl) {
+                        R.rb[i] = ok ? *reinterpret_cast<const u32x2*>(reinterpret_cast<const TG*>(K->rb_k[k]) + off) : u32x2{0u, 0u};
+                        from_mem = false;
+                    }
+                }
+                if (from_mem) R.rx[i] = ok ? *reinterpret_cast<const u32x4*>(x + off) : u32x4{0u, 0u, 0u, 0u};
                 R.ra[i] = (ok && addp) ? *reinterpret_cast<const u32x4*>(addp + off) : u32x4{0u, 0u, 0u, 0u};
                 const TG* gp = dy + off;
                 if constexpr (GW == 4) {
@@ -584,6 +688,21 @@
         };
         auto compute = [&](Regs& R, int k) __attribute__((always_inline)) {
             TG* dbr = reinterpret_cast<TG*>(K->dbr_k[k]);
+            if constexpr (CAN_IMPL) if (impl) {
+#pragma unroll
+                for (int i = 0; i < MAXV; ++i) {
+                    float fs[8], fb[4];
+                    fb[0] = mtl_lo2<TG>(R.rb[i][0]);
+                    fb[1] = mtl_hi2<TG>(R.rb[i][0]);
+                    fb[2] = mtl_lo2<TG>(R.rb[i][1]);
+                    fb[3] = mtl_hi2<TG>(R.rb[i][1]);
+                    cvt_vec<TX>(shx[i], fs);
+                    const float sc = R.sc;
+#pragma unroll
+                    for (int e = 0; e < VE; ++e) fs[e] = __builtin_fmaf(sc, fb[e], fs[e]);
+                    R.rx[i] = pack_vec<TX>(fs);
+                }
+            }
             float xh[MAXV][VE], gy[MAXV][VE];
             float c1 = 0.f, c2 = 0.f;
 #pragma unroll
@@ -764,6 +883,16 @@
         case 32: LN_LAUNCH(KERNEL, 32, __VA_ARGS__) break; \
         default: LN_LAUNCH(KERNEL, 64, __VA_ARGS__) break; \
     }
+
+#define LN_DISPATCH_IMPLICIT(KERNEL, g_dtype)        \
+    if ((g_dtype) == MTLORA_F16) {                   \
+        LN_DISPATCH_LPR(KERNEL, float, f16)          \
+    } else {                                         \
+        LN_DISPATCH_LPR(KERNEL, float, bf16)         \
+    }
+static int ln_implicit_check(int x_dtype, int g_dtype) {
+    return (x_dtype == MTLORA_F32 && (g_dtype == MTLORA_BF16 || g_dtype == MTLORA_F16)) ? MTLORA_OK : MTLORA_ERR_UNSUPPORTED;
+}
 
 static int ln_fwd_impl(const void* x, const float* gamma, const float* beta, void* y, float* mean, float* rstd, int64_t M,
                        int64_t C, float eps, int x_dtype, int y_dtype, int merge_h, int merge_w, const void* branch,
@@ -969,12 +1098,20 @@
 static int ln_multi_fwd_impl(int n, const void* const* x, const float* gamma, const float* beta, void* const* y,
                              float* const* mean, float* const* rstd, int64_t M, int64_t C, float eps, int x_dtype, int y_dtype,
                              int merge_h, int merge_w, const void* const* branch, void* const* x_new, const float* scale,
-                             int64_t B, void* stream) {
+                             int64_t B, void* stream, const void* shortcut = nullptr, const void* const* inner = nullptr,
+                             const float* scale_in = nullptr) {
+    const bool implicit = shortcut != nullptr;
     int st = ln_check(M, C, x_dtype, y_dtype);
     if (st != MTLORA_OK) return st;
     if (n < 1 || n > MTLORA_MAX_TASKS + 1) return MTLORA_ERR_SHAPE;
     if (!x || !gamma || !beta || !y || !mean || !rstd) return MTLORA_ERR_NULL;
-    if (branch && (!x_new || B <= 0 || M % B)) return MTLORA_ERR_SHAPE;
+    if (branch && ((!x_new && !implicit) || B <= 0 || M % B)) return MTLORA_ERR_SHAPE;
+    if (implicit) {
+        if (!branch || !inner) return MTLORA_ERR_NULL;
+        if ((uintptr_t)shortcut & 15u) return MTLORA_ERR_ALIGN;
+        st = ln_implicit_check(x_dtype, y_dtype);
+        if (st != MTLORA_OK) return st;
+    }
     LnParams p = {};
     for (int k = 0; k < n; ++k) {
         if (!x[k] || !y[k] || !mean[k] || !rstd[k]) return MTLORA_ERR_NULL;
@@ -984,20 +1121,22 @@
         p.mean_k[k] = mean[k];
         p.rstd_k[k] = rstd[k];
         if (branch) {
-            if (!branch[k] || !x_new[k]) return MTLORA_ERR_NULL;
-            if (((uintptr_t)branch[k] | (uintptr_t)x_new[k]) & 15u) return MTLORA_ERR_ALIGN;
+            if (!branch[k] || (!implicit && !x_new[k])) return MTLORA_ERR_NULL;
+            if (((uintptr_t)branch[k] | (uintptr_t)(implicit ? nullptr : x_new[k])) & 15u) return MTLORA_ERR_ALIGN;
             p.rb_k[k] = branch[k];
-            p.xsum_k[k] = x_new[k];
-        }
+            p.xsum_k[k] = implicit ? nullptr : x_new[k];
+        }
+        if (implicit) p.rb_in_k[k] = inner[k];
     }
     if (M == 0) return MTLORA_OK;
     if (branch) {
         p.rb = branch[0];
-        p.xsum = x_new[0];
+        p.xsum = implicit ? nullptr : x_new[0];
         p.rscale = scale;
     }
+    p.rscale_in = scale_in;
     p.multi_x = 1;
-    p.x = x[0];
+    p.x = implicit ? shortcut : x[0];
     p.y = y[0];
     p.mean = mean[0];
     p.rstd = rstd[0];
@@ -1019,9 +1158,15 @@
     const size_t lds = 0;
     hipStream_t s = (hipStream_t)stream;
     const int es_x = mtl_elem_size(x_dtype), es_y = mtl_elem_size(y_dtype);
-    mtl_prof_tag("M%lld C%lld x%d y%d mg%d n%d res%d", (long long)M, (long long)C, x_dtype, y_dtype, merge_w, n, branch ? 1 : 0);
-    MtlProfScope prof(PK_LN_FWD, (double)n * M * C * (es_x + es_y + (branch ? es_x + es_y : 0)), s);
-    if (branch) {
+    mtl_prof_tag("M%lld C%lld x%d y%d mg%d n%d res%d", (long long)M, (long long)C, x_dtype, y_dtype, merge_w, n,
+                 implicit ? 2 : (branch ? 1 : 0));
+    MtlProfScope prof(PK_LN_FWD, implicit ? (double)M * C * (es_x + (double)n * 3 * es_y)
+                                          : (double)n * M * C * (es_x + es_y + (branch ? es_x + es_y : 0)), s);
+    if (implicit) {
+#define LN_EXTRA , true, 2
+        LN_DISPATCH_IMPLICIT(k_ln_fwd, y_dtype)
+#undef LN_EXTRA
+    } else if (branch) {
 #define LN_EXTRA , true
         if (x_dtype == MTLORA_F32 && y_dtype == MTLORA_F32) {
             LN_DISPATCH_LPR(k_ln_fwd, float, float)
@@ -1085,10 +1230,18 @@
 static int ln_multi_bwd_impl(int n, const void* const* dy, const void* const* x, const float* gamma, const float* const* mean,
                              const float* const* rstd, void* const* dx, float* dgamma, float* dbeta, int64_t M, int64_t C,
                              int x_dtype, int dy_dtype, void* scratch, int64_t scratch_bytes, const void* const* dx_addend,
-                             int merge_h, int merge_w, void* const* d_branch, const float* scale, int64_t B, void* stream) {
+                             int merge_h, int merge_w, void* const* d_branch, const float* scale, int64_t B, void* stream,
+                             const void* shortcut = nullptr, const void* const* branch = nullptr, const float* scale_in = nullptr) {
+    const bool implicit = shortcut != nullptr;
     int st = ln_check(M, C, x_dtype, dy_dtype);
     if (d_branch && (B <= 0 || M % B)) return MTLORA_ERR_SHAPE;
     if (st != MTLORA_OK) return st;
+    if (implicit) {
+        if (!branch || !d_branch) return MTLORA_ERR_NULL;
+        if ((uintptr_t)shortcut & 15u) return MTLORA_ERR_ALIGN;
+        st = ln_implicit_check(x_dtype, dy_dtype);
+        if (st != MTLORA_OK) return st;
+    }
     if (n < 1 || n > MTLORA_MAX_TASKS + 1) return MTLORA_ERR_SHAPE;
     if (!dy || !x || !gamma || !mean || !rstd || !dx || !dgamma || !dbeta || !scratch) return MTLORA_ERR_NULL;
     if ((uintptr_t)scratch & 15u) return MTLORA_ERR_ALIGN;
@@ -1114,9 +1267,16 @@
             if ((uintptr_t)d_branch[k] & 15u) return MTLORA_ERR_ALIGN;
             p.dbr_k[k] = d_branch[k];
         }
-    }
+        if (implicit) {
+            if (!branch[k]) return MTLORA_ERR_NULL;
+            if ((uintptr_t)branch[k] & 15u) return MTLORA_ERR_ALIGN;
+            p.rb_in_k[k] = x[k];
+            p.rb_k[k] = branch[k];
+        }
+    }
+    p.rscale_in = scale_in;
     p.multi_x = 1;
-    p.x = x[0];
+    p.x = implicit ? shortcut : x[0];
     p.dy = dy[0];
     p.dx = dx[0];
     p.gamma = gamma;
@@ -1137,8 +1297,14 @@
     const size_t lds = (size_t)4 * (64 / lpr) * 2 * C * 4;
     const int es_x = mtl_elem_size(x_dtype), es_g = mtl_elem_size(dy_dtype);
     {
-        mtl_prof_tag("M%lld C%lld x%d g%d mg%d n%d", (long long)M, (long long)C, x_dtype, dy_dtype, merge_w, n);
-        MtlProfScope prof(PK_LN_BWD, (double)n * M * C * (2 * es_x + es_g + (dx_addend ? es_x : 0)), s);
+        mtl_prof_tag("M%lld C%lld x%d g%d mg%d n%d impl%d", (long long)M, (long long)C, x_dtype, dy_dtype, merge_w, n, implicit ? 2 : 0);
+        MtlProfScope prof(PK_LN_BWD, implicit ? (double)M * C * (es_x + (double)n * (es_x + 4 * es_g + (dx_addend ? es_x : 0)))
+                                              : (double)n * M * C * (2 * es_x + es_g + (dx_addend ? es_x : 0)), s);
+        if (implicit) {
+#define LN_EXTRA , 2
+            LN_DISPATCH_IMPLICIT(k_ln_bwd, dy_dtype)
+#undef LN_EXTRA
+        } else
 #define LN_EXTRA
         if (x_dtype == MTLORA_F32 && dy_dtype == MTLORA_F32) {
             LN_DISPATCH_LPR(k_ln_bwd, float, float)
@@ -1183,6 +1349,27 @@
                              scratch_bytes, dx_addend, merge_h, merge_w, d_branch, scale, B, stream);
 }
 
+int mtlora_residual_layernorm_streams_implicit_fwd(int n, const void* shortcut, const void* const* inner, const float* scale_in,
+                                                   const void* const* branch, const float* scale, int64_t B, const float* gamma,
+                                                   const float* beta, void* const* y, float* const* mean, float* const* rstd,
+                                                   int64_t M, int64_t C, float eps, int x_dtype, int y_dtype, int merge_h,
+                                                   int merge_w, void* stream) {
+    if (!shortcut || !inner || !branch) return MTLORA_ERR_NULL;
+    return ln_multi_fwd_impl(n, inner, gamma, beta, y, mean, rstd, M, C, eps, x_dtype, y_dtype, merge_h, merge_w, branch, nullptr,
+                             scale, B, stream, shortcut, inner, scale_in);
+}
+
+int mtlora_residual_layernorm_streams_implicit_bwd(int n, const void* const* dy, const void* shortcut, const void* const* inner,
+                                                   const float* scale_in, const void* const* branch, const float* gamma,
+                                                   const float* const* mean, const float* const* rstd, void* const* d_res,
+                                                   void* const* d_branch, float* dgamma, float* dbeta, const float* scale,
+                                                   int64_t B, int64_t M, int64_t C, int x_dtype, int dy_dtype, void* scratch,
+                                                   int64_t scratch_bytes, int merge_h, int merge_w, void* stream) {
+    if (!shortcut || !inner || !branch || !d_branch) return MTLORA_ERR_NULL;
+    return ln_multi_bwd_impl(n, dy, inner, gamma, mean, rstd, d_res, dgamma, dbeta, M, C, x_dtype, dy_dtype, scratch, scratch_bytes,
+                             nullptr, merge_h, merge_w, d_branch, scale, B, stream, shortcut, branch, scale_in);
+}
+
 int mtlora_residual_layernorm_multi_fwd(int n, const void* shortcut, const void* const* branch, const float* scale, int64_t B,
                                         const float* gamma, const float* beta, void* const* x_new, void* const* y,
                                         float* const* mean, float* const* rstd, int64_t M, int64_t C, float eps, int x_dtype,
@@ -1190,14 +1377,19 @@
     int st = ln_check(M, C, x_dtype, y_dtype);
     if (st != MTLORA_OK) return st;
     if (n < 1 || n > MTLORA_MAX_TASKS + 1 || B <= 0 || M % B) return MTLORA_ERR_SHAPE;
-    if (!shortcut || !branch || !gamma || !beta || !x_new || !y || !mean || !rstd) return MTLORA_ERR_NULL;
+    if (!shortcut || !branch || !gamma || !beta || !y || !mean || !rstd) return MTLORA_ERR_NULL;
     if ((uintptr_t)shortcut & 15u) return MTLORA_ERR_ALIGN;
+    const bool implicit = x_new == nullptr;
+    if (implicit) {
+        st = ln_implicit_check(x_dtype, y_dtype);
+        if (st != MTLORA_OK) return st;
+    }
     LnParams p = {};
     for (int k = 0; k < n; ++k) {
-        if (!branch[k] || !x_new[k] || !y[k] || !mean[k] || !rstd[k]) return MTLORA_ERR_NULL;
-        if (((uintptr_t)branch[k] | (uintptr_t)x_new[k] | (uintptr_t)y[k]) & 15u) return MTLORA_ERR_ALIGN;
+        if (!branch[k] || (!implicit && !x_new[k]) || !y[k] || !mean[k] || !rstd[k]) return MTLORA_ERR_NULL;
+        if (((uintptr_t)branch[k] | (uintptr_t)(implicit ? nullptr : x_new[k]) | (uintptr_t)y[k]) & 15u) return MTLORA_ERR_ALIGN;
         p.rb_k[k] = branch[k];
-        p.xsum_k[k] = x_new[k];
+        p.xsum_k[k] = implicit ? nullptr : x_new[k];
         p.y_k[k] = y[k];
         p.mean_k[k] = mean[k];
         p.rstd_k[k] = rstd[k];
@@ -1208,7 +1400,7 @@
     p.gamma = gamma;
     p.beta = beta;
     p.rb = branch[0];
-    p.xsum = x_new[0];
+    p.xsum = implicit ? nullptr : x_new[0];
     p.y = y[0];
     p.mean = mean[0];
     p.rstd = rstd[0];
@@ -1227,8 +1419,13 @@
     const size_t lds = 0;
     hipStream_t s = (hipStream_t)stream;
     const int es_x = mtl_elem_size(x_dtype), es_y = mtl_elem_size(y_dtype);
-    mtl_prof_tag("M%lld C%lld x%d y%d n%d", (long long)M, (long long)C, x_dtype, y_dtype, n);
-    MtlProfScope prof(PK_LN_FWD, (double)M * C * (es_x + (double)n * (es_x + 2 * es_y)), s);
+    mtl_prof_tag("M%lld C%lld x%d y%d n%d impl%d", (long long)M, (long long)C, x_dtype, y_dtype, n, implicit ? 1 : 0);
+    MtlProfScope prof(PK_LN_FWD, (double)M * C * (es_x + (double)n * ((implicit ? 0 : es_x) + 2 * es_y)), s);
+    if (implicit) {
+#define LN_EXTRA , true, 1
+        LN_DISPATCH_IMPLICIT(k_ln_fwd, y_dtype)
+#undef LN_EXTRA
+    } else
 #define LN_EXTRA , true
     if (x_dtype == MTLORA_F32 && y_dtype == MTLORA_F32) {
         LN_DISPATCH_LPR(k_ln_fwd, float, float)
@@ -1252,13 +1449,19 @@
     return MTLORA_OK;
 }
 
-int mtlora_residual_layernorm_multi_bwd(int n, const void* const* dy, const void* const* x_new, const float* gamma,
-                                        const float* const* mean, const float* const* rstd, const void* const* dx_addend,
-                                        void* d_shortcut, void* const* d_branch, float* dgamma, float* dbeta, const float* scale,
-                                        int64_t B, int64_t M, int64_t C, int x_dtype, int dy_dtype, void* scratch,
-                                        int64_t scratch_bytes, void* stream) {
+static int resln_multi_bwd_impl(int n, const void* const* dy, const void* const* x_new, const float* gamma,
+                                const float* const* mean, const float* const* rstd, const void* const* dx_addend,
+                                void* d_shortcut, void* const* d_branch, float* dgamma, float* dbeta, const float* scale,
+                                int64_t B, int64_t M, int64_t C, int x_dtype, int dy_dtype, void* scratch,
+                                int64_t scratch_bytes, void* stream, const void* shortcut) {
+    const bool implicit = shortcut != nullptr;
     int st = ln_check(M, C, x_dtype, dy_dtype);
     if (st != MTLORA_OK) return st;
+    if (implicit) {
+        if ((uintptr_t)shortcut & 15u) return MTLORA_ERR_ALIGN;
+        st = ln_implicit_check(x_dtype, dy_dtype);
+        if (st != MTLORA_OK) return st;
+    }
     if (n < 1 || n > MTLORA_MAX_TASKS + 1 || B <= 0 || M % B) return MTLORA_ERR_SHAPE;
     if (!dy || !x_new || !gamma || !mean || !rstd || !d_shortcut || !dgamma || !dbeta || !scratch) return MTLORA_ERR_NULL;
     if (((uintptr_t)d_shortcut | (uintptr_t)scratch) & 15u) return MTLORA_ERR_ALIGN;
@@ -1277,12 +1480,14 @@
         if (((uintptr_t)dy[k] | (uintptr_t)x_new[k] | (uintptr_t)ad | (uintptr_t)db) & 15u) return MTLORA_ERR_ALIGN;
         p.dy_k[k] = dy[k];
         p.xsum_k[k] = const_cast<void*>(x_new[k]);
+        p.rb_k[k] = x_new[k];
         p.mean_k[k] = const_cast<float*>(mean[k]);
         p.rstd_k[k] = const_cast<float*>(rstd[k]);
         p.add_k[k] = ad;
         p.dbr_k[k] = db;
     }
     p.nk = n;
+    p.x = shortcut;
     p.gamma = gamma;
     p.dx = d_shortcut;
     p.rscale = scale;
@@ -1293,12 +1498,13 @@
     const int nvec_h = (int)(C / (x_dtype == MTLORA_F32 ? 4 : 8));
     const int lpr = pick_lpr(nvec_h);
     const int vpl = (nvec_h + lpr - 1) / lpr;
+    if (implicit && vpl > 3) return MTLORA_ERR_UNSUPPORTED;
     const int grid = ln_grid(M, lpr);
     const size_t lds = (size_t)4 * (64 / lpr) * 2 * C * 4;
     const int es_x = mtl_elem_size(x_dtype), es_g = mtl_elem_size(dy_dtype);
     {
-        mtl_prof_tag("M%lld C%lld x%d g%d n%d", (long long)M, (long long)C, x_dtype, dy_dtype, n);
-        MtlProfScope prof(PK_LN_BWD, (double)M * C * (es_x + (double)n * (2 * es_x + 2 * es_g)), s);
+        mtl_prof_tag("M%lld C%lld x%d g%d n%d impl%d", (long long)M, (long long)C, x_dtype, dy_dtype, n, implicit ? 1 : 0);
+        MtlProfScope prof(PK_LN_BWD, (double)M * C * ((implicit ? 2 : 1) * es_x + (double)n * ((implicit ? es_g : es_x) + es_x + 2 * es_g)), s);
 #define LN_EXTRA
         if (x_dtype == MTLORA_F32 && dy_dtype == MTLORA_F32) {
             LN_DISPATCH_LPR(k_resln_bwd_multi, float, float)
@@ -1323,6 +1529,25 @@
                        dbeta, grid, (int)C);
     MTL_CHECK_LAUNCH();
     return MTLORA_OK;
+}
+
+int mtlora_residual_layernorm_multi_bwd(int n, const void* const* dy, const void* const* x_new, const float* gamma,
+                                        const float* const* mean, const float* const* rstd, const void* const* dx_addend,
+                                        void* d_shortcut, void* const* d_branch, float* dgamma, float* dbeta, const float* scale,
+                                        int64_t B, int64_t M, int64_t C, int x_dtype, int dy_dtype, void* scratch,
+                                        int64_t scratch_bytes, void* stream) {
+    return resln_multi_bwd_impl(n, dy, x_new, gamma, mean, rstd, dx_addend, d_shortcut, d_branch, dgamma, dbeta, scale, B, M, C,
+                                x_dtype, dy_dtype, scratch, scratch_bytes, stream, nullptr);
+}
+
+int mtlora_residual_layernorm_multi_implicit_bwd(int n, const void* const* dy, const void* shortcut, const void* const* branch,
+                                                 const float* gamma, const float* const* mean, const float* const* rstd,
+                                                 const void* const* dx_addend, void* d_shortcut, void* const* d_branch,
+                                                 float* dgamma, float* dbeta, const float* scale, int64_t B, int64_t M, int64_t C,
+                                                 int x_dtype, int dy_dtype, void* scratch, int64_t scratch_bytes, void* stream) {
+    if (!shortcut || !branch) return MTLORA_ERR_NULL;
+    return resln_multi_bwd_impl(n, dy, branch, gamma, mean, rstd, dx_addend, d_shortcut, d_branch, dgamma, dbeta, scale, B, M, C,
+                                x_dtype, dy_dtype, scratch, scratch_bytes, stream, shortcut);
 }
 }
 
diff --git a/mtlora_amd/functional.py b/mtlora_amd/functional.py
--- a/mtlora_amd/functional.py
+++ b/mtlora_amd/functional.py
@@ -1094,6 +1094,169 @@
         keep = 1.0 - drop_prob
         scale = droppath_scale(n, B, keep, res[0].device)
     return ResidualMergeNormStreamsFn.apply(scale, mod.weight, mod.bias, mod.eps, out_dtype, H, W, n, *res, *branches)
+
+
+class _SkipLink:
+    __slots__ = ("d_res",)
+
+    def __init__(self):
+        self.d_res = None
+
+
+class ImplicitResiduals:
+    __slots__ = ("shortcut", "branches", "scale", "token", "link")
+
+    def __init__(self, shortcut, branches, scale, token, link):
+        self.shortcut, self.branches, self.scale, self.token, self.link = shortcut, branches, scale, token, link
+
+    def __len__(self):
+        return len(self.branches)
+
+
+class ImplicitResidualNorm2Fn(torch.autograd.Function):
+
+    @staticmethod
+    def forward(ctx, link, scale, weight, bias, eps: float, out_dtype: torch.dtype, n: int, shortcut, *branches):
+        L.require_gpu(shortcut, weight, bias, *branches)
+        C, B = shortcut.shape[-1], shortcut.shape[0]
+        s2 = shortcut.reshape(-1, C).contiguous()
+        bs = [b.reshape(-1, C).contiguous() for b in branches]
+        M = s2.shape[0]
+        w, b = weight.detach().float().contiguous(), bias.detach().float().contiguous()
+        ys = [torch.empty((M, C), dtype=out_dtype, device=s2.device) for _ in range(n)]
+        stats = torch.empty((2 * n, M), dtype=torch.float32, device=s2.device)
+        means, rstds = [stats[k] for k in range(n)], [stats[n + k] for k in range(n)]
+        st = L.lib().mtlora_residual_layernorm_multi_fwd(n, L.ptr(s2), L.ptr_array9(bs), L.ptr(scale), B, L.ptr(w), L.ptr(b),
+                                                         None, L.ptr_array9(ys), L.ptr_array9(means), L.ptr_array9(rstds), M, C,
+                                                         float(eps), L.dtype_code(s2), L.dtype_code(ys[0]), L.stream_ptr())
+        L.check(st, "mtlora_residual_layernorm_multi_fwd (implicit)")
+        ctx.save_for_backward(w, stats, scale, s2, *bs)
+        ctx.link = link
+        ctx.shape, ctx.MC, ctx.B, ctx.n, ctx.bdtype = shortcut.shape, (M, C), B, n, branches[0].dtype
+        token = torch.empty(0, dtype=torch.float32, device=s2.device)
+        return (token,) + tuple(y.view(shortcut.shape) for y in ys)
+
+    @staticmethod
+    def backward(ctx, g_token, *g_y):
+        w, stats, scale, s2, *bs = ctx.saved_tensors
+        n, (M, C) = ctx.n, ctx.MC
+        dev = s2.device
+        adds, ctx.link.d_res = ctx.link.d_res, None
+        dys = [g.reshape(M, C).to(ctx.bdtype).contiguous() for g in g_y]
+        lib = L.lib()
+        sb = lib.mtlora_layernorm_bwd_scratch_bytes(M, C, L.dtype_code(s2))
+        scratch = torch.empty(sb, dtype=torch.uint8, device=dev)
+        dsh = torch.empty_like(s2)
+        dbr = [torch.empty((M, C), dtype=ctx.bdtype, device=dev) for _ in range(n)]
+        dg = torch.empty(C, dtype=torch.float32, device=dev)
+        db = torch.empty(C, dtype=torch.float32, device=dev)
+        means, rstds = [stats[k] for k in range(n)], [stats[n + k] for k in range(n)]
+        st = lib.mtlora_residual_layernorm_multi_implicit_bwd(n, L.ptr_array9(dys), L.ptr(s2), L.ptr_array9(bs), L.ptr(w),
+                                                              L.ptr_array9(means), L.ptr_array9(rstds), L.ptr_array9(adds),
+                                                              L.ptr(dsh), L.ptr_array9(dbr), L.ptr(dg), L.ptr(db), L.ptr(scale),
+                                                              ctx.B, M, C, L.dtype_code(s2), L.dtype_code(dys[0]), L.ptr(scratch),
+                                                              sb, L.stream_ptr())
+        L.check(st, "mtlora_residual_layernorm_multi_implicit_bwd")
+        return (None, None, dg, db, None, None, None, dsh.view(ctx.shape), *[d.view(ctx.shape) for d in dbr])
+
+
+class ImplicitResidualMergeFn(torch.autograd.Function):
+
+    @staticmethod
+    def forward(ctx, link, scale_in, scale, weight, bias, eps: float, out_dtype: torch.dtype, H: int, W: int, n: int, token, shortcut,
+                *tensors):
+        inner, brs = tensors[:n], tensors[n:]
+        L.require_gpu(weight, bias, shortcut, *tensors)
+        B, Lt, Ct = shortcut.shape
+        C, M = 4 * Ct, B * Lt // 4
+        s2 = shortcut.contiguous()
+        i2 = [x.contiguous() for x in inner]
+        b2 = [x.contiguous() for x in brs]
+        w, b = weight.detach().float().contiguous(), bias.detach().float().contiguous()
+        y = torch.empty((n, M, C), dtype=out_dtype, device=s2.device)
+        stats = torch.empty((2 * n, M), dtype=torch.float32, device=s2.device)
+        means, rstds = [stats[k] for k in range(n)], [stats[n + k] for k in range(n)]
+        st = L.lib().mtlora_residual_layernorm_streams_implicit_fwd(n, L.ptr(s2), L.ptr_array9(i2), L.ptr(scale_in), L.ptr_array9(b2),
+                                                                    L.ptr(scale), B, L.ptr(w), L.ptr(b),
+                                                                    L.ptr_array9([y[k] for k in range(n)]), L.ptr_array9(means),
+                                                                    L.ptr_array9(rstds), M, C, float(eps), L.dtype_code(s2),
+                                                                    L.dtype_code(y), H, W, L.stream_ptr())
+        L.check(st, "mtlora_residual_layernorm_streams_implicit_fwd")
+        ctx.save_for_backward(w, stats, scale_in, scale, s2, *i2, *b2)
+        ctx.link = link
+        ctx.cfg = (n, M, C, H, W, B, shortcut.shape, brs[0].dtype)
+        return y.view(n * B, Lt // 4, C)
+
+    @staticmethod
+    def backward(ctx, g):
+        w, stats, scale_in, scale, s2, *rest = ctx.saved_tensors
+        n, M, C, H, W, B, shape, bdt = ctx.cfg
+        i2, b2 = rest[:n], rest[n:]
+        g3 = g.reshape(n, M, C)
+        if g3.dtype != bdt:
+            g3 = g3.to(bdt)
+        g3 = g3.contiguous()
+        dev = s2.device
+        lib = L.lib()
+        sb = lib.mtlora_layernorm_multi_bwd_scratch_bytes(n, M, C, L.dtype_code(s2))
+        scratch = torch.empty(sb, dtype=torch.uint8, device=dev)
+        dres = [torch.empty_like(s2) for _ in range(n)]
+        dbr = [torch.empty(shape, dtype=bdt, device=dev) for _ in range(n)]
+        dg = torch.empty(C, dtype=torch.float32, device=dev)
+        db = torch.empty(C, dtype=torch.float32, device=dev)
+        means, rstds = [stats[k] for k in range(n)], [stats[n + k] for k in range(n)]
+        st = lib.mtlora_residual_layernorm_streams_implicit_bwd(n, L.ptr_array9([g3[k] for k in range(n)]), L.ptr(s2), L.ptr_array9(i2),
+                                                                L.ptr(scale_in), L.ptr_array9(b2), L.ptr(w), L.ptr_array9(means),
+                                                                L.ptr_array9(rstds), L.ptr_array9(dres), L.ptr_array9(dbr), L.ptr(dg),
+                                                                L.ptr(db), L.ptr(scale), B, M, C, L.dtype_code(s2), L.dtype_code(g3),
+                                                                L.ptr(scratch), sb, H, W, L.stream_ptr())
+        L.check(st, "mtlora_residual_layernorm_streams_implicit_bwd")
+        g_token = None
+        if ctx.needs_input_grad[10]:
+            ctx.link.d_res = [d.view(-1, shape[-1]) for d in dres]
+            g_token = torch.empty(0, dtype=torch.float32, device=dev)
+        return (None, None, None, dg, db, None, None, None, None, None, g_token, None, *([None] * n), *dbr)
+
+
+def _plain_layer_norm(mod) -> bool:
+    return (type(mod) is torch.nn.LayerNorm and mod.elementwise_affine and mod.bias is not None and len(mod.normalized_shape) == 1)
+
+
+def implicit_residuals_ok(norm2: torch.nn.Module, merge_norm: torch.nn.Module, x: torch.Tensor, n: int, H: int, W: int) -> bool:
+    if not (torch.is_grad_enabled() and x.is_cuda and x.dim() == 3 and x.dtype == torch.float32 and 2 <= n <= L.MAX_TASKS + 1):
+        return False
+    C = x.shape[-1]
+    return (_plain_layer_norm(norm2) and _plain_layer_norm(merge_norm) and glue_dtype(x) in (torch.bfloat16, torch.float16)
+            and C % 8 == 0 and 4 * C <= 2048 and x.shape[1] == H * W and H % 2 == 0 and W % 2 == 0)
+
+
+def residual_layer_norm_multi_implicit(mod: torch.nn.Module, shortcut: torch.Tensor, branches, drop_prob: float, training: bool):
+    n = len(branches)
+    out_dtype = glue_dtype(shortcut)
+    ok = (shortcut.dtype == torch.float32 and out_dtype in (torch.bfloat16, torch.float16) and shortcut.dim() == 3
+          and all(b.shape == shortcut.shape and b.dtype == out_dtype and b.is_cuda for b in branches)
+          and (shortcut.requires_grad or any(b.requires_grad for b in branches)))
+    if not ok:
+        return None
+    scale = None
+    if training and drop_prob > 0.0:
+        scale = droppath_scale(n, shortcut.shape[0], 1.0 - drop_prob, shortcut.device)
+    link = _SkipLink()
+    outs = ImplicitResidualNorm2Fn.apply(link, scale, mod.weight, mod.bias, mod.eps, out_dtype, n, shortcut, *branches)
+    return ImplicitResiduals(shortcut, list(branches), scale, outs[0], link), list(outs[1:])
+
+
+def residual_merge_norm_implicit(mod: torch.nn.Module, res: "ImplicitResiduals", branches, H: int, W: int, drop_prob: float,
+                                 training: bool):
+    n = len(res)
+    sh = res.shortcut
+    if len(branches) != n or any(b.shape != sh.shape or b.dtype != res.branches[0].dtype or not b.is_cuda for b in branches):
+        raise RuntimeError("mtlora_amd: implicit task residuals need one MLP branch per stream, in the shape and dtype of the attention branches")
+    scale = None
+    if training and drop_prob > 0.0:
+        scale = droppath_scale(n, sh.shape[0], 1.0 - drop_prob, sh.device)
+    return ImplicitResidualMergeFn.apply(res.link, res.scale, scale, mod.weight, mod.bias, mod.eps, res.branches[0].dtype, H, W, n,
+                                         res.token, sh.detach(), *[b.detach() for b in res.branches], *branches)
 
 
 def layer_norm_merge_multi(mod: torch.nn.Module, xs, H: int, W: int):
diff --git a/mtlora_amd/swin_transformer_mtlora.py b/mtlora_amd/swin_transformer_mtlora.py
--- a/mtlora_amd/swin_transformer_mtlora.py
+++ b/mtlora_amd/swin_transformer_mtlora.py
@@ -20,6 +20,19 @@
     global _FUSED_BLOCKS
     prev, _FUSED_BLOCKS = _FUSED_BLOCKS, bool(on)
     return prev
+
+
+_IMPLICIT_RESIDUALS = os.environ.get("MTLORA_IMPLICIT_RESIDUALS", "1") != "0"
+
+
+def set_implicit_residuals(on: bool) -> bool:
+    global _IMPLICIT_RESIDUALS
+    prev, _IMPLICIT_RESIDUALS = _IMPLICIT_RESIDUALS, bool(on)
+    return prev
+
+
+def _has_hooks(m: nn.Module) -> bool:
+    return bool(m._forward_hooks or m._forward_pre_hooks or m._backward_hooks or m._backward_pre_hooks)
 
 
 def to_2tuple(v):
@@ -360,7 +373,7 @@
         merge = lambda v: WindowProcessReverse.apply(v.reshape(-1, ws, ws, C).contiguous(), B, H, W, C, s, ws).view(B, H * W, C)
         return merge(a), None if a_t is None else {t: merge(a_t[t]) for t in self.tasks}
 
-    def forward(self, x, normed=None, next_norm=None, defer_residual=False):
+    def forward(self, x, normed=None, next_norm=None, defer_residual=False, implicit_residual=False):
         H, W = self.input_resolution
         B, L, C = x.shape
         assert L == H * W, "input feature has wrong size"
@@ -375,6 +388,15 @@
         p_dp = self.drop_path.drop_prob if isinstance(self.drop_path, DropPath) else 0.0
         x_t = None
         xn2_t = None
+        imp = None
+        if a_t is not None and defer_residual and implicit_residual:
+            imp = Fn.residual_layer_norm_multi_implicit(self.norm2, shortcut, [a] + [a_t[t] for t in self.tasks], p_dp, self.training)
+        if imp is not None:
+            imp, xns = imp
+            m, m_t = self.mlp(xns[0], {t: xns[1 + i] for i, t in enumerate(self.tasks)})
+            if m_t is None:
+                raise RuntimeError("mtlora_amd: implicit task residuals need an Mlp with task outputs")
+            return None, None, None, (imp, [m] + [m_t[t] for t in self.tasks], p_dp)
         if a_t is not None:
             xs, xns = Fn.residual_layer_norm_multi(self.norm2, shortcut, [a] + [a_t[t] for t in self.tasks], p_dp, self.training)
             x, xn2 = xs[0], xns[0]
@@ -427,7 +449,10 @@
 
     def forward_residual_multi(self, res, branches, drop_prob, training):
         H, W = self.input_resolution
-        stacked = Fn.residual_merge_norm_streams(self.norm, res, branches, H, W, drop_prob, training)
+        if isinstance(res, Fn.ImplicitResiduals):
+            stacked = Fn.residual_merge_norm_implicit(self.norm, res, branches, H, W, drop_prob, training)
+        else:
+            stacked = Fn.residual_merge_norm_streams(self.norm, res, branches, H, W, drop_prob, training)
         if stacked is None:
             return self.forward_multi(Fn.residual_droppath(list(res), list(branches), drop_prob, training))
         y, _ = self.reduction(stacked)
@@ -504,6 +529,16 @@
     def invalidate_fused_cache(self) -> None:
         self.__dict__.pop("_fusable_cache", None)
 
+    def _implicit_residual(self, blk, x) -> bool:
+        ds = self.downsample
+        mods = (blk, blk.norm2, blk.mlp, ds, getattr(ds, "norm", None))
+        if not _IMPLICIT_RESIDUALS or self.tasks is None or any(m is None or _has_hooks(m) for m in mods):
+            return False
+        if not all(getattr(getattr(blk.mlp, f), "tasks", None) for f in ("fc1", "fc2")):
+            return False
+        H, W = self.input_resolution
+        return Fn.implicit_residuals_ok(blk.norm2, ds.norm, x, 1 + len(self.tasks), H, W)
+
     def forward(self, x):
         tasks_lora = None
         deferred = None
@@ -515,7 +550,7 @@
             last = i + 1 == len(self.blocks)
             defer = (last and blk.lora and self.downsample is not None and hasattr(self.downsample, "forward_residual_multi")
                      and self.training and torch.is_grad_enabled())
-            out = blk(x, normed, nxt, defer) if defer else blk(x, normed, nxt)
+            out = blk(x, normed, nxt, defer, self._implicit_residual(blk, x)) if defer else blk(x, normed, nxt)
             x, tasks_lora = out[0], out[1]
             normed = out[2] if len(out) > 2 else None
             deferred = out[3] if len(out) > 3 else None
```

Result: no change. 1129 images/sec (-0.0%).
